# keisuke-777/HandyRL

Measured on AMD Instinct MI355X. Metric: learner env-steps/sec at B=4096 T=32 (TicTacToe net, UPGO/VTRACE), higher is better.
Workload: dtype f32; 1 GPU; TicTacToe SimpleConv2dModel learner step: forward + IS ratios + fused HIP V-trace/UPGO scans + losses + backward + grad all-reduce + clip + Adam; global_batch=4096, per_gpu_batch=4096, seq_len=32, players=2, parallelism=dp1, hip_graph=True

## Files before the change

handyrl_amd/_native.py:

```python

import ctypes
import os

import torch

LIB_PATH = os.path.join(os.path.dirname(os.path.abspath(__file__)), '_lib', 'libhrl.so')
LIB_PATH = os.environ.get('HRL_LIB_PATH', LIB_PATH)

HRL_OK = 0
HRL_EINVAL = -22

ALG = {'MC': 0, 'TD': 1, 'UPGO': 2, 'VTRACE': 3}

_f32p = ctypes.c_void_p
_i64 = ctypes.c_int64
_dbl = ctypes.c_double

SIGNATURES = {
    'hrl_abi_version': (ctypes.c_int, []),
    'hrl_targets_set_short_form': (ctypes.c_int, [ctypes.c_int]),
    'hrl_strerror': (ctypes.c_char_p, [ctypes.c_int]),
    'hrl_compute_target': (ctypes.c_int, [
        ctypes.c_int, _f32p, _f32p, _f32p, _f32p, _f32p,
        _i64, _i64, _i64, _i64, _i64, _i64, _dbl, _dbl, _f32p, _f32p, ctypes.c_void_p]),
    'hrl_compute_targets_fused': (ctypes.c_int, [
        ctypes.c_int, ctypes.c_int, _f32p, _f32p, _f32p, _f32p, _f32p,
        _i64, _i64, _i64, _i64, _i64, _i64, _dbl, _dbl, _f32p, _f32p, ctypes.c_void_p]),
    'hrl_compute_targets_strided': (ctypes.c_int, [
        ctypes.c_int, ctypes.c_int, _f32p, _f32p, _f32p, _f32p, _f32p, ctypes.c_void_p,
        _i64, _i64, _i64, _i64, _i64, _dbl, _dbl, _f32p, _f32p, ctypes.c_void_p]),
    'hrl_bn_workspace_bytes': (ctypes.c_int64, [_i64, _i64, _i64]),
    'hrl_bn_forward_train': (ctypes.c_int, [
        _f32p, _i64, _i64, _i64, _f32p, _f32p, _f32p, _f32p, _dbl, _dbl, ctypes.c_int, _f32p, _f32p, _f32p,
        ctypes.c_void_p, _i64, ctypes.c_void_p]),
    'hrl_bn_backward': (ctypes.c_int, [
        _f32p, _f32p, _i64, _i64, _i64, _f32p, _f32p, _f32p, _f32p, ctypes.c_int, _f32p, _f32p, _f32p,
        ctypes.c_void_p, _i64, ctypes.c_void_p]),
    'hrl_bn_workspace_bytes_grouped': (ctypes.c_int64, [_i64, _i64, _i64, _i64]),
    'hrl_bn_forward_train_grouped': (ctypes.c_int, [
        _f32p, _i64, _i64, _i64, _i64, _f32p, _f32p, _f32p, _f32p, _dbl, _dbl, ctypes.c_int, _f32p, _f32p, _f32p,
        ctypes.c_void_p, _i64, ctypes.c_void_p]),
    'hrl_bn_backward_grouped': (ctypes.c_int, [
        _f32p, _f32p, _i64, _i64, _i64, _i64, _f32p, _f32p, _f32p, _f32p, ctypes.c_int, _f32p, _f32p, _f32p,
        ctypes.c_void_p, _i64, ctypes.c_void_p]),
    'hrl_loss_workspace_bytes': (ctypes.c_int64, [_i64, _i64, _i64, _i64]),
    'hrl_loss_forward': (ctypes.c_int, [
        _f32p, _f32p, ctypes.c_void_p, _i64, _i64, _i64, _i64, _i64,
        _f32p, _f32p, _f32p, _f32p, _f32p, _f32p, _f32p, _f32p, _f32p,
        ctypes.c_int, ctypes.c_int, ctypes.c_int, _dbl, _dbl, _dbl, _dbl,
        ctypes.c_void_p, _i64, _f32p, ctypes.c_void_p]),
    'hrl_loss_backward': (ctypes.c_int, [
        _f32p, ctypes.c_void_p, _i64, _i64, _i64, _i64, _i64,
        _f32p, _f32p, _f32p, _f32p, _f32p, _f32p, _dbl, _dbl,
        ctypes.c_void_p, _i64, _f32p, _f32p, _f32p, _f32p, ctypes.c_void_p]),
    'hrl_loss_partials': (ctypes.c_int64, [_i64, _i64, _i64, _i64, ctypes.c_void_p]),
    'hrl_loss_forward_ex': (ctypes.c_int, [
        _f32p, _f32p, ctypes.c_void_p, _i64, _i64, _i64, _i64, _i64,
        _f32p, _f32p, _f32p, _f32p, _f32p, _f32p, _f32p, _f32p, _f32p,
        ctypes.c_int, ctypes.c_int, ctypes.c_int, _dbl, _dbl, _dbl, _dbl,
        ctypes.c_void_p, _i64, _f32p, _f32p, _f32p, _f32p, _i64, ctypes.c_int, ctypes.c_void_p]),
    'hrl_loss_backward_ex': (ctypes.c_int, [
        _f32p, ctypes.c_void_p, _i64, _i64, _i64, _i64, _i64,
        _f32p, _f32p, _f32p, _f32p, _f32p, _f32p, _dbl, _dbl,
        ctypes.c_void_p, _i64, _f32p, _f32p, _f32p, _f32p, _f32p, _f32p, _f32p, _i64, _f32p, _f32p,
        ctypes.c_void_p]),
    'hrl_output_mask_forward': (ctypes.c_int, [_f32p, _f32p, _f32p, _f32p, _f32p, _i64, _i64, _i64, _i64, _f32p,
                                               _f32p, ctypes.c_void_p]),
    'hrl_output_mask_backward': (ctypes.c_int, [_f32p, _f32p, _f32p, _f32p, _i64, _i64, _i64, _i64, _f32p, _f32p,
                                                ctypes.c_void_p]),
    'hrl_board_weight': (ctypes.c_int, [_f32p, _i64, _i64, _i64, _i64, _i64, _i64, _f32p, ctypes.c_void_p]),
    'hrl_board_fold': (ctypes.c_int, [_f32p, _i64, _i64, _i64, _i64, _i64, _i64, _f32p, ctypes.c_void_p]),
    'hrl_board_bias': (ctypes.c_int, [_f32p, _i64, _i64, _f32p, ctypes.c_void_p]),
    'hrl_board_bias_fold': (ctypes.c_int, [_f32p, _i64, _i64, _f32p, ctypes.c_void_p]),
    'hrl_conv3x3_workspace_bytes': (ctypes.c_int64, [_i64]),
    'hrl_conv3x3_forward': (ctypes.c_int, [_f32p, _i64, _i64, _i64, _f32p, _f32p, ctypes.c_int, _f32p,
                                           ctypes.c_void_p, _i64, ctypes.c_void_p]),
    'hrl_conv3x3_wgrad': (ctypes.c_int, [_f32p, _f32p, _i64, _i64, _i64, _f32p, ctypes.c_void_p, _i64,
                                         ctypes.c_void_p]),
    'hrl_colsum_workspace_bytes': (ctypes.c_int64, [_i64, _i64]),
    'hrl_colsum': (ctypes.c_int, [_f32p, _i64, _i64, _f32p, ctypes.c_void_p, _i64, ctypes.c_void_p]),
    'hrl_bn_finalize_stats': (ctypes.c_int, [ctypes.c_void_p, _i64, _i64, _i64, _f32p, _f32p, _f32p, _f32p,
                                             ctypes.c_double, ctypes.c_double, _f32p, _f32p, _f32p, _f32p,
                                             ctypes.c_void_p]),
    'hrl_bn_forward_eval': (ctypes.c_int, [_f32p, _i64, _i64, _i64, _f32p, _f32p, _f32p, _f32p, ctypes.c_double,
                                           ctypes.c_int, _f32p, _f32p, ctypes.c_void_p]),
    'hrl_bn_apply': (ctypes.c_int, [_f32p, _i64, _i64, _i64, _f32p, _f32p, ctypes.c_int, _f32p, ctypes.c_void_p]),
    'hrl_conv3x3_stats_blocks': (ctypes.c_int64, [_i64]),
    'hrl_conv3x3_block_sum_blocks': (ctypes.c_int64, [_i64]),
    'hrl_conv3x3_set_split': (ctypes.c_int, [ctypes.c_int]),
    'hrl_conv3x3_set_block_form': (ctypes.c_int, [ctypes.c_int]),
    'hrl_conv3x3_set_fwd_form': (ctypes.c_int, [ctypes.c_int]),
    'hrl_torus_set_split': (ctypes.c_int, [ctypes.c_int]),
    'hrl_torus_set_form': (ctypes.c_int, [ctypes.c_int]),
    'hrl_conv3x3_pack_n': (ctypes.c_int, [ctypes.c_void_p, ctypes.c_int, _f32p, ctypes.c_void_p]),
    'hrl_conv3x3_pack_n_zero': (ctypes.c_int, [ctypes.c_void_p, ctypes.c_int, _f32p, _f32p, _i64, ctypes.c_void_p]),
    'hrl_conv3x3_forward_ex': (ctypes.c_int, [_f32p, _i64, _f32p, _f32p, _f32p, _f32p, ctypes.c_int, _f32p,
                                              ctypes.c_int, _f32p, _f32p, _f32p, _f32p, ctypes.c_void_p,
                                              ctypes.c_void_p, _i64, ctypes.c_void_p]),
    'hrl_bn_finalize_backward': (ctypes.c_int, [ctypes.c_void_p, _i64, _i64, _i64, _f32p, _f32p, _f32p, _f32p,
                                                _f32p, _f32p, ctypes.c_void_p]),
    'hrl_bn_backward_apply': (ctypes.c_int, [_f32p, _f32p, _i64, _i64, _i64, _f32p, _f32p, _f32p, _f32p,
                                             ctypes.c_int, _f32p, _f32p, _f32p, ctypes.c_void_p]),
    'hrl_conv3x3_block_backward': (ctypes.c_int, [_f32p, _f32p, _i64, _f32p, _f32p, _f32p, _f32p, _f32p, _f32p,
                                                  _f32p, _f32p, _f32p, _f32p, _f32p, _f32p, ctypes.c_int, _f32p,
                                                  _f32p, _f32p, ctypes.c_void_p, ctypes.c_void_p, _i64,
                                                  ctypes.c_void_p]),
    'hrl_conv3x3_block_backward_dz': (ctypes.c_int, [_f32p, _f32p, _f32p, _f32p, _i64, _f32p, _f32p, _f32p, _f32p,
                                                     _f32p, _f32p, _f32p, _f32p, _f32p, _f32p, _f32p, _f32p,
                                                     ctypes.c_int, _f32p, _f32p, _f32p, ctypes.c_void_p,
                                                     ctypes.c_void_p, _i64, ctypes.c_void_p]),
    'hrl_conv3x3_wgrad_ex': (ctypes.c_int, [_f32p, _f32p, _f32p, _f32p, _i64, _f32p, ctypes.c_void_p, _i64,
                                            ctypes.c_void_p]),
    'hrl_hidden_gather': (ctypes.c_int, [ctypes.c_void_p, _f32p, _i64, _i64, ctypes.c_int, ctypes.c_void_p,
                                         ctypes.c_int, ctypes.c_void_p, ctypes.c_void_p]),
    'hrl_hidden_gather_backward': (ctypes.c_int, [ctypes.c_void_p, _f32p, _i64, _i64, ctypes.c_int, ctypes.c_void_p,
                                                  ctypes.c_int, ctypes.c_void_p, ctypes.c_void_p]),
    'hrl_hidden_gather_backward_add': (ctypes.c_int, [ctypes.c_void_p, _f32p, _i64, _i64, ctypes.c_int,
                                                      ctypes.c_void_p, ctypes.c_int, ctypes.c_void_p, ctypes.c_void_p,
                                                      ctypes.c_void_p, ctypes.c_void_p]),
    'hrl_hidden_update_gather': (ctypes.c_int, [ctypes.c_void_p, ctypes.c_void_p, _i64, _f32p, _f32p, _i64, _i64,
                                                ctypes.c_int, ctypes.c_void_p, ctypes.c_int, ctypes.c_void_p,
                                                ctypes.c_void_p, ctypes.c_void_p]),
    'hrl_hidden_update_gather_backward': (ctypes.c_int, [ctypes.c_void_p, _f32p, _f32p, _i64, _i64, _i64,
                                                         ctypes.c_int, ctypes.c_void_p, ctypes.c_int, ctypes.c_void_p,
                                                         ctypes.c_void_p, ctypes.c_void_p, ctypes.c_void_p,
                                                         ctypes.c_void_p, ctypes.c_void_p, ctypes.c_void_p]),
    'hrl_hidden_update_backward_add': (ctypes.c_int, [ctypes.c_void_p, _f32p, _i64, _i64, _i64, ctypes.c_int,
                                                      ctypes.c_void_p, ctypes.c_void_p, ctypes.c_void_p,
                                                      ctypes.c_void_p, ctypes.c_void_p, ctypes.c_void_p]),
    'hrl_hidden_update': (ctypes.c_int, [ctypes.c_void_p, ctypes.c_void_p, _i64, _f32p, _i64, _i64, ctypes.c_int,
                                         ctypes.c_void_p, ctypes.c_void_p, ctypes.c_void_p]),
    'hrl_hidden_update_backward': (ctypes.c_int, [ctypes.c_void_p, _f32p, _i64, _i64, _i64, ctypes.c_int,
                                                  ctypes.c_void_p, ctypes.c_void_p, ctypes.c_void_p, ctypes.c_void_p]),
    'hrl_lstm_gates_forward': (ctypes.c_int, [_f32p, _i64, _f32p, _f32p, _i64, _i64, _i64, _f32p, _i64, _f32p,
                                              _f32p, _f32p, ctypes.c_void_p]),
    'hrl_lstm_gates_backward': (ctypes.c_int, [_f32p, _f32p, _f32p, _f32p, _f32p, _i64, _i64, _i64, _f32p, _f32p,
                                               ctypes.c_void_p]),
    'hrl_torus_workspace_bytes': (ctypes.c_int64, [_i64]),
    'hrl_torus_stats_blocks': (ctypes.c_int64, [_i64]),
    'hrl_torus_conv_forward': (ctypes.c_int, [_f32p, _i64, _i64, _i64, _i64, _i64, _f32p, _f32p, ctypes.c_int,
                                              _f32p, ctypes.c_void_p, _f32p, _f32p, ctypes.c_void_p, _i64,
                                              ctypes.c_void_p]),
    'hrl_stem_workspace_bytes': (ctypes.c_int64, [_i64]),
    'hrl_stem_forward': (ctypes.c_int, [_f32p, _i64, _i64, _f32p, _f32p, _f32p, ctypes.c_void_p]),
    'hrl_stem_wgrad': (ctypes.c_int, [_f32p, _f32p, _i64, _i64, _f32p, _f32p, ctypes.c_void_p, _i64,
                                      ctypes.c_void_p]),
    'hrl_stem_set_wgrad_form': (ctypes.c_int, [ctypes.c_int]),
    'hrl_stem_set_fwd_form': (ctypes.c_int, [ctypes.c_int]),
    'hrl_clip_grad_norm': (ctypes.c_int, [_f32p, _i64, _dbl, _f32p, ctypes.c_void_p]),
    'hrl_clip_workspace_bytes': (ctypes.c_int64, [_i64]),
    'hrl_grad_fold_norm_blocks': (ctypes.c_int64, [_i64]),
    'hrl_grad_fold_norm': (ctypes.c_int, [_f32p, _i64, ctypes.c_void_p, ctypes.c_void_p, ctypes.c_void_p,
                                          ctypes.c_void_p, ctypes.c_void_p, ctypes.c_void_p, ctypes.c_void_p,
                                          ctypes.c_int, _f32p, ctypes.c_void_p, ctypes.c_void_p, ctypes.c_int,
                                          ctypes.c_void_p, _i64, ctypes.c_void_p]),
    'hrl_grad_fold_norm_ex': (ctypes.c_int, [_f32p, _i64, ctypes.c_void_p, ctypes.c_void_p, ctypes.c_void_p,
                                             ctypes.c_void_p, ctypes.c_void_p, ctypes.c_void_p, ctypes.c_void_p,
                                             ctypes.c_int, _f32p, ctypes.c_void_p, ctypes.c_void_p, ctypes.c_int,
                                             ctypes.c_void_p, _i64, ctypes.c_void_p, _i64, _dbl, _f32p,
                                             ctypes.c_void_p]),
    'hrl_adam_clip': (ctypes.c_int, [_f32p, _i64, ctypes.c_void_p, _dbl, _f32p, ctypes.c_void_p, ctypes.c_void_p,
                                     ctypes.c_void_p, ctypes.c_int, _f32p, _f32p, _f32p, _f32p, _dbl, _dbl, _dbl,
                                     _dbl, ctypes.c_void_p, ctypes.c_int, _f32p, ctypes.c_void_p]),
    'hrl_conv3x3_wgrad_partials': (ctypes.c_int64, [_i64, ctypes.c_void_p]),
    'hrl_stem_wgrad_partials': (ctypes.c_int64, [_i64, ctypes.c_void_p]),
    'hrl_clip_grad_norm_ws': (ctypes.c_int, [_f32p, _i64, _dbl, _f32p, ctypes.c_void_p, _i64, ctypes.c_void_p]),
    'hrl_heads_workspace_bytes': (ctypes.c_int64, [_i64]),
    'hrl_heads_bn_parts': (ctypes.c_int64, [_i64]),
    'hrl_heads_set_bwd_form': (ctypes.c_int, [ctypes.c_int]),
    'hrl_heads_forward': (ctypes.c_int, [_f32p, _i64, _f32p, _f32p, _f32p, _f32p, _f32p, _f32p, _f32p, _f32p,
                                         _f32p, _f32p, _f32p, _f32p, ctypes.c_int, ctypes.c_void_p]),
    'hrl_heads_backward': (ctypes.c_int, [_f32p, _i64, _f32p, _f32p, _f32p, _f32p, _f32p, _f32p, _f32p,
                                          ctypes.c_void_p, _f32p, _f32p, _f32p, _f32p, _f32p, _f32p, _f32p, _f32p,
                                          _f32p, _f32p, _f32p, _f32p, ctypes.c_void_p, _i64, ctypes.c_void_p]),
    'hrl_heads_backward_dz': (ctypes.c_int, [_f32p, _i64, _f32p, _f32p, _f32p, _f32p, _f32p, _f32p, _f32p,
                                             ctypes.c_void_p, _f32p, _f32p, _f32p, _f32p, _f32p, _f32p, _f32p, _f32p,
                                             _f32p, _f32p, _f32p, _f32p, ctypes.c_void_p, _i64, ctypes.c_void_p]),
    'hrl_bn_apply_residual': (ctypes.c_int, [_f32p, _f32p, _i64, _i64, _i64, _f32p, _f32p, _f32p, ctypes.c_void_p]),
    'hrl_bn_backward_masked': (ctypes.c_int, [_f32p, _f32p, _f32p, _i64, _i64, _i64, _f32p, _f32p, _f32p, _f32p,
                                              _f32p, _f32p, ctypes.c_void_p, _i64, ctypes.c_void_p]),
    'hrl_torus_conv_wgrad': (ctypes.c_int, [_f32p, _f32p, _i64, _i64, _i64, _i64, _i64, _f32p, _f32p,
                                            ctypes.c_void_p, _i64, ctypes.c_void_p]),
    'hrl_torus_conv_wgrad_bn': (ctypes.c_int, [_f32p, _i64, _i64, _i64, _i64, _f32p, _f32p, _f32p, _f32p,
                                               ctypes.c_int, _f32p, _f32p, _f32p, _f32p, _f32p, _f32p, _f32p, _f32p,
                                               ctypes.c_void_p, _i64, ctypes.c_void_p]),
    'hrl_bn_backward_masked_coefs': (ctypes.c_int, [_f32p, _f32p, _f32p, _i64, _i64, _i64, _f32p, _f32p, _f32p,
                                                    _f32p, _f32p, _f32p, _f32p, ctypes.c_void_p, _i64,
                                                    ctypes.c_void_p]),
    'hrl_torus_unit_forward': (ctypes.c_int, [_f32p, _f32p, _f32p, _f32p, _f32p, _i64, _i64, _i64, _f32p, _f32p,
                                              _f32p, ctypes.c_void_p, ctypes.c_void_p, _i64, ctypes.c_void_p]),
    'hrl_torus_unit_input_grad': (ctypes.c_int, [_f32p, _i64, _i64, _i64, _f32p, _f32p, _f32p, _f32p, _f32p,
                                                 _f32p, _f32p, ctypes.c_void_p, ctypes.c_void_p, _i64,
                                                 ctypes.c_void_p]),
    'hrl_board_conv_workspace_bytes': (ctypes.c_int64, [_i64]),
    'hrl_board_conv_forward': (ctypes.c_int, [_f32p, _i64, _i64, _i64, _i64, _f32p, _i64, _i64, _i64, _f32p, _f32p,
                                              ctypes.c_void_p, _i64, ctypes.c_void_p]),
    'hrl_board_conv_pack': (ctypes.c_int, [_f32p, _i64, _i64, _i64, ctypes.c_void_p, _i64, ctypes.c_void_p]),
    'hrl_board_conv_forward_packed': (ctypes.c_int, [_f32p, _i64, _i64, _i64, _i64, ctypes.c_void_p, _i64, _f32p,
                                                     _f32p, ctypes.c_void_p]),
    'hrl_gboard_pack_bytes': (ctypes.c_int64, [_i64, _i64]),
    'hrl_gboard_pack': (ctypes.c_int, [_f32p, _i64, _i64, _i64, _i64, ctypes.c_void_p, _i64, ctypes.c_void_p]),
    'hrl_gboard_pack_adjoint': (ctypes.c_int, [_f32p, _i64, _i64, _i64, _i64, ctypes.c_void_p, _i64,
                                               ctypes.c_void_p]),
    'hrl_gboard_wgrad_workspace_bytes': (ctypes.c_int64, [_i64, _i64, _i64]),
    'hrl_gboard_wgrad': (ctypes.c_int, [ctypes.c_void_p, ctypes.c_void_p, ctypes.c_void_p, ctypes.c_void_p,
                                        ctypes.c_void_p, ctypes.c_int, _i64, _i64, _f32p, _i64, _i64, _f32p,
                                        ctypes.c_void_p, _i64, ctypes.c_void_p]),
    'hrl_gboard_set_whole_ring': (ctypes.c_int, [ctypes.c_int]),
    'hrl_gboard_set_nctw': (ctypes.c_int, [ctypes.c_int]),
    'hrl_gboard_launch_stats': (ctypes.c_int, [ctypes.c_void_p, ctypes.c_int, ctypes.c_int]),
    'hrl_gboard_pointwise_wgrad_workspace_bytes': (_i64, [_i64, _i64, _i64]),
    'hrl_gboard_pointwise_wgrad': (ctypes.c_int, [_f32p, _i64, _f32p, _i64, _i64, _i64, _i64, _f32p, ctypes.c_void_p,
                                                  _i64, ctypes.c_void_p]),
    'hrl_gboard_forward_groups': (ctypes.c_int, [ctypes.c_void_p, ctypes.c_void_p, _i64, _i64, _i64, ctypes.c_void_p,
                                                 _i64, _i64, _f32p, _i64, ctypes.c_void_p]),
    'hrl_lstm_gates_backward_ex': (ctypes.c_int, [_f32p, _f32p, _f32p, _f32p, _i64, ctypes.c_int, _i64, _f32p, _i64,
                                                  _i64, _i64, _f32p, _f32p, _f32p, ctypes.c_int, ctypes.c_void_p]),
    'hrl_lstm_gates_forward_grouped': (ctypes.c_int, [ctypes.c_int, _f32p, _i64, ctypes.c_void_p, ctypes.c_void_p,
                                                      ctypes.c_void_p, _i64, _i64, _i64, ctypes.c_void_p,
                                                      ctypes.c_void_p, ctypes.c_void_p, ctypes.c_void_p]),
    'hrl_gboard_forward': (ctypes.c_int, [_f32p, _i64, _f32p, _i64, _i64, _i64, _i64, ctypes.c_void_p, _i64, _i64,
                                          _f32p, _f32p, _f32p, ctypes.c_int, _f32p, _i64, ctypes.c_void_p]),
    'hrl_gboard_pointwise': (ctypes.c_int, [_f32p, _i64, _i64, _f32p, _i64, _i64, _i64, _f32p, _i64, _f32p, _f32p,
                                            ctypes.c_int, _f32p, _i64, ctypes.c_void_p]),
    'hrl_torus_head_pool': (ctypes.c_int, [_f32p, _f32p, _i64, _i64, _i64, _i64, _f32p, _f32p, ctypes.c_void_p]),
    'hrl_torus_head_unpool': (ctypes.c_int, [_f32p, _f32p, _f32p, _i64, _i64, _i64, _i64, _f32p,
                                             ctypes.c_void_p]),
    'hrl_bn_backward_apply_masked': (ctypes.c_int, [_f32p, _f32p, _f32p, _i64, _i64, _i64, _f32p, _f32p, _f32p,
                                                    _f32p, _f32p, _f32p, ctypes.c_void_p]),
    'hrl_geister_legal': (ctypes.c_int, [ctypes.c_void_p, ctypes.c_void_p, ctypes.c_void_p, _i64, ctypes.c_void_p,
                                         ctypes.c_void_p]),
    'hrl_geister_observation': (ctypes.c_int, [ctypes.c_void_p, ctypes.c_void_p, ctypes.c_void_p, ctypes.c_void_p,
                                               _i64, ctypes.c_int, _f32p, _f32p, ctypes.c_void_p]),
    'hrl_geister_step': (ctypes.c_int, [ctypes.c_void_p, ctypes.c_void_p, ctypes.c_void_p, ctypes.c_void_p,
                                        ctypes.c_void_p, ctypes.c_void_p, ctypes.c_void_p, ctypes.c_void_p,
                                        ctypes.c_void_p, _i64, ctypes.c_void_p, ctypes.c_void_p]),
    'hrl_selfplay_sample_record': (ctypes.c_int, [_f32p, _i64, ctypes.c_void_p, _f32p, ctypes.c_void_p, _f32p,
                                                  ctypes.c_void_p, ctypes.c_void_p, ctypes.c_void_p, _i64, _i64,
                                                  _i64, _i64, ctypes.c_void_p, _f32p, _f32p, ctypes.c_void_p, _f32p,
                                                  ctypes.c_void_p, ctypes.c_void_p, ctypes.c_void_p]),
    'hrl_masked_rows_copy': (ctypes.c_int, [ctypes.c_int, ctypes.c_void_p, ctypes.c_void_p, ctypes.c_void_p,
                                            ctypes.c_void_p, ctypes.c_void_p, ctypes.c_void_p, _i64,
                                            ctypes.c_void_p]),
    'hrl_geister_observation_record': (ctypes.c_int, [ctypes.c_void_p, ctypes.c_void_p, ctypes.c_void_p,
                                                      ctypes.c_void_p, _i64, ctypes.c_int, _f32p, _f32p,
                                                      ctypes.c_void_p, ctypes.c_void_p, _i64, _f32p, _f32p,
                                                      ctypes.c_void_p]),
    'hrl_geister_observation_record_at': (ctypes.c_int, [ctypes.c_void_p, ctypes.c_void_p, ctypes.c_void_p,
                                                         ctypes.c_void_p, _i64, ctypes.c_int, _f32p, _f32p,
                                                         ctypes.c_void_p, ctypes.c_void_p, _i64, _f32p, _f32p,
                                                         ctypes.c_void_p]),
    'hrl_selfplay_sample_record_stream': (ctypes.c_int, [_f32p, _i64, ctypes.c_void_p, ctypes.c_uint64,
                                                         ctypes.c_void_p, ctypes.c_void_p, _f32p, ctypes.c_void_p,
                                                         ctypes.c_void_p, ctypes.c_void_p, _i64, _i64, _i64, _i64,
                                                         ctypes.c_void_p, _f32p, _f32p, ctypes.c_void_p, _f32p,
                                                         ctypes.c_void_p, ctypes.c_void_p, ctypes.c_void_p]),
    'hrl_selfplay_harvest': (ctypes.c_int, [ctypes.c_void_p, ctypes.c_void_p, ctypes.c_void_p, _f32p, _dbl,
                                            ctypes.c_void_p, ctypes.c_void_p, ctypes.c_void_p, ctypes.c_void_p,
                                            ctypes.c_void_p, ctypes.c_void_p]),
    'hrl_eval_act': (ctypes.c_int, [_f32p, _i64, ctypes.c_void_p, ctypes.c_uint64, _dbl, ctypes.c_void_p,
                                    ctypes.c_void_p, ctypes.c_void_p, ctypes.c_void_p, _i64, ctypes.c_void_p, _i64, _i64,
                                    _i64, _i64, _i64, ctypes.c_void_p, ctypes.c_void_p, ctypes.c_void_p, _f32p,
                                    ctypes.c_void_p, ctypes.c_void_p]),
# ... 83 lines not shown
```

handyrl_amd/csrc/hrl_conv.hip:

```cpp

#include <hip/hip_runtime.h>
#include <stdint.h>
#include <stdlib.h>

#include <type_traits>

#include "../../include/hrl_nn.h"
#include "../../include/hrl_targets.h"
#include "hrl_split.h"
#include "hrl_stamps.h"

namespace {

HRL_STAMP_DECL

typedef float f32x4 __attribute__((ext_vector_type(4)));

constexpr int kBoard = 3;
constexpr int kCells = kBoard * kBoard;
constexpr int kTaps = 9;
constexpr int kC = 32;
constexpr int kRow = kC * kCells;
constexpr int kStride = kRow + 2;
constexpr int kTile = 16;
// ... 386 lines not shown
                }
            }
        }
        __builtin_amdgcn_wave_barrier();
    }
    __syncthreads();
    float *red = lds;
    constexpr int kW = kTaps * kC * kC;
#pragma unroll
    for (int t = 0; t < kTaps; ++t)
#pragma unroll
        for (int it = 0; it < 2; ++it)
#pragma unroll
            for (int jt = 0; jt < 2; ++jt)
#pragma unroll
                for (int r = 0; r < 4; ++r) {
                    const int ci = it * 16 + (lane >> 4) * 4 + r;
                    const int co = jt * 16 + (lane & 15);
                    red[wave * kW + (t * kC + ci) * kC + co] = acc[t][it][jt][r];
                }
    __syncthreads();
    float *out = partial + (int64_t)blockIdx.x * kW;
    for (int i = threadIdx.x; i < kW; i += kThreads)
        out[i] = ((red[i] + red[kW + i]) + red[2 * kW + i]) + red[3 * kW + i];
}

constexpr int kStrideW = kRow + 4;
typedef float f32x16 __attribute__((ext_vector_type(16)));
typedef __bf16 bf16x8_t __attribute__((ext_vector_type(8)));

__device__ __forceinline__ f32x16 mfma32(const uint4 &a, const uint4 &b, f32x16 c) {
    return __builtin_amdgcn_mfma_f32_32x32x16_bf16(__builtin_bit_cast(bf16x8_t, a), __builtin_bit_cast(bf16x8_t, b),
                                                   c, 0, 0, 0);
}

template <bool PRO>
__global__ __launch_bounds__(kThreads) void conv3x3_wgrad_split_kernel(const float *__restrict__ x,
                                                                       const float *__restrict__ in_alpha,
                                                                       const float *__restrict__ in_beta,
                                                                       const float *__restrict__ dy, int64_t M,
                                                                       float *__restrict__ partial) {
    __shared__ __attribute__((aligned(16))) float lds[2 * kWaves * kTile * kStrideW];
    static_assert(2 * kWaves * kTile * kStrideW >= kWaves * kTaps * kC * kC, "fold buffer");
    const int lane = threadIdx.x & 63;
    const int wave = threadIdx.x >> 6;
    float *xs = lds + wave * kTile * kStrideW;
    float *gs = lds + (kWaves + wave) * kTile * kStrideW;
    const int r = lane & 31, h = lane >> 5;
    float pa = 1.f, pb = 0.f;
    if constexpr (PRO) {
        pa = in_alpha[r];
        pb = in_beta[r];
    }
    const int64_t ntiles = (M + kTile - 1) / kTile;
    const int64_t stride = (int64_t)gridDim.x * kWaves;
    const int64_t lim = M * kRow;

    f32x16 acc[kTaps];
#pragma unroll
    for (int t = 0; t < kTaps; ++t)
#pragma unroll
        for (int i = 0; i < 16; ++i) acc[t][i] = 0.f;

    for (int64_t tile = (int64_t)blockIdx.x * kWaves + wave; tile < ntiles; tile += stride) {
        {
            const int64_t base = tile * kTile * kRow;
            float4 sx[kVec], sg[kVec];
#pragma unroll
            for (int k = 0; k < kVec; ++k) {
                const int64_t e = base + (int64_t)(k * 64 + lane) * 4;
                const int64_t ec = e < lim ? e : lim - 4;
                sx[k] = *reinterpret_cast<const float4 *>(x + ec);
                sg[k] = *reinterpret_cast<const float4 *>(dy + ec);
            }
#pragma unroll
            for (int k = 0; k < kVec; ++k) {
                const int e = (k * 64 + lane) * 4;
                const int row = e / kRow, c = e - row * kRow;
                const bool ok = base + e < lim;
                *reinterpret_cast<float4 *>(xs + row * kStrideW + c) = sx[k];
                *reinterpret_cast<float4 *>(gs + row * kStrideW + c) = ok ? sg[k] : make_float4(0.f, 0.f, 0.f, 0.f);
            }
        }
        __builtin_amdgcn_s_waitcnt(0xc07f);
        __builtin_amdgcn_wave_barrier();

        uint4 Bh[kCells], Bm[kCells], Bl[kCells];
        const float *gcol = gs + (8 * h) * kStrideW + r * kCells;
#pragma unroll
        for (int q = 0; q < kCells; ++q) {
            float v[8];
#pragma unroll
            for (int j = 0; j < 8; ++j) v[j] = gcol[j * kStrideW + q];
            hrl_split::split8(v, Bh[q], Bm[q], Bl[q]);
        }
        const float *xcol = xs + (8 * h) * kStrideW + r * kCells;
#pragma unroll
        for (int p = 0; p < kCells; ++p) {
            float v[8];
#pragma unroll
            for (int j = 0; j < 8; ++j) {
                float a = xcol[j * kStrideW + p];
                if constexpr (PRO) {
                    const float t = a * pa + pb;
                    a = t < 0.f ? 0.f : t;
                }
                v[j] = a;
            }
            uint4 Ah, Am, Al;
            hrl_split::split8(v, Ah, Am, Al);
#pragma unroll
            for (int q = 0; q < kCells; ++q) {
                const int tap = tap_of(p, q);
                if (tap < 0) continue;
                f32x16 c = acc[tap];
                c = mfma32(Al, Bh[q], c);
                c = mfma32(Am, Bm[q], c);
                c = mfma32(Ah, Bl[q], c);
                c = mfma32(Am, Bh[q], c);
                c = mfma32(Ah, Bm[q], c);
                c = mfma32(Ah, Bh[q], c);
                acc[tap] = c;
            }
        }
        __builtin_amdgcn_wave_barrier();
    }
    __syncthreads();
    float *red = lds;
    constexpr int kW = kTaps * kC * kC;
#pragma unroll
    for (int t = 0; t < kTaps; ++t)
#pragma unroll
        for (int i = 0; i < 16; ++i) {
            const int ci = (i & 3) + 8 * (i >> 2) + 4 * h;
            red[wave * kW + (t * kC + ci) * kC + r] = acc[t][i];
        }
    __syncthreads();
    float *out = partial + (int64_t)blockIdx.x * kW;
    for (int i = threadIdx.x; i < kW; i += kThreads)
        out[i] = ((red[i] + red[kW + i]) + red[2 * kW + i]) + red[3 * kW + i];
}

struct BlockBwdArgs {
    const float *g, *y;
    const float *bn_w, *bn_b, *bn_mean, *bn_invstd, *bn_k, *bn_gm;
    const float *x, *in_alpha, *in_beta;
    const float *wpk;
    const float *ep_mean, *ep_alpha, *ep_beta;
    float *gin;
    double *part;
    float *wpart;
    int64_t M;
    const float *w1p = nullptr, *w1v = nullptr;
};

typedef unsigned int u32x3 __attribute__((ext_vector_type(3)));
typedef unsigned int u32x2 __attribute__((ext_vector_type(2)));
typedef unsigned int u32x4 __attribute__((ext_vector_type(4)));

__device__ __forceinline__ __amdgpu_buffer_rsrc_t wave_rsrc(const void *base, uint32_t bytes) {
    const uint64_t p = reinterpret_cast<uint64_t>(base);
    const uint32_t lo = __builtin_amdgcn_readfirstlane((uint32_t)p);
    const uint32_t hi = __builtin_amdgcn_readfirstlane((uint32_t)(p >> 32));
    const uint32_t n = __builtin_amdgcn_readfirstlane(bytes);
    return __builtin_amdgcn_make_buffer_rsrc(reinterpret_cast<void *>(((uint64_t)hi << 32) | lo), (short)0, (int)n,
                                             0x00020000);
}

__device__ __forceinline__ void load_cells(__amdgpu_buffer_rsrc_t rs, int off, float (&d)[kCells]) {
#pragma unroll
    for (int m = 0; m < 3; ++m) {
        const u32x3 v = __builtin_amdgcn_raw_buffer_load_b96(rs, off + 12 * m, 0, 0);
        d[3 * m + 0] = __uint_as_float(v.x);
        d[3 * m + 1] = __uint_as_float(v.y);
        d[3 * m + 2] = __uint_as_float(v.z);
    }
}

__device__ __forceinline__ void store_cells(__amdgpu_buffer_rsrc_t rs, int off, const float (&d)[kCells]) {
#pragma unroll
    for (int m = 0; m < 3; ++m) {
        u32x3 v;
        v.x = __float_as_uint(d[3 * m + 0]);
        v.y = __float_as_uint(d[3 * m + 1]);
        v.z = __float_as_uint(d[3 * m + 2]);
        __builtin_amdgcn_raw_buffer_store_b96(v, rs, off + 12 * m, 0, 0);
    }
}

template <bool PRO, int EPI, bool DG>
__global__ __launch_bounds__(kThreads) void conv3x3_block_bwd_kernel(BlockBwdArgs a) {
    constexpr int kWWords = kTaps * 2 * 3 * 64 * 4;
    constexpr int kTileF = kTile * kStride;
    constexpr int kW = kTaps * kC * kC;
    constexpr int kFoldF = (kWaves - 1) * kW;
    constexpr int kUseF = DG ? kWWords + kWaves * kTileF : 0;
    constexpr int kSmemF = kUseF > kFoldF ? kUseF : kFoldF;
    __shared__ __attribute__((aligned(16))) float smem[kSmemF];
    uint32_t *w_lds_u = reinterpret_cast<uint32_t *>(smem);
    const int lane = threadIdx.x & 63;
    const int wave = threadIdx.x >> 6;
    float *as = smem + kWWords + wave * kTileF;
    if constexpr (DG) {
        for (int i = threadIdx.x; i < kWWords; i += kThreads) {
            const int d = i & 3, l = (i >> 2) & 63, f = i >> 8;
            const int part = f % 3, tc = f / 3;
            const int ci = 8 * (l >> 4) + 2 * d, j = l & 15;
            const float w0 = a.wpk[(tc * kC + ci) * 16 + j];
            const float w1 = a.wpk[(tc * kC + ci + 1) * 16 + j];
            w_lds_u[i] = split_part(w0, part) | (split_part(w1, part) << 16);
        }
    }
    const int r = lane & 31, h = lane >> 5;
    const float mu = a.bn_mean[r], kk = a.bn_k[r], gmn = a.bn_gm[r], is = a.bn_invstd[r];
    const float ww = a.bn_w ? a.bn_w[r] : 1.0f;
    const float al = is * ww;
    const float be = (a.bn_b ? a.bn_b[r] : 0.0f) - mu * al;
    float pa = 1.f, pb = 0.f;
    if constexpr (PRO) {
        pa = a.in_alpha[r];
        pb = a.in_beta[r];
    }
    float em = 0.f, ea = 1.f, eb = 0.f;
    if constexpr (DG && EPI == 2) {
        em = a.ep_mean[r];
        ea = a.ep_alpha[r];
        eb = a.ep_beta[r];
    }
    double s1 = 0.0, s2 = 0.0;
    f32x16 wacc[kTaps];
#pragma unroll
    for (int t = 0; t < kTaps; ++t)
#pragma unroll
        for (int i = 0; i < 16; ++i) wacc[t][i] = 0.f;
    if constexpr (DG) __syncthreads();

    const int64_t ntiles = (a.M + kTile - 1) / kTile;
    const int64_t stride = (int64_t)gridDim.x * kWaves;
    const int off0 = ((8 * h) * kRow + r * kCells) * 4;
    HRL_STAMP_WALL(14);
    int st_it = 0;
    for (int64_t tile = (int64_t)blockIdx.x * kWaves + wave; tile < ntiles; tile += stride, ++st_it) {
        if (st_it < 2) HRL_STAMP(6 * st_it + 0);
        const int64_t row0 = tile * kTile;
        const int rows = (int)min<int64_t>(kTile, a.M - row0);
        const uint32_t bytes = (uint32_t)rows * kRow * 4;
        const int64_t eofs = row0 * kRow;
        const __amdgpu_buffer_rsrc_t rg = wave_rsrc(a.g + eofs, bytes);
        const __amdgpu_buffer_rsrc_t ry = wave_rsrc(a.y + eofs, bytes);
        const __amdgpu_buffer_rsrc_t rx = wave_rsrc(a.x + eofs, bytes);
        float G[8][kCells], X[8][kCells];
        {
            float Y[8][kCells];
            auto bn_apply = [&]() __attribute__((always_inline)) {
#pragma unroll
                for (int j = 0; j < 8; ++j) {
                    const bool valid = 8 * h + j < rows;
#pragma unroll
                    for (int c = 0; c < kCells; ++c) {
                        const float yv = Y[j][c];
                        float gv = G[j][c];
                        if (!(yv * al + be > 0.f)) gv = 0.f;
                        const float t = (yv - mu) * kk;
                        const float d = (((gv - gmn) - t) * is) * ww;
                        G[j][c] = valid ? d : 0.f;
                    }
                }
            };
#pragma unroll
            for (int j = 0; j < 8; ++j) {
                load_cells(rg, off0 + j * kRow * 4, G[j]);
                load_cells(ry, off0 + j * kRow * 4, Y[j]);
                load_cells(rx, off0 + j * kRow * 4, X[j]);
            }
            bn_apply();
        }
        if (st_it < 2) HRL_STAMP(6 * st_it + 1);
        if constexpr (DG) {
#pragma unroll
            for (int j = 0; j < 8; ++j)
#pragma unroll
                for (int c = 0; c < kCells; ++c) as[(8 * h + j) * kStride + r * kCells + c] = G[j][c];
        }
        {
            uint4 Bh[kCells], Bm[kCells], Bl[kCells];
#pragma unroll
            for (int q = 0; q < kCells; ++q) {
                float v[8];
#pragma unroll
                for (int j = 0; j < 8; ++j) v[j] = G[j][q];
                hrl_split::split8(v, Bh[q], Bm[q], Bl[q]);
            }
#pragma unroll
            for (int p = 0; p < kCells; ++p) {
                float v[8];
#pragma unroll
                for (int j = 0; j < 8; ++j) {
                    float xv = X[j][p];
                    if constexpr (PRO) {
                        const float t = xv * pa + pb;
                        xv = t < 0.f ? 0.f : t;
                    }
                    v[j] = xv;
                }
                uint4 Ah, Am, Al;
                hrl_split::split8(v, Ah, Am, Al);
#pragma unroll
                for (int q = 0; q < kCells; ++q) {
                    const int tap = tap_of(p, q);
                    if (tap < 0) continue;
                    f32x16 c = wacc[tap];
                    c = mfma32(Al, Bh[q], c);
                    c = mfma32(Am, Bm[q], c);
                    c = mfma32(Ah, Bl[q], c);
                    c = mfma32(Am, Bh[q], c);
                    c = mfma32(Ah, Bm[q], c);
                    c = mfma32(Ah, Bh[q], c);
                    wacc[tap] = c;
                }
            }
        }
        if (st_it < 2) HRL_STAMP(6 * st_it + 2);
        if constexpr (DG) {
            float R[8][kCells];
            if constexpr (EPI == 2 || EPI == 3) {
#pragma unroll
                for (int j = 0; j < 8; ++j) load_cells(rx, off0 + j * kRow * 4, R[j]);
            }
            __builtin_amdgcn_s_waitcnt(0xc07f);
            __builtin_amdgcn_wave_barrier();
            f32x4 acc[kCells][2];
#pragma unroll
            for (int q = 0; q < kCells; ++q) acc[q][0] = acc[q][1] = (f32x4){0.f, 0.f, 0.f, 0.f};
            split_tile_mfma<false, true>(as, w_lds_u, lane, nullptr, nullptr, acc);
            __builtin_amdgcn_s_waitcnt(0xc07f);
            __builtin_amdgcn_wave_barrier();
            if (st_it < 2) HRL_STAMP(6 * st_it + 3);
#pragma unroll
            for (int q = 0; q < kCells; ++q)
#pragma unroll
                for (int ct = 0; ct < 2; ++ct)
#pragma unroll
                    for (int rr = 0; rr < 4; ++rr) {
                        const int row = (lane >> 4) * 4 + rr;
                        const int co = ct * 16 + (lane & 15);
                        as[row * kStride + co * kCells + q] = acc[q][ct][rr];
                    }
            __builtin_amdgcn_s_waitcnt(0xc07f);
            __builtin_amdgcn_wave_barrier();
            const __amdgpu_buffer_rsrc_t ro = wave_rsrc(a.gin + eofs, bytes);
            float t1 = 0.f, t2 = 0.f;
#pragma unroll
            for (int j = 0; j < 8; ++j) {
                const bool valid = 8 * h + j < rows;
                float o[kCells];
#pragma unroll
                for (int c = 0; c < kCells; ++c) {
                    float v = as[(8 * h + j) * kStride + r * kCells + c];
                    const float rv = (EPI == 2 || EPI == 3) ? R[j][c] : 0.f;
                    if constexpr (EPI == 3) {
                        if (!(rv > 0.f)) v = 0.f;
                    } else if constexpr (EPI == 2) {
                        const float gm = (rv * ea + eb > 0.f && valid) ? v : 0.f;
                        t1 += gm;
                        t2 += gm * (rv - em);
                    }
                    o[c] = v;
                }
                store_cells(ro, off0 + j * kRow * 4, o);
            }
            if constexpr (EPI == 2) {
                s1 += (double)t1;
                s2 += (double)t2;
            }
            __builtin_amdgcn_s_waitcnt(0xc07f);
            __builtin_amdgcn_wave_barrier();
        }
        if (st_it < 2) HRL_STAMP(6 * st_it + 4);
    }
    HRL_STAMP(12);
    __syncthreads();
    float *red = smem;
    if (wave > 0) {
#pragma unroll
        for (int t = 0; t < kTaps; ++t)
#pragma unroll
            for (int i = 0; i < 16; ++i) {
                const int ci = (i & 3) + 8 * (i >> 2) + 4 * h;
                red[(wave - 1) * kW + (t * kC + ci) * kC + r] = wacc[t][i];
            }
    }
    __syncthreads();
    if (wave == 0) {
        float *out = a.wpart + (int64_t)blockIdx.x * kW;
#pragma unroll
        for (int t = 0; t < kTaps; ++t)
#pragma unroll
            for (int i = 0; i < 16; ++i) {
                const int idx = (t * kC + (i & 3) + 8 * (i >> 2) + 4 * h) * kC + r;
                out[idx] = ((wacc[t][i] + red[idx]) + red[kW + idx]) + red[2 * kW + idx];
            }
    }
    if constexpr (DG && EPI == 2) {
        __syncthreads();
        double *dred = reinterpret_cast<double *>(smem);
        dred[((wave * 2 + h) * kC + r) * 2 + 0] = s1;
        dred[((wave * 2 + h) * kC + r) * 2 + 1] = s2;
        __syncthreads();
        if (threadIdx.x < 2 * kC) {
            const int c = threadIdx.x >> 1, k = threadIdx.x & 1;
            double t = 0.0;
            for (int i = 0; i < 2 * kWaves; ++i) t += dred[(i * kC + c) * 2 + k];
            a.part[((int64_t)blockIdx.x * kC + c) * 2 + k] = t;
        }
    }
    HRL_STAMP(13);
    HRL_STAMP_WALL(15);
}

namespace bb2 {

constexpr int kWaves = 8;
constexpr int kThreads = 64 * kWaves;
constexpr int kPartBytes = kCells * kC * kTile * 2;
constexpr int kImgBytes = 3 * kPartBytes;
constexpr int kDy0 = 0;
constexpr int kX0 = 2 * kImgBytes;
constexpr int kXrStride = kRow + 4;
constexpr int kXrBytes = kTile * kXrStride * 4;
constexpr int kXr0 = 4 * kImgBytes;
constexpr int kLdsBytes = kXr0 + 2 * kXrBytes;
static_assert(kLdsBytes <= 160 * 1024, "LDS");
constexpr int kDzStride = 28;
constexpr int kDzBytes = kTile * kDzStride * 4;
constexpr int kDz0 = kLdsBytes;
constexpr int kLdsBytesDz = kDz0 + 2 * kDzBytes;
static_assert(kLdsBytesDz <= 160 * 1024, "LDS");
static_assert(kDzBytes / 4 <= 7 * 64, "a dword per lane of waves 0..6");

typedef short v4s __attribute__((ext_vector_type(4)));
typedef __attribute__((address_space(3))) v4s lds_v4s;

__device__ __forceinline__ int img_off(int c, int ch, int half) {
    const int R = ch >> 3, j = ch & 7;
    return c * 1024 + R * 256 + 16 * ((2 * j + half) ^ (9 * (R & 1)));
}

__device__ __forceinline__ void bar_lds() {
    asm volatile("s_waitcnt lgkmcnt(0)" ::: "memory");
    __builtin_amdgcn_s_barrier();
    asm volatile("" ::: "memory");
}

template <int W> struct Role;
template <> struct Role<0> { static constexpr bool kIg = true, kCFirst = true; static constexpr int kCt = 0, kNq = 5, kNt = 0;
                             static constexpr int kQ[5] = {4, 5, 6, 7, 8}; static constexpr int kTap[1] = {0}; };
template <> struct Role<1> { static constexpr bool kIg = true, kCFirst = true; static constexpr int kCt = 1, kNq = 5, kNt = 0;
                             static constexpr int kQ[5] = {4, 5, 6, 7, 8}; static constexpr int kTap[1] = {0}; };
template <> struct Role<2> { static constexpr bool kIg = true, kCFirst = false; static constexpr int kCt = 0, kNq = 4, kNt = 0;
                             static constexpr int kQ[4] = {0, 1, 2, 3}; static constexpr int kTap[1] = {0}; };
template <> struct Role<3> { static constexpr bool kIg = true, kCFirst = false; static constexpr int kCt = 1, kNq = 4, kNt = 0;
                             static constexpr int kQ[4] = {0, 1, 2, 3}; static constexpr int kTap[1] = {0}; };
template <> struct Role<4> { static constexpr bool kIg = false, kCFirst = false; static constexpr int kCt = 0, kNq = 0, kNt = 2;
                             static constexpr int kQ[1] = {0}; static constexpr int kTap[2] = {0, 1}; };
template <> struct Role<5> { static constexpr bool kIg = false, kCFirst = false; static constexpr int kCt = 0, kNq = 0, kNt = 2;
                             static constexpr int kQ[1] = {0}; static constexpr int kTap[2] = {2, 5}; };
template <> struct Role<6> { static constexpr bool kIg = false, kCFirst = true; static constexpr int kCt = 0, kNq = 0, kNt = 2;
                             static constexpr int kQ[1] = {0}; static constexpr int kTap[2] = {3, 4}; };
template <> struct Role<7> { static constexpr bool kIg = false, kCFirst = true; static constexpr int kCt = 0, kNq = 0, kNt = 3;
                             static constexpr int kQ[1] = {0}; static constexpr int kTap[3] = {6, 7, 8}; };

template <int W> __device__ constexpr bool uses_p(int p) {
    using R = Role<W>;
    if constexpr (R::kIg) {
        for (int s = 0; s < R::kNq; ++s)
            if (tap_of(p, R::kQ[s]) >= 0) return true;
    } else {
        for (int s = 0; s < R::kNt; ++s) {
            const int dy = R::kTap[s] / 3, dx = R::kTap[s] % 3;
            const int qy = p / 3 - dy + 1, qx = p % 3 - dx + 1;
            if (qy >= 0 && qy < 3 && qx >= 0 && qx < 3) return true;
        }
    }
    return false;
}
template <int W> __device__ constexpr bool uses_tap(int t) {
    using R = Role<W>;
    for (int s = 0; s < R::kNq; ++s)
        for (int p = 0; p < kCells; ++p)
            if (tap_of(p, R::kQ[s]) == t) return true;
    return false;
}

#ifdef HRL_STAMPS
#define BB2_STAMP(it, k)                                                                                        \
    do {                                                                                                       \
        if ((it) == 2 || (it) == 3) {                                                                          \
            const unsigned long long t_ = __builtin_amdgcn_s_memtime();                                        \
            if (lane == 0 && g_hrl_stamps)                                                                     \
                g_hrl_stamps[(((size_t)blockIdx.x * 8 + W) * 2 + (it) - 2) * 8 + (k)] = t_;                    \
        }                                                                                                      \
    } while (0)
#else
#define BB2_STAMP(it, k) do { } while (0)
#endif

template <bool PRO, int EPI, int W, bool DZ = false>
__device__ __forceinline__ void run(const BlockBwdArgs &a, unsigned char *smem, int lane) {
    static_assert(!DZ || EPI == 2, "the dz form is the last chain block's");
    using R = Role<W>;
    constexpr bool kIg = R::kIg;
    constexpr int kNq = R::kNq > 0 ? R::kNq : 1;
    constexpr int kNt = R::kNt > 0 ? R::kNt : 1;
    constexpr int kCt = R::kCt;
    const int ch = lane & 31, hh = lane >> 5;
    constexpr bool kFwd = EPI == 1;
    float mu = 0.f, kk = 0.f, gmn = 0.f, is = 1.f, ww = 1.f, al = 1.f, be = 0.f;
    if constexpr (!kFwd) {
        kk = a.bn_k[ch]; gmn = a.bn_gm[ch];
        mu = a.bn_mean[ch]; is = a.bn_invstd[ch];
        ww = a.bn_w ? a.bn_w[ch] : 1.0f;
        al = is * ww;
        be = (a.bn_b ? a.bn_b[ch] : 0.0f) - mu * al;
    }
    float pa = 1.f, pb = 0.f;
    if constexpr (PRO) {
        pa = a.in_alpha[ch];
        pb = a.in_beta[ch];
    }
    float w1[3] = {0.f, 0.f, 0.f};
    if constexpr (DZ) {
        w1[0] = a.w1p[ch];
        w1[1] = a.w1p[kC + ch];
        w1[2] = a.w1v[ch];
    }
    uint4 wh[kTaps], wm[kTaps], wl[kTaps];
    if constexpr (kIg) {
        const int ci0 = 8 * (lane >> 4), j = lane & 15;
#pragma unroll
        for (int t = 0; t < kTaps; ++t) {
            if (!uses_tap<W>(t)) continue;
            uint32_t hv[4], mv[4], lv[4];
#pragma unroll
            for (int d = 0; d < 4; ++d) {
                const int tc = t * 2 + kCt;
                const float w0 = a.wpk[(tc * kC + ci0 + 2 * d) * 16 + j];
                const float w1 = a.wpk[(tc * kC + ci0 + 2 * d + 1) * 16 + j];
                uint32_t h0, m0, l0, h1, m1, l1;
                hrl_split::split3(w0, h0, m0, l0);
                hrl_split::split3(w1, h1, m1, l1);
                hv[d] = h0 | (h1 << 16);
                mv[d] = m0 | (m1 << 16);
                lv[d] = l0 | (l1 << 16);
            }
            wh[t] = make_uint4(hv[0], hv[1], hv[2], hv[3]);
            wm[t] = make_uint4(mv[0], mv[1], mv[2], mv[3]);
            wl[t] = make_uint4(lv[0], lv[1], lv[2], lv[3]);
        }
    }
    float em = 0.f, ea = 1.f, eb = 0.f;
    if constexpr (EPI == 2 && kIg) {
        em = a.ep_mean[kCt * 16 + (lane & 15)];
        ea = a.ep_alpha[kCt * 16 + (lane & 15)];
        eb = a.ep_beta[kCt * 16 + (lane & 15)];
    }
    double s1 = 0.0, s2 = 0.0;
    f32x16 wacc[kNt];
#pragma unroll
    for (int t = 0; t < kNt; ++t)
#pragma unroll
        for (int i = 0; i < 16; ++i) wacc[t][i] = 0.f;

    const int64_t ntiles = (a.M + kTile - 1) / kTile;
    const int64_t t0 = blockIdx.x;
    const int64_t step = gridDim.x;
    const int n_iter = t0 < ntiles ? (int)((ntiles - 1 - t0) / step + 1) : 0;
    const int rho0 = 2 * ((W + (ch >> 2)) & 7);
    const int c0 = hh ? 4 : 0;
    const int ldoff = (rho0 * kRow + ch * kCells + c0) * 4;
    float G[2][5], Y[2][5], X[2][5];
    auto rsrc_of = [&](const float *base, int it, int &rows) __attribute__((always_inline)) {
        const int64_t t = t0 + (int64_t)it * step;
        const bool ok = it < n_iter;
        rows = ok ? (int)min<int64_t>(kTile, a.M - t * kTile) : 0;
        return wave_rsrc(base + (ok ? t * kTile * kRow : 0), (uint32_t)rows * kRow * 4);
    };
    auto issue = [&](int it) __attribute__((always_inline)) {
        int rows;
        const __amdgpu_buffer_rsrc_t rg = rsrc_of(a.g, it, rows), ry = rsrc_of(a.y, it, rows),
                                     rx = rsrc_of(a.x, it, rows);
#pragma unroll
        for (int r = 0; r < 2; ++r) {
            const int off = ldoff + r * kRow * 4;
#pragma unroll
            for (int k = kFwd ? 2 : (DZ ? 1 : 0); k < 3; ++k) {
                const __amdgpu_buffer_rsrc_t rs = k == 0 ? rg : (k == 1 ? ry : rx);
                float(&d)[5] = k == 0 ? G[r] : (k == 1 ? Y[r] : X[r]);
                const u32x3 v = __builtin_amdgcn_raw_buffer_load_b96(rs, off, 0, 0);
                const u32x2 u = __builtin_amdgcn_raw_buffer_load_b64(rs, off + 12, 0, 0);
                d[0] = __uint_as_float(v.x);
                d[1] = __uint_as_float(v.y);
                d[2] = __uint_as_float(v.z);
                d[3] = __uint_as_float(u.x);
                d[4] = __uint_as_float(u.y);
            }
        }
    };
    auto load_dz = [&](int it) __attribute__((always_inline)) {
        float v = 0.f;
        if constexpr (DZ && W < 7) {
            const int64_t t = t0 + (int64_t)it * step;
            const bool ok = it < n_iter;
            const int rows = ok ? (int)min<int64_t>(kTile, a.M - t * kTile) : 0;
            const __amdgpu_buffer_rsrc_t rz =
                wave_rsrc(a.g + (ok ? t * kTile * kDzStride : 0), (uint32_t)rows * kDzStride * 4);
            v = __uint_as_float(__builtin_amdgcn_raw_buffer_load_b32(rz, (W * 64 + lane) * 4, 0, 0));
        }
        return v;
    };
    auto put_dz = [&](int it, float v) __attribute__((always_inline)) {
        if constexpr (DZ && W < 7)
            reinterpret_cast<float *>(smem + kDz0 + (it & 1) * kDzBytes)[W * 64 + lane] = v;
    };
    float DZv = 0.f;
    auto stage = [&](int it) __attribute__((always_inline)) {
        const int64_t t = t0 + (int64_t)it * step;
        const int rows = (int)max<int64_t>(0, min<int64_t>(kTile, a.M - t * kTile));
        unsigned char *dyi = smem + kDy0 + (it & 1) * kImgBytes;
        unsigned char *xi = smem + kX0 + (it & 1) * kImgBytes;
        const float *dzl = reinterpret_cast<const float *>(smem + kDz0 + (it & 1) * kDzBytes);
        uint32_t dp[3][5], xp[3][5];
#pragma unroll
        for (int i = 0; i < 5; ++i) {
            float dv[2], xv2[2];
#pragma unroll
            for (int r = 0; r < 2; ++r) {
                const bool valid = rho0 + r < rows;
                const float yv = Y[r][i];
                float gv;
                if constexpr (DZ) {
                    const float *dzr = dzl + (rho0 + r) * kDzStride + c0 + i;
                    gv = 0.f;
#pragma unroll
                    for (int m = 0; m < 3; ++m) gv += w1[m] * dzr[m * kCells];
                } else {
                    gv = G[r][i];
                }
                if (!(yv * al + be > 0.f)) gv = 0.f;
                const float tt = (yv - mu) * kk;
                float d = (((gv - gmn) - tt) * is) * ww;
                d = valid ? d : 0.f;
                float xv = X[r][i];
                if constexpr (PRO) {
                    const float u = xv * pa + pb;
                    xv = u < 0.f ? 0.f : u;
                }
                if constexpr (kFwd) d = xv;
                dv[r] = d;
                xv2[r] = xv;
            }
            hrl_split::split_pair(dv[0], dv[1], dp[0][i], dp[1][i], dp[2][i]);
            if constexpr (!kFwd) hrl_split::split_pair(xv2[0], xv2[1], xp[0][i], xp[1][i], xp[2][i]);
        }
        const int half = rho0 >> 3, sub = 2 * (rho0 & 7);
#pragma unroll
        for (int i = 0; i < 5; ++i) {
            const int o = img_off(c0 + i, ch, half) + sub;
#pragma unroll
            for (int part = 0; part < 3; ++part) {
                *reinterpret_cast<uint32_t *>(dyi + part * kPartBytes + o) = dp[part][i];
                if constexpr (!kFwd) *reinterpret_cast<uint32_t *>(xi + part * kPartBytes + o) = xp[part][i];
            }
        }
        if constexpr (EPI == 2 || EPI == 3) {
            float *xr = reinterpret_cast<float *>(smem + kXr0 + (it & 1) * kXrBytes);
#pragma unroll
            for (int r = 0; r < 2; ++r)
#pragma unroll
                for (int i = 0; i < 5; ++i) xr[(rho0 + r) * kXrStride + ch * kCells + c0 + i] = X[r][i];
        }
    };
    f32x4 acc[kNq];
    auto compute = [&](int it) __attribute__((always_inline)) {
        const unsigned char *dyi = smem + kDy0 + (it & 1) * kImgBytes;
        if constexpr (!kIg && kFwd) {
        } else if constexpr (!kIg) {
            const unsigned char *xi = smem + kX0 + (it & 1) * kImgBytes;
            const int kg = lane >> 5;
#pragma unroll
            for (int p = 0; p < kCells; ++p) {
                if (!uses_p<W>(p)) continue;
                const int o = img_off(p, ch, kg);
                const uint4 Ah = *reinterpret_cast<const uint4 *>(xi + o);
                const uint4 Am = *reinterpret_cast<const uint4 *>(xi + kPartBytes + o);
                const uint4 Al = *reinterpret_cast<const uint4 *>(xi + 2 * kPartBytes + o);
#pragma unroll
                for (int s = 0; s < R::kNt; ++s) {
                    const int dy = R::kTap[s] / 3, dx = R::kTap[s] % 3;
                    const int qy = p / 3 - dy + 1, qx = p % 3 - dx + 1;
                    if (qy < 0 || qy > 2 || qx < 0 || qx > 2) continue;
                    const int ob = img_off(qy * 3 + qx, ch, kg);
                    const uint4 Bh = *reinterpret_cast<const uint4 *>(dyi + ob);
                    const uint4 Bm = *reinterpret_cast<const uint4 *>(dyi + kPartBytes + ob);
                    const uint4 Bl = *reinterpret_cast<const uint4 *>(dyi + 2 * kPartBytes + ob);
                    f32x16 c = wacc[s];
                    c = mfma32(Al, Bh, c);
                    c = mfma32(Am, Bm, c);
                    c = mfma32(Ah, Bl, c);
                    c = mfma32(Am, Bh, c);
                    c = mfma32(Ah, Bm, c);
                    c = mfma32(Ah, Bh, c);
                    wacc[s] = c;
                }
            }
        } else {
#pragma unroll
            for (int s = 0; s < kNq; ++s) acc[s] = (f32x4){0.f, 0.f, 0.f, 0.f};
            const int g = lane >> 4, i = lane & 15, qq = i >> 2, pp = i & 3;
            const int tr_sub = 8 * (pp & 1);
#pragma unroll
            for (int p = 0; p < kCells; ++p) {
                if (!uses_p<W>(p)) continue;
                uint32_t A[3][4];
#pragma unroll
                for (int part = 0; part < 3; ++part) {
#pragma unroll
                    for (int hlf = 0; hlf < 2; ++hlf) {
                        const int o = part * kPartBytes + img_off(p, 8 * g + 4 * hlf + qq, pp >> 1) + tr_sub;
                        const v4s r = __builtin_amdgcn_ds_read_tr16_b64_v4i16(
                            (lds_v4s *)((__attribute__((address_space(3))) unsigned char *)(dyi + o)));
                        const uint2 u = __builtin_bit_cast(uint2, r);
                        A[part][2 * hlf] = u.x;
                        A[part][2 * hlf + 1] = u.y;
                    }
                }
                const uint4 Ah = make_uint4(A[0][0], A[0][1], A[0][2], A[0][3]);
                const uint4 Am = make_uint4(A[1][0], A[1][1], A[1][2], A[1][3]);
                const uint4 Al = make_uint4(A[2][0], A[2][1], A[2][2], A[2][3]);
#pragma unroll
                for (int s = 0; s < R::kNq; ++s) {
                    const int tap = tap_of(p, R::kQ[s]);
                    if (tap < 0) continue;
                    const uint4 Bl = wl[tap];
                    f32x4 c = acc[s];
                    c = mfma_bf16(Al, wh[tap], c);
                    c = mfma_bf16(Am, wm[tap], c);
                    c = mfma_bf16(Ah, Bl, c);
                    c = mfma_bf16(Am, wh[tap], c);
                    c = mfma_bf16(Ah, wm[tap], c);
                    c = mfma_bf16(Ah, wh[tap], c);
                    acc[s] = c;
                }
            }
        }
    };
    auto epilogue = [&](int it) __attribute__((always_inline)) {
        if constexpr (kIg) {
            int rows;
            const __amdgpu_buffer_rsrc_t ro = rsrc_of(a.gin, it, rows);
            const int co = kCt * 16 + (lane & 15);
            float rv[kNq < 4 ? 4 : kNq][4];
            if constexpr (EPI == 2 || EPI == 3) {
                const float *xr = reinterpret_cast<const float *>(smem + kXr0 + (it & 1) * kXrBytes);
#pragma unroll
                for (int rr = 0; rr < 4; ++rr) {
                    const int row = (lane >> 4) * 4 + rr;
#pragma unroll
                    for (int s = 0; s < R::kNq; ++s) rv[s][rr] = xr[row * kXrStride + co * kCells + R::kQ[s]];
                }
            }
            if constexpr (EPI == 1) {
                float t1 = 0.f, t2 = 0.f;
#pragma unroll
                for (int s = 0; s < R::kNq; ++s) {
#pragma unroll
                    for (int rr = 0; rr < 4; ++rr) {
                        const int row = (lane >> 4) * 4 + rr;
                        const float u = row < rows ? acc[s][rr] : 0.f;
                        t1 += u;
                        t2 += u * u;
                    }
                }
                s1 += (double)t1;
                s2 += (double)t2;
            }
            if constexpr (EPI == 2) {
                float t1 = 0.f, t2 = 0.f;
#pragma unroll
                for (int s = 0; s < R::kNq; ++s) {
#pragma unroll
                    for (int rr = 0; rr < 4; ++rr) {
                        const int row = (lane >> 4) * 4 + rr;
                        const float x0 = rv[s][rr];
                        const float gm = (x0 * ea + eb > 0.f && row < rows) ? acc[s][rr] : 0.f;
                        t1 += gm;
                        t2 += gm * (x0 - em);
                    }
                }
                s1 += (double)t1;
                s2 += (double)t2;
            }
#pragma unroll
            for (int rr = 0; rr < 4; ++rr) {
                const int row = (lane >> 4) * 4 + rr;
                const int off = (row * kRow + co * kCells + R::kQ[0]) * 4;
                float v[kNq];
#pragma unroll
                for (int s = 0; s < R::kNq; ++s) {
                    v[s] = acc[s][rr];
                    if constexpr (EPI == 3)
                        if (!(rv[s][rr] > 0.f)) v[s] = 0.f;
                }
                u32x4 w;
                w.x = __float_as_uint(v[0]);
                w.y = __float_as_uint(v[1]);
                w.z = __float_as_uint(v[2]);
                w.w = __float_as_uint(v[3]);
                __builtin_amdgcn_raw_buffer_store_b128(w, ro, off, 0, 0);
                if constexpr (R::kNq > 4)
                    __builtin_amdgcn_raw_buffer_store_b32(__float_as_uint(v[4 % kNq]), ro, off + 16, 0, 0);
            }
        }
    };

    if constexpr (DZ) {
        if (n_iter > 0) {
            const float d0 = load_dz(0), d1 = load_dz(1);
            issue(0);
            put_dz(0, d0);
            put_dz(1, d1);
            DZv = load_dz(2);
        }
        bar_lds();
        if (n_iter > 0) {
            stage(0);
            issue(1);
        }
    } else if (n_iter > 0) {
        issue(0);
        stage(0);
        issue(1);
    }
    bar_lds();
    for (int it = 0; it < n_iter; ++it) {
        BB2_STAMP(it, 0);
        if constexpr (R::kCFirst) {
            compute(it);
            epilogue(it);
            BB2_STAMP(it, 1);
            stage(it + 1);
            if constexpr (DZ) {
                put_dz(it + 2, DZv);
                DZv = load_dz(it + 3);
            }
            issue(it + 2);
            BB2_STAMP(it, 2);
        } else {
            stage(it + 1);
            if constexpr (DZ) {
                put_dz(it + 2, DZv);
                DZv = load_dz(it + 3);
            }
            issue(it + 2);
            BB2_STAMP(it, 1);
            compute(it);
            epilogue(it);
            BB2_STAMP(it, 2);
        }
        bar_lds();
        BB2_STAMP(it, 3);
    }
    if constexpr (!kIg && !kFwd) {
        constexpr int kW = kTaps * kC * kC;
        float *outp = a.wpart + (int64_t)blockIdx.x * kW;
        const int h = lane >> 5;
#pragma unroll
        for (int s = 0; s < R::kNt; ++s)
#pragma unroll
            for (int i = 0; i < 16; ++i) {
                const int ci = (i & 3) + 8 * (i >> 2) + 4 * h;
                outp[(R::kTap[s] * kC + ci) * kC + ch] = wacc[s][i];
            }
    }
    if constexpr (EPI == 1 || EPI == 2) {
        __syncthreads();
        double *dred = reinterpret_cast<double *>(smem);
        if (kIg) {
            dred[(W * 64 + lane) * 2 + 0] = s1;
            dred[(W * 64 + lane) * 2 + 1] = s2;
        }
        __syncthreads();
        if (W == 0) {
            const int c = lane >> 1, k = lane & 1, ct = c >> 4, l16 = c & 15;
            double tot = 0.0;
            for (int w = ct; w < 4; w += 2)
                for (int lg = 0; lg < 4; ++lg) tot += dred[(w * 64 + lg * 16 + l16) * 2 + k];
            a.part[((int64_t)blockIdx.x * kC + c) * 2 + k] = tot;
        }
    }
}

}

namespace fw3 {

constexpr int kSlots = 5;
constexpr int kRawBytes = kTile * kRow * 4;
constexpr int kPieces = kRawBytes / 1024;
constexpr int kImg0 = 0;
constexpr int kRaw0 = 2 * bb2::kImgBytes;
constexpr int kLdsBytes = kRaw0 + kSlots * kRawBytes;
static_assert(kLdsBytes <= 160 * 1024, "LDS");
static_assert(kRawBytes % 1024 == 0, "whole LDS-DMA pieces per tile");

template <int N> __device__ __forceinline__ void vm_wait() { asm volatile("s_waitcnt vmcnt(%0)" ::"n"(N) : "memory"); }

__device__ __forceinline__ void dma16(u32x4 desc, uint32_t voff, uint32_t lds_byte) {
    uint32_t keep;
    asm volatile("s_mov_b32 %0, m0\n\ts_mov_b32 m0, %3\n\ts_nop 0\n\tbuffer_load_dwordx4 %1, %2, 0 offen lds\n\t"
                 "s_mov_b32 m0, %0"
                 : "=&s"(keep)
                 : "v"(voff), "s"(desc), "s"(lds_byte)
                 : "memory");
}

__device__ __forceinline__ u32x4 wave_desc(const void *base, uint32_t bytes) {
    const uint64_t p = reinterpret_cast<uint64_t>(base);
    u32x4 d;
    d.x = __builtin_amdgcn_readfirstlane((uint32_t)p);
    d.y = __builtin_amdgcn_readfirstlane((uint32_t)(p >> 32)) & 0xffffu;
    d.z = __builtin_amdgcn_readfirstlane(bytes);
    d.w = 0x00020000u;
    return d;
}

template <int G> struct Cells;
template <> struct Cells<0> { static constexpr int kN = 3; static constexpr int kQ[3] = {0, 1, 2}; };
template <> struct Cells<1> { static constexpr int kN = 2; static constexpr int kQ[2] = {3, 4}; };
template <> struct Cells<2> { static constexpr int kN = 2; static constexpr int kQ[2] = {5, 6}; };
template <> struct Cells<3> { static constexpr int kN = 2; static constexpr int kQ[2] = {7, 8}; };

template <int G> __device__ constexpr bool g_uses_p(int p) {
    for (int s = 0; s < Cells<G>::kN; ++s)
        if (tap_of(p, Cells<G>::kQ[s]) >= 0) return true;
    return false;
}
template <int G> __device__ constexpr bool g_uses_tap(int t) {
    for (int s = 0; s < Cells<G>::kN; ++s)
        for (int p = 0; p < kCells; ++p)
            if (tap_of(p, Cells<G>::kQ[s]) == t) return true;
    return false;
}

template <int W> __device__ constexpr int pieces_of() {
    int n = 0;
    for (int p = W; p < kPieces; p += 8) ++n;
    return n;
}

template <int NP, int NS>
__device__ __forceinline__ void wait_tile_after(int it) {
    static_assert((kSlots - 2) * (NP + NS) + NS <= 63, "vmcnt");
    if (it == 0) vm_wait<(kSlots - 2) * NP + NS>();
    else if (it == 1) vm_wait<(kSlots - 2) * NP + 2 * NS>();
    else if (it == 2) vm_wait<(kSlots - 2) * NP + 3 * NS>();
    else vm_wait<(kSlots - 2) * (NP + NS) + NS>();
    static_assert(kSlots == 5, "the early-iteration counts above are written for kSlots = 5");
}

template <bool PRO, int W>
__device__ __forceinline__ void run(const BlockBwdArgs &a, unsigned char *smem, int lane) {
    constexpr int kCt = W & 1, G = W >> 1;
    using C = Cells<G>;
    constexpr int kNq = C::kN;
    constexpr int NP = pieces_of<W>();
    constexpr int NS = 4;
    const int64_t ntiles = (a.M + kTile - 1) / kTile;
    const int64_t t0 = blockIdx.x;
    const int64_t step = gridDim.x;
    const int n_iter = t0 < ntiles ? (int)((ntiles - 1 - t0) / step + 1) : 0;
    const int ch = lane & 31, hh = lane >> 5;
    uint4 wh[kTaps], wm[kTaps], wl[kTaps];
    {
        const int ci0 = 8 * (lane >> 4), j = lane & 15;
#pragma unroll
        for (int t = 0; t < kTaps; ++t) {
            if (!g_uses_tap<G>(t)) continue;
            uint32_t hv[4], mv[4], lv[4];
#pragma unroll
            for (int d = 0; d < 4; ++d) {
                const int tc = t * 2 + kCt;
                const float w0 = a.wpk[(tc * kC + ci0 + 2 * d) * 16 + j];
                const float w1 = a.wpk[(tc * kC + ci0 + 2 * d + 1) * 16 + j];
                uint32_t h0, m0, l0, h1, m1, l1;
                hrl_split::split3(w0, h0, m0, l0);
                hrl_split::split3(w1, h1, m1, l1);
                hv[d] = h0 | (h1 << 16);
                mv[d] = m0 | (m1 << 16);
                lv[d] = l0 | (l1 << 16);
            }
            wh[t] = make_uint4(hv[0], hv[1], hv[2], hv[3]);
            wm[t] = make_uint4(mv[0], mv[1], mv[2], mv[3]);
            wl[t] = make_uint4(lv[0], lv[1], lv[2], lv[3]);
        }
    }
    float pa = 1.f, pb = 0.f;
    if constexpr (PRO) {
        pa = a.in_alpha[ch];
        pb = a.in_beta[ch];
    }
    asm volatile("s_waitcnt vmcnt(0)" ::: "memory");
    const uint32_t smem_base = (uint32_t)(uintptr_t)smem;
    auto dma = [&](int it, int slot) __attribute__((always_inline)) {
        const int64_t t = t0 + (int64_t)it * step;
        const bool ok = it < n_iter;
        const int rows = ok ? (int)min<int64_t>(kTile, a.M - t * kTile) : 0;
        const u32x4 desc = wave_desc(a.x + (ok ? t * kTile * kRow : 0), (uint32_t)rows * kRow * 4);
        const uint32_t raw = smem_base + kRaw0 + (uint32_t)slot * kRawBytes;
#pragma unroll
        for (int j = 0; j < NP; ++j) {
            const int p = W + 8 * j;
            dma16(desc, p * 1024 + lane * 16, raw + p * 1024);
        }
    };
    const int c0 = hh ? 4 : 0;
    const int rho0 = 2 * ((W + (ch >> 2)) & 7);
    auto stage = [&](int it, int slot) __attribute__((always_inline)) {
        const float *raw = reinterpret_cast<const float *>(smem + kRaw0 + slot * kRawBytes);
        unsigned char *xi = smem + kImg0 + (it & 1) * bb2::kImgBytes;
        uint32_t xp[3][5];
        float xv[2][5];
#pragma unroll
        for (int r = 0; r < 2; ++r) {
            const float *src = raw + (rho0 + r) * kRow + ch * kCells + c0;
#pragma unroll
            for (int i = 0; i < 5; ++i) {
                float v = src[i];
                if constexpr (PRO) {
                    const float u = v * pa + pb;
                    v = u < 0.f ? 0.f : u;
                }
                xv[r][i] = v;
            }
        }
#pragma unroll
        for (int i = 0; i < 5; ++i) hrl_split::split_pair(xv[0][i], xv[1][i], xp[0][i], xp[1][i], xp[2][i]);
        const int half = rho0 >> 3, sub = 2 * (rho0 & 7);
#pragma unroll
        for (int i = 0; i < 5; ++i) {
            const int o = bb2::img_off(c0 + i, ch, half) + sub;
#pragma unroll
            for (int part = 0; part < 3; ++part)
                *reinterpret_cast<uint32_t *>(xi + part * bb2::kPartBytes + o) = xp[part][i];
        }
    };
    const int co = kCt * 16 + (lane & 15);
    const int g = lane >> 4, i16 = lane & 15, qq = i16 >> 2, pp = i16 & 3;
    const int tr_sub = 8 * (pp & 1);
    double s1 = 0.0, s2 = 0.0;
#pragma unroll
    for (int j = 0; j < kSlots; ++j) dma(j, j);
    vm_wait<(kSlots - 1) * NP>();
    bb2::bar_lds();
    stage(0, 0);
    vm_wait<(kSlots - 2) * NP>();
    bb2::bar_lds();
    int slot = 0;
    for (int it = 0; it < n_iter; ++it) {
        BB2_STAMP(it, 0);
        dma(it + kSlots, slot);
        const int next = slot + 1 == kSlots ? 0 : slot + 1;
        stage(it + 1, next);
        BB2_STAMP(it, 1);
        const unsigned char *img = smem + kImg0 + (it & 1) * bb2::kImgBytes;
        f32x4 acc[kNq];
#pragma unroll
        for (int s = 0; s < kNq; ++s) acc[s] = (f32x4){0.f, 0.f, 0.f, 0.f};
#pragma unroll
        for (int p = 0; p < kCells; ++p) {
            if (!g_uses_p<G>(p)) continue;
            uint32_t A[3][4];
#pragma unroll
            for (int part = 0; part < 3; ++part) {
#pragma unroll
                for (int hlf = 0; hlf < 2; ++hlf) {
                    const int o = part * bb2::kPartBytes + bb2::img_off(p, 8 * g + 4 * hlf + qq, pp >> 1) + tr_sub;
                    const bb2::v4s r = __builtin_amdgcn_ds_read_tr16_b64_v4i16(
                        (bb2::lds_v4s *)((__attribute__((address_space(3))) unsigned char *)(img + o)));
                    const uint2 u = __builtin_bit_cast(uint2, r);
                    A[part][2 * hlf] = u.x;
                    A[part][2 * hlf + 1] = u.y;
                }
            }
            const uint4 Ah = make_uint4(A[0][0], A[0][1], A[0][2], A[0][3]);
            const uint4 Am = make_uint4(A[1][0], A[1][1], A[1][2], A[1][3]);
            const uint4 Al = make_uint4(A[2][0], A[2][1], A[2][2], A[2][3]);
#pragma unroll
            for (int s = 0; s < kNq; ++s) {
                const int tap = tap_of(p, C::kQ[s]);
                if (tap < 0) continue;
                f32x4 c = acc[s];
                c = mfma_bf16(Al, wh[tap], c);
                c = mfma_bf16(Am, wm[tap], c);
                c = mfma_bf16(Ah, wl[tap], c);
                c = mfma_bf16(Am, wh[tap], c);
                c = mfma_bf16(Ah, wm[tap], c);
                c = mfma_bf16(Ah, wh[tap], c);
                acc[s] = c;
            }
        }
        BB2_STAMP(it, 2);
        const int64_t t = t0 + (int64_t)it * step;
        const int rows = (int)min<int64_t>(kTile, a.M - t * kTile);
        const __amdgpu_buffer_rsrc_t od = wave_rsrc(a.gin + t * kTile * kRow, (uint32_t)rows * kRow * 4);
        float t1 = 0.f, t2 = 0.f;
#pragma unroll
        for (int s = 0; s < kNq; ++s) {
#pragma unroll
            for (int rr = 0; rr < 4; ++rr) {
                const int row = (lane >> 4) * 4 + rr;
                const float u = row < rows ? acc[s][rr] : 0.f;
                t1 += u;
                t2 += u * u;
            }
        }
        s1 += (double)t1;
        s2 += (double)t2;
#pragma unroll
        for (int rr = 0; rr < 4; ++rr) {
            const int row = (lane >> 4) * 4 + rr;
            const int off = (row * kRow + co * kCells + C::kQ[0]) * 4;
            if constexpr (kNq == 3) {
                u32x3 v;
                v.x = __float_as_uint(acc[0][rr]);
                v.y = __float_as_uint(acc[1][rr]);
                v.z = __float_as_uint(acc[2 % kNq][rr]);
                __builtin_amdgcn_raw_buffer_store_b96(v, od, off, 0, 0);
            } else {
                u32x2 v;
                v.x = __float_as_uint(acc[0][rr]);
                v.y = __float_as_uint(acc[1][rr]);
                __builtin_amdgcn_raw_buffer_store_b64(v, od, off, 0, 0);
            }
        }
        wait_tile_after<NP, NS>(it);
        BB2_STAMP(it, 3);
        bb2::bar_lds();
        slot = next;
    }
    vm_wait<0>();
    __syncthreads();
    double *dred = reinterpret_cast<double *>(smem);
    dred[(W * 64 + lane) * 2 + 0] = s1;
    dred[(W * 64 + lane) * 2 + 1] = s2;
    __syncthreads();
    if (W == 0) {
        const int c = lane >> 1, k = lane & 1, ct = c >> 4, l16 = c & 15;
        double tot = 0.0;
        for (int w = ct; w < 8; w += 2)
            for (int lg = 0; lg < 4; ++lg) tot += dred[(w * 64 + lg * 16 + l16) * 2 + k];
        a.part[((int64_t)blockIdx.x * kC + c) * 2 + k] = tot;
    }
}

}

template <bool PRO>
__global__ __launch_bounds__(bb2::kThreads) void conv3x3_fwd_dma_kernel(BlockBwdArgs a) {
    __shared__ __attribute__((aligned(16))) unsigned char smem[fw3::kLdsBytes];
    const int lane = threadIdx.x & 63;
    const int wave = __builtin_amdgcn_readfirstlane(threadIdx.x >> 6);
    switch (wave) {
    case 0: fw3::run<PRO, 0>(a, smem, lane); break;
    case 1: fw3::run<PRO, 1>(a, smem, lane); break;
    case 2: fw3::run<PRO, 2>(a, smem, lane); break;
    case 3: fw3::run<PRO, 3>(a, smem, lane); break;
    case 4: fw3::run<PRO, 4>(a, smem, lane); break;
    case 5: fw3::run<PRO, 5>(a, smem, lane); break;
    case 6: fw3::run<PRO, 6>(a, smem, lane); break;
    default: fw3::run<PRO, 7>(a, smem, lane); break;
    }
}

template <bool PRO, int EPI, bool DZ = false>
__global__ __launch_bounds__(bb2::kThreads) void conv3x3_block_bwd2_kernel(BlockBwdArgs a) {
    __shared__ __attribute__((aligned(16))) unsigned char smem[DZ ? bb2::kLdsBytesDz : bb2::kLdsBytes];
    const int lane = threadIdx.x & 63;
    const int wave = __builtin_amdgcn_readfirstlane(threadIdx.x >> 6);
    switch (wave) {
    case 0: bb2::run<PRO, EPI, 0, DZ>(a, smem, lane); break;
    case 1: bb2::run<PRO, EPI, 1, DZ>(a, smem, lane); break;
    case 2: bb2::run<PRO, EPI, 2, DZ>(a, smem, lane); break;
    case 3: bb2::run<PRO, EPI, 3, DZ>(a, smem, lane); break;
    case 4: bb2::run<PRO, EPI, 4, DZ>(a, smem, lane); break;
    case 5: bb2::run<PRO, EPI, 5, DZ>(a, smem, lane); break;
    case 6: bb2::run<PRO, EPI, 6, DZ>(a, smem, lane); break;
    default: bb2::run<PRO, EPI, 7, DZ>(a, smem, lane); break;
    }
}

__global__ __launch_bounds__(256) void conv3x3_wgrad_reduce_kernel(const float *__restrict__ partial, int nparts,
                                                                   float *__restrict__ dw) {
    __shared__ float red[4][64];
    constexpr int kW = kTaps * kC * kC;
    const int col = threadIdx.x & 63, sub = threadIdx.x >> 6;
    const int i = blockIdx.x * 64 + col;
    float s0 = 0.f, s1 = 0.f, s2 = 0.f, s3 = 0.f;
    int w = sub;
    for (; w + 12 < nparts; w += 16) {
        s0 += partial[(int64_t)w * kW + i];
        s1 += partial[(int64_t)(w + 4) * kW + i];
        s2 += partial[(int64_t)(w + 8) * kW + i];
        s3 += partial[(int64_t)(w + 12) * kW + i];
    }
    for (; w < nparts; w += 4) s0 += partial[(int64_t)w * kW + i];
    red[sub][col] = (s0 + s1) + (s2 + s3);
    __syncthreads();
    if (sub == 0) {
        const float s = ((red[0][col] + red[1][col]) + red[2][col]) + red[3][col];
        const int co = i % kC, ci = (i / kC) % kC, tap = i / (kC * kC);
        dw[(co * kC + ci) * kTaps + tap] = s;
    }
}

__global__ void conv3x3_pack_kernel(const float *__restrict__ w, int flip, float *__restrict__ wpk) {
    const int i = blockIdx.x * blockDim.x + threadIdx.x;
    if (i >= kTaps * 2 * kC * 16) return;
    const int j = i % 16, k = (i / 16) % kC, ct = (i / (16 * kC)) % 2, tap = i / (16 * kC * 2);
    const int out_c = ct * 16 + j;
    const int in_c = k;
    float v;
    if (!flip) v = w[(out_c * kC + in_c) * kTaps + tap];
    else v = w[(in_c * kC + out_c) * kTaps + (kTaps - 1 - tap)];
    wpk[i] = v;
}

constexpr int kPack = kTaps * 2 * kC * 16;
struct WeightList {
    const float *w[8];
};
__device__ __forceinline__ void pack_n_element(const WeightList &wl, int n, float *__restrict__ packed, int i) {
    if (i >= n * 2 * kPack) return;
    const int l = i / (2 * kPack), flip = (i / kPack) & 1, e = i % kPack;
    const int j = e % 16, k = (e / 16) % kC, ct = (e / (16 * kC)) % 2, tap = e / (16 * kC * 2);
    const int out_c = ct * 16 + j, in_c = k;
    const float *w = wl.w[l];
    packed[i] = !flip ? w[(out_c * kC + in_c) * kTaps + tap] : w[(in_c * kC + out_c) * kTaps + (kTaps - 1 - tap)];
}
__global__ void conv3x3_pack_n_kernel(WeightList wl, int n, float *__restrict__ packed) {
    pack_n_element(wl, n, packed, blockIdx.x * blockDim.x + threadIdx.x);
}

__global__ __launch_bounds__(256) void conv3x3_pack_n_zero_kernel(WeightList wl, int n, float *__restrict__ packed,
                                                                  int pack_blocks, float *__restrict__ zero,
                                                                  int64_t nz, int head, int64_t nvec) {
    if ((int)blockIdx.x < pack_blocks) {
        pack_n_element(wl, n, packed, blockIdx.x * blockDim.x + threadIdx.x);
        return;
    }
    const int64_t zb = (int64_t)blockIdx.x - pack_blocks;
    const int64_t v = zb * 256 + threadIdx.x;
    if (v < nvec) reinterpret_cast<float4 *>(zero + head)[v] = make_float4(0.f, 0.f, 0.f, 0.f);
    if (zb == 0) {
        const int t = threadIdx.x;
        const int64_t tail0 = head + nvec * 4;
        if (t < head) zero[t] = 0.f;
        if (tail0 + t < nz && t < 4) zero[tail0 + t] = 0.f;
    }
}

int g_split = 1;
int g_block_form = 1;
int g_fwd_form = 2;

constexpr int kGrid = 256;

int status() {
    const hipError_t e = hipGetLastError();
    return e == hipSuccess ? HRL_OK : HRL_ELAUNCH_BASE - (int)e;
}

bool aligned16(const void *p) { return (reinterpret_cast<uintptr_t>(p) & 15) == 0; }

int grid_for(int64_t M) {
    const int64_t tiles = (M + kTile - 1) / kTile;
    const int64_t blocks = (tiles + kWaves - 1) / kWaves;
    return (int)(blocks < kGrid ? blocks : kGrid);
}

}

extern "C" {

#ifdef HRL_STAMPS
int hrl_debug_set_stamps_conv(void *buf) { return (int)hipMemcpyToSymbol(HIP_SYMBOL(g_hrl_stamps), &buf, sizeof(buf)); }
#endif

int64_t hrl_conv3x3_workspace_bytes(int64_t M) {
    if (M < 1) return -1;
    return (int64_t)grid_for(M) * kTaps * kC * kC * 4 + (int64_t)kTaps * 2 * kC * 16 * 4 * 2;
}

int64_t hrl_conv3x3_stats_blocks(int64_t M) { return M < 1 ? -1 : grid_for(M); }

int64_t hrl_conv3x3_block_sum_blocks(int64_t M) { return M < 1 ? -1 : grid_for(M); }

int hrl_conv3x3_set_block_form(int form) {
    const int prev = g_block_form;
    g_block_form = form < 0 ? 0 : (form > 1 ? 1 : form);
    return prev;
}

int hrl_conv3x3_set_fwd_form(int form) {
    const int prev = g_fwd_form;
    g_fwd_form = form < 0 ? 0 : (form > 2 ? 2 : form);
    return prev;
}

int hrl_conv3x3_set_split(int on) {
    const int prev = g_split;
    g_split = on ? 1 : 0;
    return prev;
}

int hrl_conv3x3_forward_ex(const float *x, int64_t M, const float *in_alpha, const float *in_beta,
                           const float *weight, const float *bias, int flip, float *y, int epilogue,
                           const float *ref, const float *ep_mean, const float *ep_alpha, const float *ep_beta,
                           double *part, void *workspace, int64_t workspace_bytes, void *stream) {
    if (M < 1 || !x || !weight || !y || !workspace) return HRL_EINVAL;
    if (!aligned16(x) || !aligned16(y) || workspace_bytes < hrl_conv3x3_workspace_bytes(M)) return HRL_EINVAL;
    if ((in_alpha == nullptr) != (in_beta == nullptr)) return HRL_EINVAL;
    if (epilogue < 0 || epilogue > 3) return HRL_EINVAL;
    if ((epilogue == 1 || epilogue == 2) && !part) return HRL_EINVAL;
    if ((epilogue == 2 || epilogue == 3) && (!ref || !aligned16(ref))) return HRL_EINVAL;
    if (epilogue == 2 && (!ep_mean || !ep_alpha || !ep_beta)) return HRL_EINVAL;
    if (epilogue >= 2 && bias) return HRL_EINVAL;
    hipStream_t s = static_cast<hipStream_t>(stream);
    const float *wpk = weight;
    if (!(flip & 2)) {
        float *dst = static_cast<float *>(workspace);
        hipLaunchKernelGGL(conv3x3_pack_kernel, dim3((kPack + 255) / 256), dim3(256), 0, s, weight, flip & 1, dst);
        const int rc = status();
        if (rc) return rc;
        wpk = dst;
    }
    if (epilogue == 1 && (flip & 2) && !bias && g_split && g_fwd_form >= 1 && M * kRow * 4 <= 0xffffffffLL) {
        BlockBwdArgs a{};
        a.x = x; a.in_alpha = in_alpha; a.in_beta = in_beta; a.wpk = wpk; a.gin = y; a.part = part; a.M = M;
        const dim3 grid(grid_for(M)), block(bb2::kThreads);
        if (g_fwd_form == 2) {
// ... 26 lines not shown
#undef HRL_CONV_LAUNCH
    return status();
}

int hrl_conv3x3_pack_n(const float *const *weights, int n, float *packed, void *stream) {
    if (n < 1 || n > 8 || !weights || !packed) return HRL_EINVAL;
    WeightList wl{};
    for (int i = 0; i < n; ++i) {
        if (!weights[i]) return HRL_EINVAL;
        wl.w[i] = weights[i];
    }
    hipLaunchKernelGGL(conv3x3_pack_n_kernel, dim3((n * 2 * kPack + 255) / 256), dim3(256), 0,
                       static_cast<hipStream_t>(stream), wl, n, packed);
    return status();
}

int hrl_conv3x3_pack_n_zero(const float *const *weights, int n, float *packed, float *zero, int64_t zero_floats,
                            void *stream) {
    if (n < 1 || n > 8 || !weights || !packed || zero_floats < 0 || zero_floats > ((int64_t)1 << 36)) return HRL_EINVAL;
    if (zero_floats > 0 && (!zero || (reinterpret_cast<uintptr_t>(zero) & 3) != 0)) return HRL_EINVAL;
    WeightList wl{};
    for (int i = 0; i < n; ++i) {
        if (!weights[i]) return HRL_EINVAL;
        wl.w[i] = weights[i];
    }
    const int pack_blocks = (n * 2 * kPack + 255) / 256;
    int64_t head = 0, nvec = 0;
    if (zero_floats > 0) {
        head = (int64_t)((16 - (reinterpret_cast<uintptr_t>(zero) & 15)) & 15) / 4;
        if (head > zero_floats) head = zero_floats;
        nvec = (zero_floats - head) / 4;
    }
    const int64_t zero_blocks = zero_floats > 0 ? (nvec > 256 ? (nvec + 255) / 256 : 1) : 0;
    hipLaunchKernelGGL(conv3x3_pack_n_zero_kernel, dim3((unsigned)(pack_blocks + zero_blocks)), dim3(256), 0,
                       static_cast<hipStream_t>(stream), wl, n, packed, pack_blocks, zero, zero_floats, (int)head,
                       nvec);
    return status();
}

int hrl_conv3x3_forward(const float *x, int64_t M, int64_t C_in, int64_t C_out, const float *weight,
                        const float *bias, int flip, float *y, void *workspace, int64_t workspace_bytes,
                        void *stream) {
    if (C_in != kC || C_out != kC) return HRL_EINVAL;
    return hrl_conv3x3_forward_ex(x, M, nullptr, nullptr, weight, bias, flip, y, 0, nullptr, nullptr, nullptr,
                                  nullptr, nullptr, workspace, workspace_bytes, stream);
}

int hrl_conv3x3_wgrad_ex(const float *x, const float *in_alpha, const float *in_beta, const float *dy, int64_t M,
                         float *dweight, void *workspace, int64_t workspace_bytes, void *stream) {
    if (M < 1 || !x || !dy || !dweight || !workspace) return HRL_EINVAL;
    if ((in_alpha == nullptr) != (in_beta == nullptr)) return HRL_EINVAL;
    if (!aligned16(x) || !aligned16(dy) || workspace_bytes < hrl_conv3x3_workspace_bytes(M)) return HRL_EINVAL;
    hipStream_t s = static_cast<hipStream_t>(stream);
    const int grid = grid_for(M);
    float *partial = static_cast<float *>(workspace) + kTaps * 2 * kC * 16 * 2;
    if (g_split) {
        if (in_alpha)
            hipLaunchKernelGGL((conv3x3_wgrad_split_kernel<true>), dim3(grid), dim3(kThreads), 0, s, x, in_alpha,
                               in_beta, dy, M, partial);
        else
            hipLaunchKernelGGL((conv3x3_wgrad_split_kernel<false>), dim3(grid), dim3(kThreads), 0, s, x, in_alpha,
                               in_beta, dy, M, partial);
    } else if (in_alpha) {
        hipLaunchKernelGGL((conv3x3_wgrad_kernel<true>), dim3(grid), dim3(kThreads), 0, s, x, in_alpha, in_beta, dy,
                           M, partial);
    } else {
        hipLaunchKernelGGL((conv3x3_wgrad_kernel<false>), dim3(grid), dim3(kThreads), 0, s, x, in_alpha, in_beta,
                           dy, M, partial);
    }
    int rc = status();
    if (rc) return rc;
    hipLaunchKernelGGL(conv3x3_wgrad_reduce_kernel, dim3(kTaps * kC * kC / 64), dim3(256), 0, s, partial, grid,
                       dweight);
    return status();
}

int hrl_conv3x3_block_backward(const float *g, const float *y, int64_t M, const float *bn_weight,
                               const float *bn_bias, const float *save_mean, const float *save_invstd,
                               const float *kcoef, const float *gmean, const float *x, const float *in_alpha,
                               const float *in_beta, const float *packed_flip, float *dweight, float *gin,
                               int epilogue, const float *ep_mean, const float *ep_alpha, const float *ep_beta,
                               double *part, void *workspace, int64_t workspace_bytes, void *stream) {
    if (M < 1 || !g || !y || !save_mean || !save_invstd || !kcoef || !gmean || !x || !workspace)
        return HRL_EINVAL;
    if ((in_alpha == nullptr) != (in_beta == nullptr)) return HRL_EINVAL;
    if (workspace_bytes < hrl_conv3x3_workspace_bytes(M) || M * kRow * 4 > 0xffffffffLL) return HRL_EINVAL;
    if (gin && (!packed_flip || epilogue < 0 || epilogue == 1 || epilogue > 3)) return HRL_EINVAL;
    if (gin && epilogue == 2 && (!ep_mean || !ep_alpha || !ep_beta || !part)) return HRL_EINVAL;
    hipStream_t s = static_cast<hipStream_t>(stream);
    const int grid = grid_for(M);
    float *wpart = static_cast<float *>(workspace) + kTaps * 2 * kC * 16 * 2;
    BlockBwdArgs a{g, y, bn_weight, bn_bias, save_mean, save_invstd, kcoef, gmean, x, in_alpha, in_beta, packed_flip,
                   ep_mean, ep_alpha, ep_beta, gin, part, wpart, M};
    const bool pro = in_alpha != nullptr;
#define HRL_BLOCK_LAUNCH(PRO, EPI, DG) \
    hipLaunchKernelGGL((conv3x3_block_bwd_kernel<PRO, EPI, DG>), dim3(grid), dim3(kThreads), 0, s, a)
#define HRL_BLOCK2_LAUNCH(PRO, EPI) \
    hipLaunchKernelGGL((conv3x3_block_bwd2_kernel<PRO, EPI>), dim3(grid), dim3(bb2::kThreads), 0, s, a)
    if (!gin) {
        if (pro) HRL_BLOCK_LAUNCH(true, 0, false); else HRL_BLOCK_LAUNCH(false, 0, false);
    } else if (g_block_form == 0) {
        if (epilogue == 2) {
            if (pro) HRL_BLOCK_LAUNCH(true, 2, true); else HRL_BLOCK_LAUNCH(false, 2, true);
        } else if (epilogue == 3) {
            if (pro) HRL_BLOCK_LAUNCH(true, 3, true); else HRL_BLOCK_LAUNCH(false, 3, true);
        } else {
            if (pro) HRL_BLOCK_LAUNCH(true, 0, true); else HRL_BLOCK_LAUNCH(false, 0, true);
        }
    } else if (epilogue == 2) {
        if (pro) HRL_BLOCK2_LAUNCH(true, 2); else HRL_BLOCK2_LAUNCH(false, 2);
    } else if (epilogue == 3) {
        if (pro) HRL_BLOCK2_LAUNCH(true, 3); else HRL_BLOCK2_LAUNCH(false, 3);
    } else {
        if (pro) HRL_BLOCK2_LAUNCH(true, 0); else HRL_BLOCK2_LAUNCH(false, 0);
    }
#undef HRL_BLOCK_LAUNCH
#undef HRL_BLOCK2_LAUNCH
    int rc = status();
    if (rc || !dweight) return rc;
    hipLaunchKernelGGL(conv3x3_wgrad_reduce_kernel, dim3(kTaps * kC * kC / 64), dim3(256), 0, s, wpart, grid,
                       dweight);
    return status();
}

int hrl_conv3x3_block_backward_dz(const float *dz, const float *w1p, const float *w1v, const float *y, int64_t M,
                                  const float *bn_weight, const float *bn_bias, const float *save_mean,
                                  const float *save_invstd, const float *kcoef, const float *gmean, const float *x,
                                  const float *in_alpha, const float *in_beta, const float *packed_flip,
                                  float *dweight, float *gin, int epilogue, const float *ep_mean,
                                  const float *ep_alpha, const float *ep_beta, double *part, void *workspace,
                                  int64_t workspace_bytes, void *stream) {
    if (M < 1 || !dz || !w1p || !w1v || !y || !save_mean || !save_invstd || !kcoef || !gmean || !x || !workspace)
        return HRL_EINVAL;
    if ((in_alpha == nullptr) != (in_beta == nullptr)) return HRL_EINVAL;
    if (workspace_bytes < hrl_conv3x3_workspace_bytes(M) || M * kRow * 4 > 0xffffffffLL) return HRL_EINVAL;
    if (g_block_form != 1 || epilogue != 2 || !gin || !packed_flip) return HRL_EINVAL;
    if (!ep_mean || !ep_alpha || !ep_beta || !part) return HRL_EINVAL;
    hipStream_t s = static_cast<hipStream_t>(stream);
    const int grid = grid_for(M);
    float *wpart = static_cast<float *>(workspace) + kTaps * 2 * kC * 16 * 2;
    BlockBwdArgs a{dz, y, bn_weight, bn_bias, save_mean, save_invstd, kcoef, gmean, x, in_alpha, in_beta, packed_flip,
                   ep_mean, ep_alpha, ep_beta, gin, part, wpart, M, w1p, w1v};
    if (in_alpha)
        hipLaunchKernelGGL((conv3x3_block_bwd2_kernel<true, 2, true>), dim3(grid), dim3(bb2::kThreads), 0, s, a);
    else
        hipLaunchKernelGGL((conv3x3_block_bwd2_kernel<false, 2, true>), dim3(grid), dim3(bb2::kThreads), 0, s, a);
    int rc = status();
    if (rc || !dweight) return rc;
    hipLaunchKernelGGL(conv3x3_wgrad_reduce_kernel, dim3(kTaps * kC * kC / 64), dim3(256), 0, s, wpart, grid,
                       dweight);
    return status();
}

int64_t hrl_conv3x3_wgrad_partials(int64_t M, int64_t *offset_bytes) {
    if (M < 1) return -1;
    if (offset_bytes) *offset_bytes = (int64_t)kTaps * 2 * kC * 16 * 2 * 4;
    return grid_for(M);
}

int hrl_conv3x3_wgrad(const float *x, const float *dy, int64_t M, int64_t C_in, int64_t C_out, float *dweight,
                      void *workspace, int64_t workspace_bytes, void *stream) {
    if (C_in != kC || C_out != kC) return HRL_EINVAL;
    return hrl_conv3x3_wgrad_ex(x, nullptr, nullptr, dy, M, dweight, workspace, workspace_bytes, stream);
}

}
```

handyrl_amd/nn.py:

```python

import ctypes
import operator

import os

import torch
import torch.fx
import torch.nn as nn
import torch.nn.functional as F

from . import _native

__all__ = ['BatchNorm2d', 'BoardConv2d', 'Linear', 'accelerate', 'batch_norm_train', 'fuse_bn_relu', 'unfuse']

_MAX_ROW = 3072
_MAX_ROW_SCALAR = 1024


class DeferredGrads:

    def __init__(self):
        self.conv = {}
        self.late_params = set()
        self.affine = {}
# ... 1156 lines not shown
        g = torch.empty(N, C, H, W, device=x.device, dtype=x.dtype)
        _native.check(lib.hrl_torus_head_unpool(_native.ptr(dhead), _native.ptr(davg), _native.ptr(x), N, H, W,
                                                x.shape[1] * H * W, _native.ptr(g), _native.stream_of(x.device)),
                      'hrl_torus_head_unpool')
        return g, None


def geese_pool(h, x):
    if h.shape[1] != 32 or h.dtype != torch.float32 or x.dtype != torch.float32:
        raise RuntimeError('geese_pool: expects float32 h with 32 channels, got %s %s'
                           % (tuple(h.shape), h.dtype))
    return _GeesePool.apply(h, x)


def _board_head_spec(m):
    unit, fc = getattr(m, 'conv', None), getattr(m, 'fc', None)
    conv = getattr(unit, 'conv', None)
    if not isinstance(fc, nn.Linear) or fc.bias is not None or not isinstance(conv, nn.Conv2d):
        return None
    if getattr(unit, 'bn', 0) is not None or conv.bias is None or conv.kernel_size != (1, 1) or \
            conv.stride != (1, 1) or conv.groups != 1 or conv.padding_mode != 'zeros':
        return None
    act = getattr(m, 'activation', None)
    slope = act.negative_slope if isinstance(act, nn.LeakyReLU) else getattr(m, 'LEAKY_SLOPE', None)
    return (conv, fc) if slope == 0.1 else None


def _head_pair(model):
    pol = val = None
    for m in model.modules():
        spec = _board_head_spec(m)
        if spec is None:
            continue
        conv, fc = spec
        shape = (conv.in_channels, conv.out_channels, fc.in_features, fc.out_features)
        if shape == (32, 2, 18, 9):
            pol = m if pol is None else False
        elif shape == (32, 1, 9, 1):
            val = m if val is None else False
    return (pol, val) if pol and val else None


class _BoardHeadsFn(torch.autograd.Function):

    @staticmethod
    def forward(ctx, h, w1p, b1p, w1v, b1v, wp, wv):
        h = h.contiguous()
        N = h.shape[0]
        dev = h.device
        lib = _native.load()
        a_p = torch.empty(N, 18, device=dev, dtype=h.dtype)
        a_v = torch.empty(N, 9, device=dev, dtype=h.dtype)
        p = torch.empty(N, 9, device=dev, dtype=h.dtype)
        v = torch.empty(N, 1, device=dev, dtype=h.dtype)
        P = _native.ptr
        w1p, w1v, wp, wv = w1p.contiguous(), w1v.contiguous(), wp.contiguous(), wv.contiguous()
        _native.check(lib.hrl_heads_forward(P(h), N, P(w1p), P(b1p.contiguous()), P(w1v), P(b1v.contiguous()),
                                            P(wp), P(wv), None, None, P(a_p), P(a_v), P(p), P(v), 0,
                                            _native.stream_of(dev)), 'hrl_heads_forward')
        ctx.save_for_backward(h, w1p, w1v, wp, wv, a_p, a_v)
        ctx.biases = (b1p, b1v)
        return p, v

    @staticmethod
    def backward(ctx, dp, dv):
        h, w1p, w1v, wp, wv, a_p, a_v = ctx.saved_tensors
        N = h.shape[0]
        dev = h.device
        lib = _native.load()
        dp, dv = dp.contiguous(), dv.contiguous()
        dh = torch.empty_like(h)
        b1p, b1v = ctx.biases
        bufs = [_grad_buffer(t) for t in (w1p, b1p, w1v, b1v, wp, wv)]
        ws_bytes = lib.hrl_heads_workspace_bytes(N)
        ws = torch.empty(ws_bytes, dtype=torch.uint8, device=dev)
        P = _native.ptr

        def call(*dws):
            _native.check(lib.hrl_heads_backward(P(h), N, P(w1p), P(w1v), P(wp), P(wv), None, None, None, None,
                                                 P(a_p), P(a_v), P(dp), P(dv), None, P(dh), *(P(t) for t in dws),
                                                 P(ws), ws_bytes, _native.stream_of(dev)), 'hrl_heads_backward')
        df = _defer_folds(bufs, 6) if lib.hrl_heads_set_bwd_form(0) == 2 else None
        if df is not None:
            _heads_backward_deferred(lib, df, bufs, N, ws, call)
        else:
            call(*(b[0] for b in bufs))
        return (dh, *(_ret(b) for b in bufs))


class _FusedHeads(nn.Module):

    def __init__(self, head_p, head_v):
        super().__init__()
        object.__setattr__(self, 'head_p', head_p)
        object.__setattr__(self, 'head_v', head_v)

    def forward(self, x):
        if not (x.is_cuda and x.dtype == torch.float32 and x.dim() == 4 and tuple(x.shape[1:]) == (32, 3, 3)
                and x.shape[0] > 0):
            return self.head_p(x), self.head_v(x)
        (cp, fp), (cv, fv) = _board_head_spec(self.head_p), _board_head_spec(self.head_v)
        params = (cp.weight, cp.bias, cv.weight, cv.bias, fp.weight, fv.weight)
        if torch.is_grad_enabled() and (x.requires_grad or any(t.requires_grad for t in params)):
            return _BoardHeadsFn.apply(x, *params)
        x = x.contiguous()
        N = x.shape[0]
        p = torch.empty(N, 9, device=x.device, dtype=x.dtype)
        v = torch.empty(N, 1, device=x.device, dtype=x.dtype)
        P = _native.ptr
        _native.check(_native.load().hrl_heads_forward(P(x), N, P(cp.weight.contiguous()), P(cp.bias.contiguous()),
                                                       P(cv.weight.contiguous()), P(cv.bias.contiguous()),
                                                       P(fp.weight.contiguous()), P(fv.weight.contiguous()), None,
                                                       None, None, None, P(p), P(v), 0, _native.stream_of(x.device)),
                      'hrl_heads_forward')
        return p, v


def _fuse_heads(gm, heads):
    head_p, head_v = heads
    calls = {}
    for node in gm.graph.nodes:
        if node.op == 'call_module':
            m = gm.get_submodule(node.target)
            if m is head_p or m is head_v:
                calls.setdefault('p' if m is head_p else 'v', []).append(node)
    if len(calls.get('p', [])) != 1 or len(calls.get('v', [])) != 1:
        return 0
    np_, nv_ = calls['p'][0], calls['v'][0]
    if np_.args != nv_.args or len(np_.args) != 1 or np_.kwargs or nv_.kwargs:
        return 0
    gm.add_submodule('_hrl_heads', _FusedHeads(head_p, head_v))
    first = np_ if list(gm.graph.nodes).index(np_) < list(gm.graph.nodes).index(nv_) else nv_
    with gm.graph.inserting_before(first):
        call = gm.graph.call_module('_hrl_heads', np_.args)
        outs = [gm.graph.call_function(operator.getitem, (call, i)) for i in range(2)]
    np_.replace_all_uses_with(outs[0])
    nv_.replace_all_uses_with(outs[1])
    gm.graph.erase_node(np_)
    gm.graph.erase_node(nv_)
    return 1


class _StemConv(torch.autograd.Function):

    @staticmethod
    def forward(ctx, x, weight, bias):
        N, Cin = x.shape[0], x.shape[1]
        lib = _native.load()
        y = torch.empty(N, 32, 3, 3, device=x.device, dtype=x.dtype)
        w = weight.contiguous()
        b = bias.contiguous() if bias is not None else None
        _native.check(lib.hrl_stem_forward(_native.ptr(x), N, Cin, _native.ptr(w), _native.ptr(b), _native.ptr(y),
                                           _native.stream_of(x.device)), 'hrl_stem_forward')
        ctx.save_for_backward(x, w)
        ctx.params = (weight, bias)
        return y

    @staticmethod
    def backward(ctx, dy):
        x, w = ctx.saved_tensors
        weight, bias = ctx.params
        N, Cin = x.shape[0], x.shape[1]
        lib = _native.load()
        ws_bytes = lib.hrl_stem_workspace_bytes(N)
        ws = torch.empty(ws_bytes, dtype=torch.uint8, device=x.device)
        bw = _grad_buffer(weight)
        bb = _grad_buffer(bias) if bias is not None else (None, False)
        df = _defer_folds([bw, bb]) if lib.hrl_stem_set_wgrad_form(0) == 2 else None
        dwp, dbp = (None, None) if df is not None else (bw[0], bb[0])
        _native.check(lib.hrl_stem_wgrad(_native.ptr(x), _native.ptr(dy.contiguous()), N, Cin, _native.ptr(dwp),
                                         _native.ptr(dbp), _native.ptr(ws), ws_bytes,
                                         _native.stream_of(x.device)), 'hrl_stem_wgrad')
        if df is not None:
            row = ctypes.c_int64(0)
            nparts = lib.hrl_stem_wgrad_partials(N, ctypes.byref(row))
            part = ws.view(torch.float32)
            nw = 32 * Cin * 9
            df.add(part, row.value, 0, nparts, bw[0], nw)
            if bb[0] is not None:
                df.add(part, row.value, nw, nparts, bb[0], 32)
            df.keep.append(ws)
        return None, _ret(bw), _ret(bb)


class _BoardWeight(torch.autograd.Function):

    @staticmethod
    def forward(ctx, weight, H, W):
        Cout, Cin, kh, kw = weight.shape
        w = weight.contiguous()
        out = torch.empty(Cin * H * W, Cout * H * W, dtype=w.dtype, device=w.device)
        _native.check(_native.load().hrl_board_weight(_native.ptr(w), Cout, Cin, kh, kw, H, W, _native.ptr(out),
                                                       _native.stream_of(w.device)), 'hrl_board_weight')
        ctx.geom = (Cout, Cin, kh, kw, H, W)
        ctx.weight = weight
        return out

    @staticmethod
    def backward(ctx, grad):
        Cout, Cin, kh, kw, H, W = ctx.geom
        g = grad.contiguous()
        buf = _grad_buffer(ctx.weight)
        _native.check(_native.load().hrl_board_fold(_native.ptr(g), Cout, Cin, kh, kw, H, W, _native.ptr(buf[0]),
                                                     _native.stream_of(g.device)), 'hrl_board_fold')
        return _ret(buf), None, None


class _BoardBias(torch.autograd.Function):

    @staticmethod
    def forward(ctx, bias, HW):
        out = torch.empty(bias.shape[0] * HW, dtype=bias.dtype, device=bias.device)
        _native.check(_native.load().hrl_board_bias(_native.ptr(bias.contiguous()), bias.shape[0], HW,
                                                     _native.ptr(out), _native.stream_of(bias.device)), 'hrl_board_bias')
        ctx.shape = (bias.shape[0], HW)
        ctx.bias = bias
        return out

    @staticmethod
    def backward(ctx, grad):
        Cout, HW = ctx.shape
        g = grad.contiguous()
        buf = _grad_buffer(ctx.bias)
        _native.check(_native.load().hrl_board_bias_fold(_native.ptr(g), Cout, HW, _native.ptr(buf[0]),
                                                          _native.stream_of(g.device)), 'hrl_board_bias_fold')
        return _ret(buf), None


class _LSTMGates(torch.autograd.Function):

    @staticmethod
    def forward(ctx, zx, zh, c, save=True, bias=None, bias_rows=1, out=None):
        ctx.set_materialize_grads(False)
        N, G, Hh, Ww = zh.shape
        H, HW = G // 4, Hh * Ww
        zh = zh.contiguous()
        c = c.contiguous()
        if zx is not None and (zx.shape != zh.shape or zx.stride()[1:] != zh.stride()[1:]):
            zx = zx.contiguous()
        if out is not None:
            h_out, c_out = out
            assert not save and h_out.shape == c.shape and c_out.shape == c.shape
            assert h_out.is_contiguous() and c_out.is_contiguous()
        else:
            h_out = torch.empty_like(c)
            c_out = torch.empty_like(c)
        gates = torch.empty_like(zh) if save else None
        lib = _native.load()
        if bias is not None:
            assert zx is not None and not save and bias.is_contiguous() and bias.numel() == bias_rows * G
        _native.check(lib.hrl_lstm_gates_forward(_native.ptr(zx), 0 if zx is None else zx.stride(0), _native.ptr(zh),
                                                 _native.ptr(c), N, H, HW, _native.ptr(bias), bias_rows,
                                                 _native.ptr(h_out), _native.ptr(c_out), _native.ptr(gates),
                                                 _native.stream_of(zh.device)),
                      'hrl_lstm_gates_forward')
        ctx.save_for_backward(gates, c, c_out)
        ctx.has_zx = zx is not None
        return h_out, c_out

    @staticmethod
    def backward(ctx, dh, dc_out):
        if dh is None and dc_out is None:
            return None, None, None, None, None, None, None
        gates, c, c_out = ctx.saved_tensors
        N, G, Hh, Ww = gates.shape
        dz = torch.empty_like(gates)
        dc = torch.empty_like(c)
        dh = None if dh is None else dh.contiguous()
        dc_out = None if dc_out is None else dc_out.contiguous()
        _native.check(_native.load().hrl_lstm_gates_backward(
            _native.ptr(gates), _native.ptr(c), _native.ptr(c_out), _native.ptr(dh), _native.ptr(dc_out),
            N, G // 4, Hh * Ww, _native.ptr(dz), _native.ptr(dc), _native.stream_of(gates.device)),
            'hrl_lstm_gates_backward')
        return (dz if ctx.has_zx else None), dz, dc, None, None, None, None


def lstm_gates(zx, zh, c, bias=None, bias_rows=1, out=None):
    if not zh.is_cuda:
        raise RuntimeError('lstm_gates runs on the HIP device only (no CPU fallback)')
    save = torch.is_grad_enabled() and any(t is not None and t.requires_grad for t in (zx, zh, c))
    if (bias is not None or out is not None) and save:
        raise ValueError('lstm_gates: the folded bias and output buffers are inference-only forms')
    return _LSTMGates.apply(zx, zh, c, save, bias, bias_rows, out)


def _live(xs):
    return [k for k, x in enumerate(xs) if x is not None]


def _rows_view(t, lead):
    rows = t.flatten(lead) if t.dim() > lead else t.unsqueeze(-1)
    if rows.stride(-1) != 1:
        rows = rows.contiguous()
    rows = rows.reshape(-1, rows.shape[-1]) if lead > 1 else rows
    if rows.stride(-1) != 1 or (rows.shape[0] > 1 and rows.stride(0) < rows.shape[-1]):
        rows = rows.contiguous()
    return rows


class _HiddenGather(torch.autograd.Function):

    @staticmethod
    def forward(ctx, m, summed, B, P, *H):
        ctx.set_materialize_grads(False)
        H = [h.contiguous() for h in H]
        rows = B if summed else B * P
        outs = [torch.empty(rows, *h.shape[2:], dtype=h.dtype, device=h.device) for h in H]
        F = [h[0, 0].numel() for h in H]
        _native.check(_native.load().hrl_hidden_gather(
            _native.ptr_array(H), _native.ptr(m), B, P, len(H), _native.i64_array(F), int(summed),
            _native.ptr_array(outs), _native.stream_of(m.device)), 'hrl_hidden_gather')
        ctx.save_for_backward(m)
        ctx.meta = (summed, B, P, [tuple(h.shape) for h in H])
        return (*outs, *[h.view_as(h) for h in H])

    @staticmethod
    def backward(ctx, *grads):
        (m,) = ctx.saved_tensors
        summed, B, P, shapes = ctx.meta
        n = len(shapes)
        gout, galias = grads[:n], grads[n:]
        dH = [None] * n
        live = [k for k in range(n) if gout[k] is not None]
        for k in range(n):
            if gout[k] is None and galias[k] is not None:
                dH[k] = galias[k]
        if live:
            g = [gout[k].contiguous() for k in live]
            F = [int(torch.Size(shapes[k][2:]).numel()) for k in live]
            add = [None if galias[k] is None else _rows_view(galias[k], 2) for k in live]
            d = [torch.empty(shapes[k], dtype=m.dtype, device=m.device) for k in live]
            _native.check(_native.load().hrl_hidden_gather_backward_add(
                _native.ptr_array(g), _native.ptr(m), B, P, len(live), _native.i64_array(F), int(summed),
                _native.ptr_array(add) if any(a is not None for a in add) else None,
                _native.i64_array([a.stride(-2) if a is not None else f for a, f in zip(add, F)]),
# ... 66 lines not shown

    @staticmethod
    def forward(ctx, m, m_next, summed, B, P, Pn, n, out_k, *tensors):
        ctx.set_materialize_grads(False)
        H = [h.contiguous() for h in tensors[:n]]
        nh = [x.contiguous() for x in tensors[n:]]
        outs = [torch.empty_like(h) for h in H]
        rows = B if summed else B * P
        gath = [torch.empty(rows, *h.shape[2:], dtype=h.dtype, device=h.device) for h in H]
        F = [h[0, 0].numel() for h in H]
        _native.check(_native.load().hrl_hidden_update_gather(
            _native.ptr_array(H), _native.ptr_array(nh), Pn, _native.ptr(m), _native.ptr(m_next), B, P, n,
            _native.i64_array(F), int(summed), _native.ptr_array(outs), _native.ptr_array(gath),
            _native.stream_of(m.device)), 'hrl_hidden_update_gather')
        ctx.save_for_backward(m, m_next)
        ctx.meta = (summed, B, P, Pn, n, out_k, [tuple(h.shape) for h in H], [tuple(x.shape) for x in nh])
        res = (*gath, *[o.view_as(o) for o in outs])
        if out_k >= 0:
            res = res + (tensors[n + out_k].view_as(tensors[n + out_k]),)
        return res

    @staticmethod
    def backward(ctx, *grads):
        m, m_next = ctx.saved_tensors
        summed, B, P, Pn, n, out_k, h_shapes, nh_shapes = ctx.meta
        ggath, gstate = grads[:n], grads[n:2 * n]
        gk = grads[2 * n] if out_k >= 0 else None
        dH, dnh = [None] * n, [None] * n
        live = [k for k in range(n) if ggath[k] is not None or gstate[k] is not None]
        if gk is not None and out_k not in live:
            dnh[out_k] = gk
        if live:
            g = [None if ggath[k] is None else ggath[k].contiguous() for k in live]
            st = [None if gstate[k] is None else _rows_view(gstate[k], 2) for k in live]
            add = [_rows_view(gk, 1) if (k == out_k and gk is not None) else None for k in live]
            F = [int(torch.Size(h_shapes[k][2:]).numel()) for k in live]
            a = [torch.empty(h_shapes[k], dtype=m.dtype, device=m.device) for k in live]
            b = [torch.empty(nh_shapes[k], dtype=m.dtype, device=m.device) for k in live]
            _native.check(_native.load().hrl_hidden_update_gather_backward(
                _native.ptr_array(g), _native.ptr(m), _native.ptr(m_next), B, P, Pn, len(live), _native.i64_array(F),
                int(summed), _native.ptr_array(st) if any(x is not None for x in st) else None,
                _native.i64_array([x.stride(-2) if x is not None else f for x, f in zip(st, F)]),
                _native.ptr_array(add) if any(x is not None for x in add) else None,
                _native.i64_array([x.stride(-2) if x is not None else f for x, f in zip(add, F)]),
                _native.ptr_array(a), _native.ptr_array(b), _native.stream_of(m.device)),
                'hrl_hidden_update_gather_backward')
            for k, x, y in zip(live, a, b):
                dH[k], dnh[k] = x, y
        return (None, None, None, None, None, None, None, None, *dH, *dnh)


def _board_conv_ok(m):
    k = m.kernel_size
    return (m.stride == (1, 1) and m.dilation == (1, 1) and m.groups == 1 and m.padding_mode == 'zeros'
            and isinstance(m.padding, tuple) and m.padding == (k[0] // 2, k[1] // 2) and k[0] % 2 == 1
            and k[1] % 2 == 1)


class BatchNorm2d(nn.BatchNorm2d):

    fused_relu = False

    def forward(self, x):
        row = x.shape[1] * x.shape[2] * x.shape[3] if x.dim() == 4 else 0
        shape_ok = (x.is_cuda and x.dtype == torch.float32 and x.dim() == 4
                    and x.shape[0] > 0 and (row <= _MAX_ROW_SCALAR or (row % 4 == 0 and row <= _MAX_ROW)))
        if shape_ok and not self.training and self.track_running_stats and self.running_mean is not None:
            return batch_norm_eval(x, self.weight, self.bias, self.running_mean, self.running_var, self.eps,
                                   self.fused_relu)
        use_hip = shape_ok and self.training
        if not use_hip:
            y = super().forward(x)
            return torch.relu(y) if self.fused_relu else y
        self._check_input_dim(x)
        momentum = 0.0 if self.momentum is None else self.momentum
        if self.track_running_stats and self.num_batches_tracked is not None:
            self.num_batches_tracked.add_(1)
            if self.momentum is None:
                momentum = 1.0 / float(self.num_batches_tracked.item())
        rm = self.running_mean if self.track_running_stats else None
        rv = self.running_var if self.track_running_stats else None
        return batch_norm_train(x, self.weight, self.bias, rm, rv, momentum, self.eps, self.fused_relu)


def accelerate(model):
    for name, child in list(model.named_children()):
        if type(child) is nn.Conv2d and _board_conv_ok(child):
            new = BoardConv2d(child.in_channels, child.out_channels, child.kernel_size, stride=1,
                              padding=child.padding, bias=child.bias is not None,
                              device=child.weight.device, dtype=child.weight.dtype)
            new.weight = child.weight
            if child.bias is not None:
                new.bias = child.bias
            new.train(child.training)
            setattr(model, name, new)
        elif type(child) is nn.Linear:
            new = Linear(child.in_features, child.out_features, bias=child.bias is not None,
                         device=child.weight.device, dtype=child.weight.dtype)
            new.weight = child.weight
            if child.bias is not None:
                new.bias = child.bias
            new.train(child.training)
            setattr(model, name, new)
        elif type(child) is nn.BatchNorm2d:
            new = BatchNorm2d(child.num_features, eps=child.eps, momentum=child.momentum,
                              affine=child.affine, track_running_stats=child.track_running_stats)
            new.weight, new.bias = child.weight, child.bias
            if child.track_running_stats:
                new.running_mean, new.running_var = child.running_mean, child.running_var
                new.num_batches_tracked = child.num_batches_tracked
            new.train(child.training)
            setattr(model, name, new)
        else:
            accelerate(child)
    if hasattr(model, 'use_hip'):
        model.use_hip = True
    return model


class _MultiBoardConv(nn.Module):

    def __init__(self, convs):
        super().__init__()
        object.__setattr__(self, 'convs', list(convs))

    def forward(self, x):
        convs = self.convs
        if not (x.is_cuda and x.dim() == 4 and x.dtype == torch.float32
                and x.shape[2] * x.shape[3] <= BOARD_MAX_CELLS):
            return tuple(c(x) for c in convs)
        N, Cin, H, W = x.shape
        HW = H * W
        wb = torch.cat([_BoardWeight.apply(c.weight, H, W) for c in convs], dim=1)
        parts = [_BoardBias.apply(c.bias, HW) if c.bias is not None else c.weight.new_zeros(c.out_channels * HW)
                 for c in convs]
        y = _RowMatmul.apply(x.reshape(N, Cin * HW), wb, torch.cat(parts))
        outs, off = [], 0
        for c in convs:
            n = c.out_channels * HW
            outs.append(y[:, off:off + n].reshape(N, c.out_channels, H, W))
            off += n
        return tuple(outs)


_UNIT = {}

def _unit_coefs(dev):
    u = _UNIT.get(dev)
    if u is None:
        u = _UNIT[dev] = torch.stack([torch.ones(32, device=dev), torch.zeros(32, device=dev)])
    return u


def _chain_forward(h0, meta, relu_in, params, apply_out=True):
    lib = _native.load()
    M = h0.shape[0]
    dev = h0.device
    stream = _native.stream_of(dev)
    P = _native.ptr
    ws_bytes = lib.hrl_conv3x3_workspace_bytes(M)
    ws = torch.empty(ws_bytes, dtype=torch.uint8, device=dev)
    nblk = lib.hrl_conv3x3_stats_blocks(M)
    part = torch.empty(nblk * 32 * 2, dtype=torch.float64, device=dev)
    unit = _unit_coefs(dev) if relu_in else None
    x = h0
    a_prev, b_prev = (unit[0], unit[1]) if relu_in else (None, None)
    ys, coefs = [], []
    weights = [params[3 * i].contiguous() for i in range(len(meta))]
    packed = torch.empty(len(weights), 2, 9216, dtype=torch.float32, device=dev)
    for k in range(0, len(weights), 8):
        zero = take_zero(dev)
        if zero is not None:
            _native.check(lib.hrl_conv3x3_pack_n_zero(_native.ptr_array(weights[k:k + 8]), len(weights[k:k + 8]),
                                                      P(packed[k]), P(zero), zero.numel(), stream),
                          'hrl_conv3x3_pack_n_zero')
            continue
        _native.check(lib.hrl_conv3x3_pack_n(_native.ptr_array(weights[k:k + 8]), len(weights[k:k + 8]),
                                             P(packed[k]), stream), 'hrl_conv3x3_pack_n')
    for i, (rm, rv, momentum, eps) in enumerate(meta):
        w, gamma, beta = params[3 * i:3 * i + 3]
        y = torch.empty_like(h0)
        _native.check(lib.hrl_conv3x3_forward_ex(P(x), M, P(a_prev), P(b_prev), P(packed[i, 0]), None, 2, P(y),
                                                 1, None, None, None, None, P(part), P(ws), ws_bytes, stream),
                      'hrl_conv3x3_forward_ex')
        coef = torch.empty(4, 32, dtype=torch.float32, device=dev)
        _native.check(lib.hrl_bn_finalize_stats(P(part), nblk, 32, M * 9, P(gamma), P(beta), P(rm), P(rv),
                                                float(momentum), float(eps), P(coef[0]), P(coef[1]),
                                                P(coef[2]), P(coef[3]), stream), 'hrl_bn_finalize_stats')
        ys.append(y)
        coefs.append(coef)
        x, a_prev, b_prev = y, coef[2], coef[3]
    out = None
    if apply_out:
        out = torch.empty_like(h0)
        _native.check(lib.hrl_bn_apply(P(x), M, 32, 9, P(a_prev), P(b_prev), 1, P(out), stream), 'hrl_bn_apply')
    return out, ys, coefs, unit, packed


HEADS_DZ = True


def _heads_dz_ok(lib, n):
    return HEADS_DZ and n >= 2 and lib.hrl_heads_set_bwd_form(0) == 2 and _block_form(lib) == 1


def _block_form(lib):
    form = lib.hrl_conv3x3_set_block_form(1)
    lib.hrl_conv3x3_set_block_form(form)
    return form


def _chain_backward(h0, ys, coefs, unit, params, relu_in, g, need_input_grad, packed, part_in=None, nblk_in=0,
                    heads_dz=None):
    lib = _native.load()
    n = len(ys)
    M = h0.shape[0]
    dev = h0.device
    stream = _native.stream_of(dev)
    P = _native.ptr
    ws_bytes = lib.hrl_conv3x3_workspace_bytes(M)
    ws = torch.empty(ws_bytes, dtype=torch.uint8, device=dev)
    bn_ws_bytes = lib.hrl_bn_workspace_bytes(M, 32, 9)
    bn_ws = torch.empty(bn_ws_bytes, dtype=torch.uint8, device=dev)
    nblk = lib.hrl_conv3x3_block_sum_blocks(M)
    part = torch.empty(nblk * 32 * 2, dtype=torch.float64, device=dev)
    g = g.contiguous()
    assert heads_dz is None or (part_in is not None and n >= 2)
    grads = [None] * (3 * n)
    sums, sums_n = (part_in, nblk_in) if part_in is not None else (None, 0)
    for i in reversed(range(n)):
        w, gamma, beta = params[3 * i:3 * i + 3]
        mean, invstd = coefs[i][0], coefs[i][1]
        bw, bgam, bbet = _grad_buffer(w), _grad_buffer(gamma), _grad_buffer(beta)
        dgam, dbet = bgam[0], bbet[0]
        if i == 0:
            x, a, b = h0, (unit[0] if unit is not None else None), (unit[1] if unit is not None else None)
        else:
            x, a, b = ys[i - 1], coefs[i - 1][2], coefs[i - 1][3]
        dw = bw[0]
        if sums is not None:
            kg = torch.empty(2, 32, dtype=torch.float32, device=dev)
            _native.check(lib.hrl_bn_finalize_backward(P(sums), sums_n, 32, M * 9, P(gamma), P(invstd),
                                                       P(dgam), P(dbet), P(kg[0]), P(kg[1]), stream),
                          'hrl_bn_finalize_backward')
            gin, epi, ep = None, 0, (None, None, None)
            if i > 0:
                gin, epi, ep = torch.empty_like(h0), 2, (coefs[i - 1][0], coefs[i - 1][2], coefs[i - 1][3])
            elif need_input_grad:
                gin, epi = torch.empty_like(h0), (3 if relu_in else 0)
            df = _defer_folds([bw])
            wsb = ws if df is None else torch.empty(ws_bytes, dtype=torch.uint8, device=dev)
            ev = _block_timing_start()
            if heads_dz is not None and i == n - 1:
                _native.check(lib.hrl_conv3x3_block_backward_dz(
                    P(g), P(heads_dz[0]), P(heads_dz[1]), P(ys[i]), M, P(gamma), P(beta), P(mean), P(invstd),
                    P(kg[0]), P(kg[1]), P(x), P(a), P(b), P(packed[i, 1]), None if df is not None else P(dw), P(gin),
                    epi, P(ep[0]), P(ep[1]), P(ep[2]), P(part), P(wsb), ws_bytes, stream),
                    'hrl_conv3x3_block_backward_dz')
            else:
                _native.check(lib.hrl_conv3x3_block_backward(
                    P(g), P(ys[i]), M, P(gamma), P(beta), P(mean), P(invstd), P(kg[0]), P(kg[1]), P(x), P(a), P(b),
                    P(packed[i, 1]), None if df is not None else P(dw), P(gin), epi, P(ep[0]), P(ep[1]), P(ep[2]),
                    P(part) if i > 0 else None, P(wsb), ws_bytes, stream), 'hrl_conv3x3_block_backward')
            _block_timing_end(ev)
            if df is not None:
                off = ctypes.c_int64(0)
                nparts = lib.hrl_conv3x3_wgrad_partials(M, ctypes.byref(off))
                df.add(wsb[off.value:].view(torch.float32), 9216, 0, nparts, dw, 9216, mode=1)
                df.keep.append(wsb)
            grads[3 * i:3 * i + 3] = [_ret(bw), _ret(bgam), _ret(bbet)]
            g = gin
            if i > 0:
                sums, sums_n = part, lib.hrl_conv3x3_block_sum_blocks(M)
            continue
        dy = torch.empty_like(h0)
        _native.check(lib.hrl_bn_backward(P(ys[i]), P(g), M, 32, 9, P(gamma), P(beta), P(mean), P(invstd),
                                          1, P(dy), P(dgam), P(dbet), P(bn_ws), bn_ws_bytes, stream),
                      'hrl_bn_backward')
        _native.check(lib.hrl_conv3x3_wgrad_ex(P(x), P(a), P(b), P(dy), M, P(dw), P(ws), ws_bytes, stream),
                      'hrl_conv3x3_wgrad_ex')
        grads[3 * i:3 * i + 3] = [_ret(bw), _ret(bgam), _ret(bbet)]
        if i > 0:
            g = torch.empty_like(h0)
            _native.check(lib.hrl_conv3x3_forward_ex(P(dy), M, None, None, P(packed[i, 1]), None, 3, P(g), 2,
                                                     P(ys[i - 1]),
                                                     P(coefs[i - 1][0]), P(coefs[i - 1][2]),
                                                     P(coefs[i - 1][3]), P(part), P(ws), ws_bytes, stream),
                          'hrl_conv3x3_forward_ex(flip, bn sums)')
            sums, sums_n = part, lib.hrl_conv3x3_stats_blocks(M)
        elif need_input_grad:
            g = torch.empty_like(h0)
            _native.check(lib.hrl_conv3x3_forward_ex(P(dy), M, None, None, P(packed[i, 1]), None, 3, P(g),
                                                     3 if relu_in else 0, P(h0) if relu_in else None,
                                                     None, None, None, None, P(ws), ws_bytes, stream),
                          'hrl_conv3x3_forward_ex(flip)')
        else:
            g = None
    return g, grads


class _BoardChain(torch.autograd.Function):

    @staticmethod
    def forward(ctx, h0, meta, relu_in, *params):
        h0 = h0.contiguous()
        out, ys, coefs, unit, packed = _chain_forward(h0, meta, relu_in, params)
        ctx.save_for_backward(h0, *ys, *coefs, packed, *params)
        ctx.n = len(meta)
        ctx.relu_in = relu_in
        return out

    @staticmethod
    def backward(ctx, g):
        n = ctx.n
        t = ctx.saved_tensors
        h0, ys, coefs, packed, params = t[0], list(t[1:1 + n]), list(t[1 + n:1 + 2 * n]), t[1 + 2 * n], t[2 + 2 * n:]
        unit = _unit_coefs(h0.device) if ctx.relu_in else None
        g_in, grads = _chain_backward(h0, ys, coefs, unit, params, ctx.relu_in, g, ctx.needs_input_grad[0], packed)
        return (g_in, None, None, *grads)


class _ChainHeadsFn(torch.autograd.Function):

    @staticmethod
    def forward(ctx, h0, meta, relu_in, tanh_v, w1p, b1p, w1v, b1v, wp, wv, *params):
        h0 = h0.contiguous()
        _, ys, coefs, unit, packed = _chain_forward(h0, meta, relu_in, params, apply_out=False)
        y, coef = ys[-1], coefs[-1]
        N = h0.shape[0]
        dev = h0.device
        lib = _native.load()
        a_p = torch.empty(N, 18, device=dev, dtype=h0.dtype)
        a_v = torch.empty(N, 9, device=dev, dtype=h0.dtype)
        p = torch.empty(N, 9, device=dev, dtype=h0.dtype)
        v = torch.empty(N, 1, device=dev, dtype=h0.dtype)
        P = _native.ptr
        w1p, w1v, wp, wv = w1p.contiguous(), w1v.contiguous(), wp.contiguous(), wv.contiguous()
        _native.check(lib.hrl_heads_forward(P(y), N, P(w1p), P(b1p.contiguous()), P(w1v), P(b1v.contiguous()),
                                            P(wp), P(wv), P(coef[2]), P(coef[3]), P(a_p), P(a_v), P(p), P(v),
                                            int(tanh_v), _native.stream_of(dev)), 'hrl_heads_forward(bn)')
        ctx.save_for_backward(h0, *ys, *coefs, a_p, a_v, w1p, w1v, wp, wv, packed, v, *params)
        ctx.tanh_v = tanh_v
        ctx.biases = (b1p, b1v)
        ctx.n = len(meta)
        ctx.relu_in = relu_in
        return p, v

    @staticmethod
    def backward(ctx, dp, dv):
        n = ctx.n
        t = ctx.saved_tensors
        h0, ys, coefs = t[0], list(t[1:1 + n]), list(t[1 + n:1 + 2 * n])
        a_p, a_v, w1p, w1v, wp, wv, packed, v = t[1 + 2 * n:9 + 2 * n]
        params = t[9 + 2 * n:]
        b1p, b1v = ctx.biases
        N = h0.shape[0]
        dev = h0.device
        lib = _native.load()
        P = _native.ptr
        y, coef = ys[-1], coefs[-1]
        dp, dv = dp.contiguous(), dv.contiguous()
        use_dz = _heads_dz_ok(lib, n)
        dh = torch.empty(N, 28, device=dev, dtype=h0.dtype) if use_dz else torch.empty_like(h0)
        heads_backward = lib.hrl_heads_backward_dz if use_dz else lib.hrl_heads_backward
        hbufs = [_grad_buffer(x) for x in (w1p, b1p, w1v, b1v, wp, wv)]
        ws_bytes = lib.hrl_heads_workspace_bytes(N)
        ws = torch.empty(ws_bytes, dtype=torch.uint8, device=dev)
        nparts = lib.hrl_heads_bn_parts(N)
        bn_part = torch.empty(nparts * 64, dtype=torch.float64, device=dev)
        def call(*dws):
            _native.check(heads_backward(P(y), N, P(w1p), P(w1v), P(wp), P(wv), P(coef[2]), P(coef[3]),
                                         P(coef[0]), P(bn_part), P(a_p), P(a_v), P(dp), P(dv),
                                         P(v) if ctx.tanh_v else None, P(dh), *(P(t) for t in dws),
                                         P(ws), ws_bytes, _native.stream_of(dev)), 'hrl_heads_backward(bn)')
        df = _defer_folds(hbufs, 6) if lib.hrl_heads_set_bwd_form(0) == 2 else None
        if df is not None:
            _heads_backward_deferred(lib, df, hbufs, N, ws, call)
        else:
            call(*(b[0] for b in hbufs))
        unit = _unit_coefs(dev) if ctx.relu_in else None
        g_in, grads = _chain_backward(h0, ys, coefs, unit, params, ctx.relu_in, dh, ctx.needs_input_grad[0], packed,
                                      part_in=bn_part, nblk_in=nparts, heads_dz=(w1p, w1v) if use_dz else None)
        return (g_in, None, None, None, *(_ret(b) for b in hbufs), *grads)


class _ConvBNChain(nn.Module):

    def __init__(self, convs, bns, relu_in=False):
        super().__init__()
        object.__setattr__(self, 'convs', list(convs))
        object.__setattr__(self, 'bns', list(bns))
        self.relu_in = relu_in

    @staticmethod
    def layers_ok(convs, bns):
        return all(type(c) is BoardConv2d and c.bias is None and tuple(c.weight.shape) == (32, 32, 3, 3)
                   and _board_conv_ok(c) for c in convs) and \
            all(isinstance(b, BatchNorm2d) and b.affine and b.track_running_stats and b.momentum is not None
                and b.num_features == 32 for b in bns)

    def forward(self, x):
        convs, bns = self.convs, self.bns
        if not self.fused_ok(x):
            if self.relu_in:
                x = torch.relu(x)
            for c, b in zip(convs, bns):
                x = b(c(x))
            return x
        meta, params = self.meta_params()
        return _BoardChain.apply(x, meta, self.relu_in, *params)

    def fused_ok(self, x):
        return (x.is_cuda and x.dtype == torch.float32 and x.dim() == 4 and tuple(x.shape[1:]) == (32, 3, 3)
                and x.shape[0] > 0 and all(b.training and b.fused_relu for b in self.bns)
                and torch.is_grad_enabled())

    def meta_params(self):
        counters = [b.num_batches_tracked for b in self.bns]
        if not _defer_counters(counters):
            torch._foreach_add_(counters, 1)
        meta, params = [], []
        for c, b in zip(self.convs, self.bns):
            meta.append((b.running_mean, b.running_var, b.momentum, b.eps))
            params += [c.weight, b.weight, b.bias]
        return meta, params


class _ChainHeads(nn.Module):

    def __init__(self, chain, heads):
        super().__init__()
        object.__setattr__(self, 'chain', chain)
        object.__setattr__(self, 'heads', heads)
        self.tanh_v = False

    def forward(self, x):
        if not self.chain.fused_ok(x):
            p, v = self.heads(self.chain(x))
            return p, (torch.tanh(v) if self.tanh_v else v)
        (cp, fp), (cv, fv) = _board_head_spec(self.heads.head_p), _board_head_spec(self.heads.head_v)
        meta, params = self.chain.meta_params()
        return _ChainHeadsFn.apply(x, meta, self.chain.relu_in, self.tanh_v, cp.weight, cp.bias, cv.weight, cv.bias,
                                   fp.weight, fv.weight, *params)


def _fuse_chain_heads(gm):
    for node in list(gm.graph.nodes):
        if node.op != 'call_module' or not isinstance(gm.get_submodule(node.target), _FusedHeads):
            continue
        src = node.args[0] if len(node.args) == 1 else None
        if not (isinstance(src, torch.fx.Node) and src.op == 'call_module'
                and isinstance(gm.get_submodule(src.target), _ConvBNChain) and len(src.users) == 1):
            return 0
        fused = _ChainHeads(gm.get_submodule(src.target), gm.get_submodule(node.target))
        gm.add_submodule('_hrl_chain_heads', fused)
        with gm.graph.inserting_before(src):
            call = gm.graph.call_module('_hrl_chain_heads', src.args)
        node.replace_all_uses_with(call)
        gm.graph.erase_node(node)
        gm.graph.erase_node(src)
        for item in list(call.users):
            if item.op == 'call_function' and item.target is operator.getitem and item.args[1] == 1 \
                    and len(item.users) == 1:
                user = next(iter(item.users))
                if _is_tanh(user, item):
                    user.replace_all_uses_with(item)
                    gm.graph.erase_node(user)
                    fused.tanh_v = True
        return 1
    return 0


class _LeafTracer(torch.fx.Tracer):

    def __init__(self, leaves=()):
        super().__init__()
        self.extra = set(id(m) for m in leaves)

    def is_leaf_module(self, m, qualname):
        return isinstance(m, (BatchNorm2d, BoardConv2d, Linear, _MultiBoardConv, _ConvBNChain)) or \
            id(m) in self.extra or super().is_leaf_module(m, qualname)


def _is_tanh(node, arg):
    if node.op == 'call_function' and node.target in (torch.tanh, torch.nn.functional.tanh):
        return node.args == (arg,) and not node.kwargs
    if node.op == 'call_method' and node.target == 'tanh':
        return node.args == (arg,) and not node.kwargs
    return False


def _is_relu(gm, node):
    if node.op == 'call_function' and node.target in (torch.relu, torch.nn.functional.relu):
        return len(node.args) == 1
    if node.op == 'call_method' and node.target == 'relu':
        return len(node.args) == 1
    if node.op == 'call_module':
        return isinstance(gm.get_submodule(node.target), nn.ReLU)
    return False


def fuse_bn_relu(model, example=None):
    if hasattr(model, 'init_hidden') or 'forward' in model.__dict__:
        return 0
    try:
        heads = _head_pair(model)
        graph = _LeafTracer(leaves=heads or ()).trace(model)
    except Exception:
        return 0
    gm = torch.fx.GraphModule(model, graph)
    pairs = []
    for node in gm.graph.nodes:
        if node.op == 'call_module' and isinstance(gm.get_submodule(node.target), BatchNorm2d):
            users = list(node.users)
            if len(users) == 1 and _is_relu(gm, users[0]) and users[0].args[0] is node:
                pairs.append((node, users[0]))
    for bn_node, relu_node in pairs:
        relu_node.replace_all_uses_with(bn_node)
        gm.graph.erase_node(relu_node)
    bns = [gm.get_submodule(n.target) for n, _ in pairs]
    chains = _fuse_chains(gm, set(n for n, _ in pairs))
    merged = 0
    for node in list(gm.graph.nodes):
        sibs = [u for u in node.users if u.op == 'call_module' and type(gm.get_submodule(u.target)) is BoardConv2d
                and u.args == (node,) and not u.kwargs]
        if len(sibs) < 2:
            continue
        name = '_hrl_multiconv%d' % merged
        gm.add_submodule(name, _MultiBoardConv([gm.get_submodule(u.target) for u in sibs]))
        with gm.graph.inserting_after(node):
            multi = gm.graph.call_module(name, (node,))
        anchor = multi
        for i, u in enumerate(sibs):
            with gm.graph.inserting_after(anchor):
                item = gm.graph.call_function(operator.getitem, (multi, i))
            u.replace_all_uses_with(item)
            gm.graph.erase_node(u)
            anchor = item
        merged += 1
    fused_heads = _fuse_heads(gm, heads) if heads else 0
    if fused_heads:
        fused_heads += _fuse_chain_heads(gm)
    if not pairs and not merged and not fused_heads:
        return 0
    gm.graph.lint()
    gm.recompile()
    if example is not None:
        was = model.training
        model.eval()
        with torch.no_grad():
            ref = model(example, None)
            for bn in bns:
                bn.fused_relu = True
            new = gm(example, None)
        model.train(was)
        same = _same_outputs(ref, new, rtol=1e-4, atol=1e-5)
        if same and chains and example.is_cuda:
            same = _same_training_outputs(model, gm, bns, example)
        if not same:
            for bn in bns:
                bn.fused_relu = False
            return 0
    for bn in bns:
        bn.fused_relu = True
    model.forward = gm.forward
    object.__setattr__(model, '_hrl_graph', gm)
    return len(pairs) + merged + chains + fused_heads


def _same_outputs(ref, new, rtol=1e-5, atol=1e-6):
    return set(ref) == set(new) and all(
        torch.allclose(ref[k], new[k], rtol=rtol, atol=atol) for k in ref if ref[k] is not None)


def _same_training_outputs(model, gm, bns, example):
    buffers = [(b.running_mean.clone(), b.running_var.clone(), b.num_batches_tracked.clone()) for b in bns]

    def restore():
        for b, (m, v, n) in zip(bns, buffers):
            b.running_mean.copy_(m)
            b.running_var.copy_(v)
            b.num_batches_tracked.copy_(n)
    was = model.training
    model.train()
    try:
        for bn in bns:
            bn.fused_relu = False
        ref = model(example, None)
        restore()
        for bn in bns:
            bn.fused_relu = True
        new = gm(example, None)
        restore()
    finally:
        model.train(was)
    ref = {k: v.detach() for k, v in ref.items() if v is not None}
    new = {k: v.detach() for k, v in new.items() if v is not None}
    return _same_outputs(ref, new, rtol=1e-4, atol=1e-5)


def _fuse_chains(gm, fused_bn_nodes):
    def conv_bn(node):
        if node.op != 'call_module' or type(gm.get_submodule(node.target)) is not BoardConv2d or node.kwargs:
            return None
        users = list(node.users)
        if len(users) != 1 or users[0] not in fused_bn_nodes or users[0].args != (node,):
            return None
        return users[0]

    chains, seen = [], set()
    for node in list(gm.graph.nodes):
        if node in seen:
            continue
        bn = conv_bn(node)
        if bn is None:
            continue
        links = [(node, bn)]
        while True:
            users = list(links[-1][1].users)
            if len(users) != 1:
                break
            nxt = conv_bn(users[0])
            if nxt is None:
                break
            links.append((users[0], nxt))
        convs = [gm.get_submodule(c.target) for c, _ in links]
        bns = [gm.get_submodule(b.target) for _, b in links]
        if not _ConvBNChain.layers_ok(convs, bns):
            continue
        for c, b in links:
            seen.update((c, b))
        chains.append((links, convs, bns))
    for k, (links, convs, bns) in enumerate(chains):
        name = '_hrl_chain%d' % k
        first, last = links[0][0], links[-1][1]
        src = first.args[0]
        relu_in = (isinstance(src, torch.fx.Node) and _is_relu(gm, src) and len(src.users) == 1
                   and src.op != 'call_module')
        gm.add_submodule(name, _ConvBNChain(convs, bns, relu_in=relu_in))
        with gm.graph.inserting_before(first):
            call = gm.graph.call_module(name, (src.args[0],) if relu_in else first.args)
        last.replace_all_uses_with(call)
        for c, b in reversed(links):
            gm.graph.erase_node(b)
            gm.graph.erase_node(c)
        if relu_in:
            gm.graph.erase_node(src)
    return len(chains)


def unfuse(model):
    if 'forward' in model.__dict__:
        del model.forward
    model.__dict__.pop('_hrl_graph', None)
    for m in model.modules():
        if isinstance(m, BatchNorm2d):
            m.fused_relu = False
    return model
```

handyrl_amd/trainer.py:

```python

import contextlib
import copy

import torch
import torch.nn as nn

from . import distributed as hdist
from . import nn as hnn
from .nn import accelerate, fuse_bn_relu, deferred_weight_grads, deferred_folds, direct_grads
from .train import backward_total, forward_prediction, loss_terms
from .util import map_r, bimap_r

DEFAULT_LR = 3e-8


class StepTail:

    def __init__(self, grads, lr, weight_decay=1e-5, betas=(0.9, 0.999), eps=1e-8, max_norm=4.0):
        from . import _native
        self.lib = _native.load()
        self.grads = grads
        flat = grads.flat
        dev = flat.device
        n = flat.numel()
# ... 269 lines not shown
            return self.tail.state_tensors() + ([self.stats] if self._tail_stats else [])
        return [v for st in self.optimizer.state.values() for v in st.values() if isinstance(v, torch.Tensor)]

    def _body(self, batch, hidden):
        losses, dcnt = self._grads(batch, hidden)
        if self.reducer is not None:
            self.reducer.finish()
        return self._update(losses, dcnt)

    def _accumulate(self, out):
        if self._tail_stats:
            self.batches += 1
            return
        vec = torch.stack([out[k].reshape(()) for k in sorted(out)])
        if self.stats is None:
            self.stats_keys = sorted(out)
            self.stats = torch.zeros_like(vec)
            self.batches = 0
        self.stats += vec
        self.batches += 1

    def step(self, batch, hidden=None):
        if self.graph:
            if self._graph is None:
                self._capture(batch, hidden)
            else:
                if not _same_tensors(batch, self._static):
                    self.load_batch(batch)
                if hidden is not None and hidden is not self._static_hidden:
                    bimap_r(self._static_hidden, hidden, lambda dst, src: dst.copy_(src, non_blocking=True))
            self._graph.replay()
            if self._graph_update is not None:
                if self._graph_seg2 is not None:
                    works = [self.reducer.all_reduce_ranges(self.segments[0][0])]
                    self._graph_seg2.replay()
                    works.append(self.reducer.all_reduce_ranges(self.segments[1][0]))
                    for w in works:
                        for x in w:
                            x.wait()
                else:
                    self.reducer.all_reduce_flat()
                self._graph_update.replay()
            out = self._static_out
        else:
            out = self._body(batch, hidden)
        self._accumulate(out)
        return out

    def _capture(self, batch, hidden):
        self._static = batch
        self._static_hidden = hidden
        params = list(self.net.parameters())
        saved_p = [p.detach().clone() for p in params]
        saved_b = [b.detach().clone() for b in self.net.buffers()]
        side = torch.cuda.Stream(self.device)
        side.wait_stream(torch.cuda.current_stream(self.device))
        with torch.cuda.stream(side):
            for _ in range(3):
                self._body(batch, hidden)
            if self.reducer is not None and hidden is None and self.segment_backward:
                self._try_plan_segments(batch)
            elif self.reducer is not None and hidden is not None and self.defer and self.segment_backward:
                self._plan_flush_segments()
        torch.cuda.current_stream(self.device).wait_stream(side)
        with torch.no_grad():
            for p, v in zip(params, saved_p):
                p.copy_(v)
            for b, v in zip(self.net.buffers(), saved_b):
                b.copy_(v)
            for v in self._opt_state():
                v.zero_()
        if self.reducer is None:
            self._graph = torch.cuda.CUDAGraph()
            with torch.cuda.graph(self._graph):
                self._static_out = self._body(batch, hidden)
            return
        torch.cuda.synchronize(self.device)
        self.reducer.enabled = False
        seg2 = None
        try:
            grads_graph, update_graph = torch.cuda.CUDAGraph(), torch.cuda.CUDAGraph()
            if self.segments is not None and hidden is not None:
                seg2 = torch.cuda.CUDAGraph()
                with torch.cuda.graph(grads_graph, capture_error_mode='thread_local'):
                    self.grads.zero()
                    with deferred_weight_grads() as deferred:
                        outputs = forward_prediction(self.net, hidden, batch, self.args)
                        losses, dcnt = self.loss_fn(outputs, batch, self.args)
                        backward_total(losses)
                    deferred.flush(phase=1)
                with torch.cuda.graph(seg2, capture_error_mode='thread_local'):
                    deferred.flush(phase=2)
            elif self.segments is not None:
                seg2 = torch.cuda.CUDAGraph()
                with self._cut_hook():
                    with direct_grads():
                        with torch.cuda.graph(grads_graph, capture_error_mode='thread_local'):
                            self.grads.zero()
                            outputs = forward_prediction(self.net, hidden, batch, self.args)
                            losses, dcnt = self.loss_fn(outputs, batch, self.args)
                            cut, upper, lower = self._cut, self.segments[0][1], self.segments[1][1]
                            backward_total(losses, inputs=[cut] + upper, retain_graph=True)
                        with torch.cuda.graph(seg2, capture_error_mode='thread_local'):
                            torch.autograd.backward(cut, grad_tensors=cut.grad, inputs=lower)
            else:
                with torch.cuda.graph(grads_graph, capture_error_mode='thread_local'):
                    losses, dcnt = self._grads(batch, hidden)
            with torch.cuda.graph(update_graph, capture_error_mode='thread_local'):
                self._static_out = self._update(losses, dcnt)
        finally:
            self.reducer.enabled = True
            self.reducer.reset()
        self._graph, self._graph_update, self._graph_seg2 = grads_graph, update_graph, seg2

    @contextlib.contextmanager
    def _cut_hook(self):
        from . import nn as hnn
        mod = self._cut_module()
        handle = mod.register_forward_pre_hook(self._grab_cut) if mod is not None else None
        prev = hnn._CUT_FN
        if mod is None:
            hnn._CUT_FN = self._grab_cut_tensor
        try:
            yield
        finally:
            if handle is not None:
                handle.remove()
            hnn._CUT_FN = prev
            self._cut = None

    def _has_cut_site(self):
        if self._cut_module() is not None:
            return True
        return any(getattr(m, 'tower_split', None) for m in self.net.modules())

    def _grab_cut_tensor(self, t):
        cut = t.view_as(t)
        self._cut = cut
        return cut

    def _cut_module(self):
        from .nn import _ChainHeads, _ConvBNChain
        gm = getattr(self.net, '_hrl_graph', None)
        if gm is None:
            return None
        for node in gm.graph.nodes:
            if node.op == 'call_module':
                m = gm.get_submodule(node.target)
                if isinstance(m, (_ChainHeads, _ConvBNChain)):
                    return m
        return None

    def _grab_cut(self, _module, args):
        cut = args[0].view_as(args[0])
        self._cut = cut
        return (cut,) + tuple(args[1:])

    def _try_plan_segments(self, batch):
        if not self._has_cut_site():
            self.segment_error = 'no fused conv chain or split torus tower in the net'
            return
        try:
            with self._cut_hook(), direct_grads():
                outputs = forward_prediction(self.net, None, batch, self.args)
                losses, _ = self.loss_fn(outputs, batch, self.args)
                self._plan_segments(losses['total'])
        except RuntimeError as e:
            self.segments = None
            self.segment_error = str(e)
            split_torus_tower(self.net, False)

    def _plan_flush_segments(self):
        late = [p for p, l in zip(self.params, self.live) if l and id(p) in self._late_ids]
        early = [p for p, l in zip(self.params, self.live) if l and id(p) not in self._late_ids]
        if not late or not early:
            self.segments = None
            self.segment_error = 'no late (recurrent-cell) weight records in the unroll'
            return
        self.segments = [(self._ranges(early), early), (self._ranges(late), late)]

    def _ranges(self, ps):
        index = {id(p): i for i, p in enumerate(self.params)}
        out = []
        for off, n in sorted(self.grads.slices[index[id(p)]] for p in ps):
            if out and out[-1][1] == off:
                out[-1][1] = off + n
            else:
                out.append([off, off + n])
        return [tuple(r) for r in out]

    def _plan_segments(self, loss):
        cut = self._cut
        if cut is None or not cut.requires_grad or cut.grad_fn is None:
            raise RuntimeError('segmented capture: the chain input was not seen or does not require grad')

        def reach(root, stop):
            seen, params, todo = set(), set(), [root]
            while todo:
                fn = todo.pop()
                if fn is None or fn in seen or fn is stop:
                    continue
                seen.add(fn)
                var = getattr(fn, 'variable', None)
                if var is not None:
                    params.add(id(var))
                todo.extend(f for f, _ in fn.next_functions)
            return params
        up = reach(loss.grad_fn, cut.grad_fn)
        low = reach(cut.grad_fn, None)
        live = self.live or [True] * len(self.params)
        upper = [p for p, l in zip(self.params, live) if l and id(p) in up]
        lower = [p for p, l in zip(self.params, live) if l and id(p) in low]
        if set(map(id, upper)) & set(map(id, lower)) or len(upper) + len(lower) != sum(live):
            raise RuntimeError('segmented capture: parameters shared across the cut')
        self.segments = [(self._ranges(upper), upper), (self._ranges(lower), lower)]
        return cut, upper, lower

    def load_batch(self, batch):
        for k, v in batch.items():
            dst = self._static[k]
            if isinstance(v, dict):
                for kk, vv in v.items():
                    dst[kk].copy_(vv, non_blocking=True)
            else:
                dst.copy_(v, non_blocking=True)

    def pop_stats(self):
        if self.stats is None or self.batches == 0:
            return {}, 0
        vals = self.stats
        if self.reducer is not None:
            vals = hdist.all_reduce_sum_([vals.clone()], self.reducer.group)[0]
        vals = vals.tolist()
        res = dict(zip(self.stats_keys, vals))
        n = self.batches
        if self._tail_stats:
            self.stats.zero_()
            self.batches = 0
        else:
            self.stats = None
        return res, n


class Trainer:

    def __init__(self, args, model, batcher, device=None, graph=False, world_size=1, group=None, loss_fn=None):
        self.args = args
        self.model = model
        self.batcher = batcher
        self.device = device or torch.device('cuda', torch.cuda.current_device())
        self.default_lr = DEFAULT_LR
        self.data_cnt_ema = args['batch_size'] * world_size * args['forward_steps']
        self.steps = 0
        self.update_flag = False
        self.shutdown_flag = False
        self.learner = LearnerStep(model, args, self.device, lr=self.default_lr * self.data_cnt_ema,
                                   graph=graph, reduce_group=group, world_size=world_size, loss_fn=loss_fn)

    def _to_device(self, batch):
        return map_r(batch, lambda x: x.to(self.device, non_blocking=True) if x is not None else None)

    def train(self, max_steps=None):
        self.model.train()
        n = 0
        while (n == 0 or not (self.update_flag or self.shutdown_flag)) and (max_steps is None or n < max_steps):
            batch = self._to_device(self.batcher.batch())
            B, P = batch['value'].size(0), batch['value'].size(2)
            hidden = self.model.init_hidden([B, P]) if hasattr(self.model, 'init_hidden') else None
            if hidden is not None:
                hidden = self._to_device(hidden)
            self.learner.step(batch, hidden)
            n += 1
            self.steps += 1
        sums, batch_cnt = self.learner.pop_stats()
        data_cnt = sums.pop('dcnt', 0.0)
        sums.pop('grad_norm', None)
        print('loss = %s' % ' '.join('%s:%.3f' % (k, v / max(data_cnt, 1e-9)) for k, v in sums.items()))
        self.data_cnt_ema = self.data_cnt_ema * 0.8 + data_cnt / (1e-2 + batch_cnt) * 0.2
        self.lr = self.default_lr * self.data_cnt_ema / (1 + self.steps * 1e-5)
        self.learner.set_lr(self.lr)
        model = copy.deepcopy(self.model).cpu()
        model.eval()
        return model


def clip_grad_norm_reference(params, max_norm=4.0):
    return nn.utils.clip_grad_norm_(params, max_norm)
```

include/hrl_nn.h:

```cpp
#ifndef HRL_NN_H
#define HRL_NN_H

#include <stdint.h>

#ifdef __cplusplus
extern "C" {
#endif

int64_t hrl_bn_workspace_bytes(int64_t N, int64_t C, int64_t HW);

int hrl_bn_forward_train(const float *x, int64_t N, int64_t C, int64_t HW,
                         const float *weight, const float *bias,
                         float *running_mean, float *running_var, double momentum, double eps, int relu,
                         float *y, float *save_mean, float *save_invstd,
                         void *workspace, int64_t workspace_bytes, void *stream);

int hrl_bn_backward(const float *x, const float *dy, int64_t N, int64_t C, int64_t HW,
                    const float *weight, const float *bias, const float *save_mean, const float *save_invstd,
                    int relu, float *dx, float *dweight, float *dbias,
                    void *workspace, int64_t workspace_bytes, void *stream);

int hrl_bn_finalize_stats(const double *part, int64_t nparts, int64_t C, int64_t count, const float *weight,
                          const float *bias, float *running_mean, float *running_var, double momentum, double eps,
                          float *save_mean, float *save_invstd, float *alpha, float *beta, void *stream);
int hrl_bn_apply(const float *x, int64_t N, int64_t C, int64_t HW, const float *alpha, const float *beta, int relu,
                 float *y, void *stream);
int hrl_bn_forward_eval(const float *x, int64_t N, int64_t C, int64_t HW, const float *weight, const float *bias,
                        const float *running_mean, const float *running_var, double eps, int relu, float *y,
                        float *coef, void *stream);
int64_t hrl_bn_workspace_bytes_grouped(int64_t N, int64_t C, int64_t HW, int64_t G);
int hrl_bn_forward_train_grouped(const float *x, int64_t N, int64_t C, int64_t HW, int64_t G, const float *weight,
                                 const float *bias, float *running_mean, float *running_var, double momentum,
                                 double eps, int relu, float *y, float *save_mean, float *save_invstd,
                                 void *workspace, int64_t workspace_bytes, void *stream);
int hrl_bn_backward_grouped(const float *x, const float *dy, int64_t N, int64_t C, int64_t HW, int64_t G,
                            const float *weight, const float *bias, const float *save_mean, const float *save_invstd,
                            int relu, float *dx, float *dweight, float *dbias, void *workspace,
                            int64_t workspace_bytes, void *stream);
int hrl_bn_finalize_backward(const double *part, int64_t nparts, int64_t C, int64_t count, const float *weight,
                             const float *save_invstd, float *dweight, float *dbias, float *kcoef, float *gmean,
                             void *stream);
int hrl_bn_backward_apply(const float *x, const float *dy, int64_t N, int64_t C, int64_t HW, const float *weight,
                          const float *bias, const float *save_mean, const float *save_invstd, int relu,
                          const float *kcoef, const float *gmean, float *dx, void *stream);

int hrl_bn_apply_residual(const float *x, const float *res, int64_t N, int64_t C, int64_t HW, const float *alpha,
                          const float *beta, float *y, void *stream);
int hrl_bn_backward_masked(const float *x, const float *dy, const float *out, int64_t N, int64_t C, int64_t HW,
                           const float *weight, const float *save_mean, const float *save_invstd, float *dx,
                           float *dweight, float *dbias, void *workspace, int64_t workspace_bytes, void *stream);
int hrl_bn_backward_masked_coefs(const float *x, const float *dy, const float *out, int64_t N, int64_t C,
                                 int64_t HW, const float *weight, const float *save_mean, const float *save_invstd,
                                 float *kcoef, float *gmean, float *dweight, float *dbias, void *workspace,
                                 int64_t workspace_bytes, void *stream);
int hrl_bn_backward_apply_masked(const float *x, const float *dy, const float *out, int64_t N, int64_t C, int64_t HW,
                                 const float *weight, const float *save_mean, const float *save_invstd,
                                 const float *kcoef, const float *gmean, float *dx, void *stream);

int hrl_board_weight(const float *w, int64_t Cout, int64_t Cin, int64_t kh, int64_t kw, int64_t H, int64_t W,
                     float *w_board, void *stream);
int hrl_board_fold(const float *g_board, int64_t Cout, int64_t Cin, int64_t kh, int64_t kw, int64_t H, int64_t W,
                   float *g_w, void *stream);
int hrl_board_bias(const float *b, int64_t Cout, int64_t HW, float *b_board, void *stream);
int hrl_board_bias_fold(const float *g_board, int64_t Cout, int64_t HW, float *g_b, void *stream);

int64_t hrl_colsum_workspace_bytes(int64_t M, int64_t N);
int hrl_colsum(const float *x, int64_t M, int64_t N, float *out, void *workspace, int64_t workspace_bytes,
               void *stream);

int64_t hrl_conv3x3_workspace_bytes(int64_t M);
int hrl_conv3x3_forward(const float *x, int64_t M, int64_t C_in, int64_t C_out, const float *weight,
                        const float *bias, int flip, float *y, void *workspace, int64_t workspace_bytes,
                        void *stream);
int hrl_conv3x3_wgrad(const float *x, const float *dy, int64_t M, int64_t C_in, int64_t C_out, float *dweight,
                      void *workspace, int64_t workspace_bytes, void *stream);

int64_t hrl_conv3x3_stats_blocks(int64_t M);
int hrl_conv3x3_set_split(int on);
int hrl_conv3x3_set_block_form(int form);
int64_t hrl_conv3x3_block_sum_blocks(int64_t M);
int hrl_conv3x3_set_fwd_form(int form);
int hrl_conv3x3_pack_n(const float *const *weights, int n, float *packed, void *stream);
int hrl_conv3x3_pack_n_zero(const float *const *weights, int n, float *packed, float *zero, int64_t zero_floats,
                            void *stream);
int hrl_conv3x3_forward_ex(const float *x, int64_t M, const float *in_alpha, const float *in_beta,
                           const float *weight, const float *bias, int flip, float *y, int epilogue,
                           const float *ref, const float *ep_mean, const float *ep_alpha, const float *ep_beta,
                           double *part, void *workspace, int64_t workspace_bytes, void *stream);
int hrl_conv3x3_wgrad_ex(const float *x, const float *in_alpha, const float *in_beta, const float *dy, int64_t M,
                         float *dweight, void *workspace, int64_t workspace_bytes, void *stream);

int64_t hrl_conv3x3_wgrad_partials(int64_t M, int64_t *offset_bytes);
int hrl_conv3x3_block_backward(const float *g, const float *y, int64_t M, const float *bn_weight,
                               const float *bn_bias, const float *save_mean, const float *save_invstd,
                               const float *kcoef, const float *gmean, const float *x, const float *in_alpha,
                               const float *in_beta, const float *packed_flip, float *dweight, float *gin,
                               int epilogue, const float *ep_mean, const float *ep_alpha, const float *ep_beta,
                               double *part, void *workspace, int64_t workspace_bytes, void *stream);
int hrl_conv3x3_block_backward_dz(const float *dz, const float *w1p, const float *w1v, const float *y, int64_t M,
                                  const float *bn_weight, const float *bn_bias, const float *save_mean,
                                  const float *save_invstd, const float *kcoef, const float *gmean, const float *x,
                                  const float *in_alpha, const float *in_beta, const float *packed_flip,
                                  float *dweight, float *gin, int epilogue, const float *ep_mean,
                                  const float *ep_alpha, const float *ep_beta, double *part, void *workspace,
                                  int64_t workspace_bytes, void *stream);

int hrl_lstm_gates_forward(const float *zx, int64_t zx_stride, const float *zh, const float *c, int64_t N, int64_t H,
                           int64_t HW, const float *bias, int64_t bias_rows, float *h_out, float *c_out, float *gates,
                           void *stream);
int hrl_lstm_gates_forward_grouped(int L, const float *zh, int64_t zh_stride, const float *const *zx,
                                   const int64_t *zx_strides, const float *const *c, int64_t N, int64_t H, int64_t HW,
                                   float *const *h_out, float *const *c_out, float *const *gates, void *stream);
int hrl_lstm_gates_backward_ex(const float *gates, const float *c, const float *c_out, const float *dh,
                               int64_t dh_stride, int dh_parts, int64_t dh_part_stride, const float *dc_out,
                               int64_t N, int64_t H, int64_t HW, float *dz, float *dc, float *dzx, int dzx_init,
                               void *stream);
int hrl_lstm_gates_backward(const float *gates, const float *c, const float *c_out, const float *dh,
                            const float *dc_out, int64_t N, int64_t H, int64_t HW, float *dz, float *dc,
                            void *stream);

int hrl_hidden_gather(const float *const *H, const float *mask, int64_t B, int64_t P, int nleaves, const int64_t *F,
                      int sum, float *const *out, void *stream);
int hrl_hidden_gather_backward(const float *const *dout, const float *mask, int64_t B, int64_t P, int nleaves,
                               const int64_t *F, int sum, float *const *dH, void *stream);
int hrl_hidden_update(const float *const *H, const float *const *nh, int64_t Pn, const float *mask, int64_t B,
                      int64_t P, int nleaves, const int64_t *F, float *const *out, void *stream);
int hrl_hidden_update_backward(const float *const *dout, const float *mask, int64_t B, int64_t P, int64_t Pn,
                               int nleaves, const int64_t *F, float *const *dH, float *const *dnh, void *stream);
int hrl_hidden_gather_backward_add(const float *const *dout, const float *mask, int64_t B, int64_t P, int nleaves,
                                   const int64_t *F, int sum, const float *const *addend,
                                   const int64_t *addend_strides, float *const *dH, void *stream);
int hrl_hidden_update_backward_add(const float *const *dout, const float *mask, int64_t B, int64_t P, int64_t Pn,
                                   int nleaves, const int64_t *F, const float *const *addend,
                                   const int64_t *addend_strides, float *const *dH, float *const *dnh,
                                   void *stream);
int hrl_hidden_update_gather(const float *const *H, const float *const *nh, int64_t Pn, const float *mask,
                             const float *mask_next, int64_t B, int64_t P, int nleaves, const int64_t *F, int sum,
                             float *const *out, float *const *gathered, void *stream);
int hrl_hidden_update_gather_backward(const float *const *dgathered, const float *mask, const float *mask_next,
                                      int64_t B, int64_t P, int64_t Pn, int nleaves, const int64_t *F, int sum,
                                      const float *const *dstate, const int64_t *dstate_strides,
                                      const float *const *dout_add, const int64_t *dout_add_strides,
                                      float *const *dH, float *const *dnh, void *stream);

int64_t hrl_torus_workspace_bytes(int64_t N);
int hrl_torus_set_split(int on);
int hrl_torus_set_form(int form);
int64_t hrl_torus_stats_blocks(int64_t N);
int hrl_torus_conv_forward(const float *x, int64_t N, int64_t Cin, int64_t Cout, int64_t H, int64_t W,
                           const float *weight, const float *bias, int flip, float *y, double *part,
                           const float *add, const float *add_mask, void *workspace, int64_t workspace_bytes,
                           void *stream);
int hrl_torus_conv_wgrad(const float *x, const float *dy, int64_t N, int64_t Cin, int64_t Cout, int64_t H, int64_t W,
                         float *dweight, float *dbias, void *workspace, int64_t workspace_bytes, void *stream);
int hrl_torus_conv_wgrad_bn(const float *x, int64_t N, int64_t Cin, int64_t H, int64_t W, const float *y,
                            const float *g, const float *alpha, const float *beta, int residual, const float *gamma,
                            const float *save_mean, const float *save_invstd, const float *kcoef, const float *gmean,
                            float *dy, float *dweight, float *dbias, void *workspace, int64_t workspace_bytes,
                            void *stream);

int hrl_torus_unit_forward(const float *y_prev, const float *res, const float *alpha, const float *beta, float *h,
                           int64_t N, int64_t H, int64_t W, const float *weight, const float *bias, float *y,
                           double *part, void *workspace, int64_t workspace_bytes, void *stream);
int64_t hrl_board_conv_workspace_bytes(int64_t Cout);
int hrl_board_conv_forward(const float *x, int64_t N, int64_t Cin, int64_t H, int64_t W, const float *weight,
                           int64_t w_cin_total, int64_t w_ci0, int64_t Cout, const float *bias, float *y,
                           void *workspace, int64_t workspace_bytes, void *stream);
int hrl_board_conv_pack(const float *weight, int64_t w_cin_total, int64_t w_ci0, int64_t Cout, void *packed,
                        int64_t packed_bytes, void *stream);
int hrl_board_conv_forward_packed(const float *x, int64_t N, int64_t Cin, int64_t H, int64_t W, const void *packed,
                                  int64_t Cout, const float *bias, float *y, void *stream);

int64_t hrl_gboard_pack_bytes(int64_t Cout, int64_t Cin_g);
int hrl_gboard_pack(const float *weight, int64_t Cout, int64_t Cin_g, int64_t w_cin_total, int64_t w_ci0,
                    void *packed, int64_t packed_bytes, void *stream);
int hrl_gboard_pack_adjoint(const float *weight, int64_t Cout_fwd, int64_t w_cin_total, int64_t w_ci0,
                            int64_t Cin_slice, void *packed, int64_t packed_bytes, void *stream);
int64_t hrl_gboard_wgrad_workspace_bytes(int64_t Cout, int64_t Cin, int64_t total_games);
int hrl_gboard_wgrad(const float *const *xs, const int64_t *x_strides, const float *const *dys,
                     const int64_t *dy_strides, const int64_t *ns, int nseg, int64_t Cout, int64_t Cin,
                     float *dweight, int64_t w_cin_total, int64_t w_ci0, float *dbias, void *workspace,
                     int64_t workspace_bytes, void *stream);
int hrl_gboard_set_whole_ring(int on);
int hrl_gboard_set_nctw(int nctw);
int hrl_gboard_launch_stats(int64_t *counts, int n, int reset);
int64_t hrl_gboard_pointwise_wgrad_workspace_bytes(int64_t C, int64_t O, int64_t N);
int hrl_gboard_pointwise_wgrad(const float *x, int64_t x_stride, const float *dy, int64_t dy_stride, int64_t N,
                               int64_t C, int64_t O, float *dweight, void *workspace, int64_t workspace_bytes,
                               void *stream);
int hrl_gboard_forward_groups(const float *const *xs, const int64_t *x_strides, int64_t N, int64_t Cin_g,
                              int64_t groups, const void *packed, int64_t packed_bytes, int64_t Cout, float *y,
                              int64_t y_stride, void *stream);
int hrl_gboard_forward(const float *x, int64_t x_stride, const float *x2, int64_t x2_stride, int64_t N, int64_t Cin_g,
                       int64_t groups, const void *packed, int64_t packed_bytes, int64_t Cout, const float *bias,
                       const float *alpha, const float *beta, int relu, float *y, int64_t y_stride, void *stream);

int hrl_gboard_pointwise(const float *x1, int64_t x1_stride, int64_t C1, const float *x2, int64_t x2_stride,
                          int64_t C2, int64_t N, const float *weight, int64_t O, const float *alpha, const float *beta,
                          int relu, float *y, int64_t y_stride, void *stream);

int hrl_torus_head_pool(const float *h, const float *x, int64_t N, int64_t H, int64_t W, int64_t x_stride,
                        float *head, float *avg, void *stream);
int hrl_torus_head_unpool(const float *dhead, const float *davg, const float *x, int64_t N, int64_t H, int64_t W,
                          int64_t x_stride, float *g, void *stream);
int hrl_torus_unit_input_grad(const float *dy, int64_t N, int64_t H, int64_t W, const float *weight, const float *g,
                              const float *out, float *dh, const float *h_mask, const float *y_prev,
                              const float *mean_prev, double *part, void *workspace, int64_t workspace_bytes,
                              void *stream);

int64_t hrl_heads_workspace_bytes(int64_t N);
int64_t hrl_heads_bn_parts(int64_t N);
int hrl_heads_forward(const float *h, int64_t N, const float *w1p, const float *b1p, const float *w1v,
                      const float *b1v, const float *wp, const float *wv, const float *bn_alpha, const float *bn_beta,
                      float *a_p, float *a_v, float *p_out, float *v_out, int tanh_v, void *stream);
int hrl_heads_set_bwd_form(int form);
int hrl_heads_backward(const float *h, int64_t N, const float *w1p, const float *w1v, const float *wp,
                       const float *wv, const float *bn_alpha, const float *bn_beta, const float *bn_mean,
                       double *bn_part, const float *a_p, const float *a_v, const float *dp, const float *dv,
                       const float *v_tanh, float *dh, float *dw1p, float *db1p, float *dw1v, float *db1v, float *dwp, float *dwv,
                       void *workspace, int64_t workspace_bytes, void *stream);
int hrl_heads_backward_dz(const float *h, int64_t N, const float *w1p, const float *w1v, const float *wp,
                          const float *wv, const float *bn_alpha, const float *bn_beta, const float *bn_mean,
                          double *bn_part, const float *a_p, const float *a_v, const float *dp, const float *dv,
                          const float *v_tanh, float *dz, float *dw1p, float *db1p, float *dw1v, float *db1v,
                          float *dwp, float *dwv, void *workspace, int64_t workspace_bytes, void *stream);

int64_t hrl_stem_workspace_bytes(int64_t N);
int hrl_stem_forward(const float *x, int64_t N, int64_t Cin, const float *weight, const float *bias, float *y,
                     void *stream);
int hrl_stem_wgrad(const float *x, const float *dy, int64_t N, int64_t Cin, float *dweight, float *dbias,
                   void *workspace, int64_t workspace_bytes, void *stream);
int64_t hrl_stem_wgrad_partials(int64_t N, int64_t *row_floats);
int hrl_stem_set_wgrad_form(int form);
int hrl_stem_set_fwd_form(int form);

int64_t hrl_grad_fold_norm_blocks(int64_t n);
int hrl_grad_fold_norm(float *grads, int64_t n, const float *const *parts, const int64_t *strides,
                       const int64_t *col0, const int64_t *nparts, const int64_t *dst, const int64_t *count,
                       const int *modes, int nfolds, float *step, int64_t *const *counters,
                       const int64_t *increments, int ncounters, double *norm_part, int64_t norm_part_bytes,
                       void *stream);
int hrl_grad_fold_norm_ex(float *grads, int64_t n, const float *const *parts, const int64_t *strides,
                          const int64_t *col0, const int64_t *nparts, const int64_t *dst, const int64_t *count,
                          const int *modes, int nfolds, float *step, int64_t *const *counters,
                          const int64_t *increments, int ncounters, double *norm_part, int64_t norm_part_bytes,
                          const double *loss_part, int64_t loss_nparts, double ent_coef, float *losses,
                          void *stream);
int hrl_adam_clip(float *grads, int64_t n, const double *norm_part, double max_norm, float *total_norm,
                  float *const *params, const int64_t *offsets, const int *live, int ntensors, float *exp_avg,
                  float *exp_avg_sq, const float *lr, const float *step, double beta1, double beta2, double eps,
                  double weight_decay, const float *const *acc_src, int nacc, float *acc_dst, void *stream);

int hrl_clip_grad_norm(float *grads, int64_t n, double max_norm, float *total_norm, void *stream);
int64_t hrl_clip_workspace_bytes(int64_t n);
int hrl_clip_grad_norm_ws(float *grads, int64_t n, double max_norm, float *total_norm, void *workspace,
                          int64_t workspace_bytes, void *stream);

#ifdef __cplusplus
// ... 5 lines not shown
```

Before: 134.4 million env-steps/s.

## Fuse stem 3x3 conv into first residual-chain block forward and backward

Removes the separate stem convolution by recomputing its output inside the first chain block's forward and backward kernels. The kernels read the small observation tile and the stem weights into LDS and rebuild the 32-channel activations on the fly. This avoids writing and re-reading the stem activation tensor and saves separate kernel launches. The cost is extra recompute per tile and more LDS per block, plus a more complex FX fusion path with fallbacks.

```diff
diff --git a/handyrl_amd/_native.py b/handyrl_amd/_native.py
--- a/handyrl_amd/_native.py
+++ b/handyrl_amd/_native.py
@@ -109,6 +109,11 @@
                                                      _f32p, _f32p, _f32p, _f32p, _f32p, _f32p, _f32p, _f32p,
                                                      ctypes.c_int, _f32p, _f32p, _f32p, ctypes.c_void_p,
                                                      ctypes.c_void_p, _i64, ctypes.c_void_p]),
+    'hrl_conv3x3_forward_stem': (ctypes.c_int, [_f32p, _i64, _i64, _f32p, _f32p, _f32p, _f32p, ctypes.c_void_p,
+                                                ctypes.c_void_p, _i64, ctypes.c_void_p]),
+    'hrl_conv3x3_block_backward_stem': (ctypes.c_int, [_f32p, _f32p, _i64, _f32p, _f32p, _f32p, _f32p, _f32p, _f32p,
+                                                       _f32p, _i64, _f32p, _f32p, _f32p, _f32p, _f32p,
+                                                       ctypes.c_void_p, _i64, ctypes.c_void_p]),
     'hrl_conv3x3_wgrad_ex': (ctypes.c_int, [_f32p, _f32p, _f32p, _f32p, _i64, _f32p, ctypes.c_void_p, _i64,
                                             ctypes.c_void_p]),
     'hrl_hidden_gather': (ctypes.c_int, [ctypes.c_void_p, _f32p, _i64, _i64, ctypes.c_int, ctypes.c_void_p,
diff --git a/handyrl_amd/csrc/hrl_conv.hip b/handyrl_amd/csrc/hrl_conv.hip
--- a/handyrl_amd/csrc/hrl_conv.hip
+++ b/handyrl_amd/csrc/hrl_conv.hip
@@ -562,6 +562,8 @@
     float *wpart;
     int64_t M;
     const float *w1p = nullptr, *w1v = nullptr;
+    const float *obs = nullptr, *stem_w = nullptr, *stem_b = nullptr;
+    int cin = 0;
 };
 
 typedef unsigned int u32x3 __attribute__((ext_vector_type(3)));
@@ -828,6 +830,77 @@
     HRL_STAMP_WALL(15);
 }
 
+namespace stemx {
+
+constexpr int kKMax = 27;
+constexpr int kObBytes = kKMax * kTile * 4;
+constexpr int kWtBytes = (kKMax + 1) * kC * 4;
+constexpr int kBytes = 2 * kObBytes + kWtBytes;
+static_assert(kKMax * kTile <= 7 * 64, "a dword per lane of waves 0..6");
+
+typedef float f32x2 __attribute__((ext_vector_type(2)));
+
+__device__ __forceinline__ void fill_table(float *wt, const float *w, const float *b, int cin, int tid) {
+    const int K = cin * kCells;
+    for (int i = tid; i < (kKMax + 1) * kC; i += 512) {
+        const int k = i / kC, c = i - k * kC;
+        float v = 0.f;
+        if (k < K) v = w[c * K + k];
+        else if (k == kKMax && b) v = b[c];
+        wt[i] = v;
+    }
+}
+
+__device__ __forceinline__ int slot_off(int d, int cin) {
+    const int K = cin * kCells;
+    const int row = d / K, k = d - row * K;
+    return d < kTile * K ? k * kTile + row : -1;
+}
+
+template <int W> struct Map {
+    static constexpr int kC0 = W < 4 ? 0 : 5, kNc = W < 4 ? 5 : 4;
+    static __device__ __forceinline__ int rho0(int ch, int hh) { return 2 * ((2 * (W & 3) + hh + (ch >> 2)) & 7); }
+};
+
+template <int C0, int NC>
+__device__ __forceinline__ void taps(const float (&w)[kTaps], const f32x2 (&x)[kCells], f32x2 (&acc)[5]) {
+#pragma unroll
+    for (int i = 0; i < NC; ++i)
+#pragma unroll
+        for (int p = 0; p < kCells; ++p) {
+            const int t = tap_of(p, C0 + i);
+            if (t < 0) continue;
+            acc[i] = __builtin_elementwise_fma((f32x2){w[t], w[t]}, x[p], acc[i]);
+        }
+}
+
+template <int C0, int NC>
+__device__ __forceinline__ void rebuild(const float *wt, const float *ob, int cin, int ch, int rho0, int rows,
+                                        float (&X)[2][5]) {
+    const float b = wt[kKMax * kC + ch];
+    f32x2 acc[5];
+#pragma unroll
+    for (int i = 0; i < 5; ++i) acc[i] = (f32x2){b, b};
+#pragma unroll 1
+    for (int ci = 0; ci < cin; ++ci) {
+        float w[kTaps];
+        f32x2 x[kCells];
+#pragma unroll
+        for (int t = 0; t < kTaps; ++t) w[t] = wt[(ci * kTaps + t) * kC + ch];
+#pragma unroll
+        for (int p = 0; p < kCells; ++p) x[p] = *reinterpret_cast<const f32x2 *>(ob + (ci * kCells + p) * kTile + rho0);
+        taps<C0, NC>(w, x, acc);
+    }
+    const bool v0 = rho0 < rows, v1 = rho0 + 1 < rows;
+#pragma unroll
+    for (int i = 0; i < NC; ++i) {
+        X[0][i] = v0 ? acc[i].x : 0.f;
+        X[1][i] = v1 ? acc[i].y : 0.f;
+    }
+}
+
+}
+
 namespace bb2 {
 
 constexpr int kWaves = 8;
@@ -847,6 +920,10 @@
 constexpr int kLdsBytesDz = kDz0 + 2 * kDzBytes;
 static_assert(kLdsBytesDz <= 160 * 1024, "LDS");
 static_assert(kDzBytes / 4 <= 7 * 64, "a dword per lane of waves 0..6");
+constexpr int kOb0 = kLdsBytes;
+constexpr int kWt0 = kOb0 + 2 * stemx::kObBytes;
+constexpr int kLdsBytesStem = kLdsBytes + stemx::kBytes;
+static_assert(kLdsBytesStem <= 160 * 1024, "LDS");
 
 typedef short v4s __attribute__((ext_vector_type(4)));
 typedef __attribute__((address_space(3))) v4s lds_v4s;
@@ -915,9 +992,10 @@
 #define BB2_STAMP(it, k) do { } while (0)
 #endif
 
-template <bool PRO, int EPI, int W, bool DZ = false>
+template <bool PRO, int EPI, int W, bool DZ = false, bool STEM = false>
 __device__ __forceinline__ void run(const BlockBwdArgs &a, unsigned char *smem, int lane) {
     static_assert(!DZ || EPI == 2, "the dz form is the last chain block's");
+    static_assert(!STEM || (EPI == 3 && PRO && !DZ), "the stem form is block 0's, behind the stem's ReLU");
     using R = Role<W>;
     constexpr bool kIg = R::kIg;
     constexpr int kNq = R::kNq > 0 ? R::kNq : 1;
@@ -934,7 +1012,7 @@
         be = (a.bn_b ? a.bn_b[ch] : 0.0f) - mu * al;
     }
     float pa = 1.f, pb = 0.f;
-    if constexpr (PRO) {
+    if constexpr (PRO && !STEM) {
         pa = a.in_alpha[ch];
         pb = a.in_beta[ch];
     }
@@ -1003,7 +1081,7 @@
         for (int r = 0; r < 2; ++r) {
             const int off = ldoff + r * kRow * 4;
 #pragma unroll
-            for (int k = kFwd ? 2 : (DZ ? 1 : 0); k < 3; ++k) {
+            for (int k = kFwd ? 2 : (DZ ? 1 : 0); k < (STEM ? 2 : 3); ++k) {
                 const __amdgpu_buffer_rsrc_t rs = k == 0 ? rg : (k == 1 ? ry : rx);
                 float(&d)[5] = k == 0 ? G[r] : (k == 1 ? Y[r] : X[r]);
                 const u32x3 v = __builtin_amdgcn_raw_buffer_load_b96(rs, off, 0, 0);
@@ -1033,9 +1111,53 @@
             reinterpret_cast<float *>(smem + kDz0 + (it & 1) * kDzBytes)[W * 64 + lane] = v;
     };
     float DZv = 0.f;
+    const int ob_off = STEM && W < 7 ? stemx::slot_off(W * 64 + lane, a.cin) : -1;
+    auto load_ob = [&](int it) __attribute__((always_inline)) {
+        float v = 0.f;
+        if constexpr (STEM && W < 7) {
+            const int K = a.cin * kCells;
+            const int64_t t = t0 + (int64_t)it * step;
+            const bool ok = it < n_iter;
+            const int rows = ok ? (int)min<int64_t>(kTile, a.M - t * kTile) : 0;
+            const __amdgpu_buffer_rsrc_t ro = wave_rsrc(a.obs + (ok ? t * kTile * K : 0), (uint32_t)(rows * K * 4));
+            v = __uint_as_float(__builtin_amdgcn_raw_buffer_load_b32(ro, (W * 64 + lane) * 4, 0, 0));
+        }
+        return v;
+    };
+    auto put_ob = [&](int it, float v) __attribute__((always_inline)) {
+        if constexpr (STEM && W < 7)
+            if (ob_off >= 0) reinterpret_cast<float *>(smem + kOb0 + (it & 1) * stemx::kObBytes)[ob_off] = v;
+    };
+    float OBv = 0.f;
     auto stage = [&](int it) __attribute__((always_inline)) {
         const int64_t t = t0 + (int64_t)it * step;
         const int rows = (int)max<int64_t>(0, min<int64_t>(kTile, a.M - t * kTile));
+        if constexpr (STEM) {
+            using SM = stemx::Map<W>;
+            const int rx0 = SM::rho0(ch, hh);
+            float XS[2][5];
+            stemx::rebuild<SM::kC0, SM::kNc>(reinterpret_cast<const float *>(smem + kWt0),
+                                             reinterpret_cast<const float *>(smem + kOb0 + (it & 1) * stemx::kObBytes),
+                                             a.cin, ch, rx0, rows, XS);
+            float *xr = reinterpret_cast<float *>(smem + kXr0 + (it & 1) * kXrBytes);
+            unsigned char *xi = smem + kX0 + (it & 1) * kImgBytes;
+            const int halfx = rx0 >> 3, subx = 2 * (rx0 & 7);
+#pragma unroll
+            for (int i = 0; i < SM::kNc; ++i) {
+                float xv2[2];
+                uint32_t xs[3];
+#pragma unroll
+                for (int r = 0; r < 2; ++r) {
+                    const float u = XS[r][i] * pa + pb;
+                    xv2[r] = u < 0.f ? 0.f : u;
+                    xr[(rx0 + r) * kXrStride + ch * kCells + SM::kC0 + i] = XS[r][i];
+                }
+                hrl_split::split_pair(xv2[0], xv2[1], xs[0], xs[1], xs[2]);
+                const int o = img_off(SM::kC0 + i, ch, halfx) + subx;
+#pragma unroll
+                for (int part = 0; part < 3; ++part) *reinterpret_cast<uint32_t *>(xi + part * kPartBytes + o) = xs[part];
+            }
+        }
         unsigned char *dyi = smem + kDy0 + (it & 1) * kImgBytes;
         unsigned char *xi = smem + kX0 + (it & 1) * kImgBytes;
         const float *dzl = reinterpret_cast<const float *>(smem + kDz0 + (it & 1) * kDzBytes);
@@ -1060,8 +1182,8 @@
                 const float tt = (yv - mu) * kk;
                 float d = (((gv - gmn) - tt) * is) * ww;
                 d = valid ? d : 0.f;
-                float xv = X[r][i];
-                if constexpr (PRO) {
+                float xv = STEM ? 0.f : X[r][i];
+                if constexpr (PRO && !STEM) {
                     const float u = xv * pa + pb;
                     xv = u < 0.f ? 0.f : u;
                 }
@@ -1070,7 +1192,7 @@
                 xv2[r] = xv;
             }
             hrl_split::split_pair(dv[0], dv[1], dp[0][i], dp[1][i], dp[2][i]);
-            if constexpr (!kFwd) hrl_split::split_pair(xv2[0], xv2[1], xp[0][i], xp[1][i], xp[2][i]);
+            if constexpr (!kFwd && !STEM) hrl_split::split_pair(xv2[0], xv2[1], xp[0][i], xp[1][i], xp[2][i]);
         }
         const int half = rho0 >> 3, sub = 2 * (rho0 & 7);
 #pragma unroll
@@ -1079,10 +1201,11 @@
 #pragma unroll
             for (int part = 0; part < 3; ++part) {
                 *reinterpret_cast<uint32_t *>(dyi + part * kPartBytes + o) = dp[part][i];
-                if constexpr (!kFwd) *reinterpret_cast<uint32_t *>(xi + part * kPartBytes + o) = xp[part][i];
-            }
-        }
-        if constexpr (EPI == 2 || EPI == 3) {
+                if constexpr (!kFwd && !STEM)
+                    *reinterpret_cast<uint32_t *>(xi + part * kPartBytes + o) = xp[part][i];
+            }
+        }
+        if constexpr ((EPI == 2 || EPI == 3) && !STEM) {
             float *xr = reinterpret_cast<float *>(smem + kXr0 + (it & 1) * kXrBytes);
 #pragma unroll
             for (int r = 0; r < 2; ++r)
@@ -1246,6 +1369,20 @@
             stage(0);
             issue(1);
         }
+    } else if constexpr (STEM) {
+        stemx::fill_table(reinterpret_cast<float *>(smem + kWt0), a.stem_w, a.stem_b, a.cin, W * 64 + lane);
+        if (n_iter > 0) {
+            const float o0 = load_ob(0), o1 = load_ob(1);
+            issue(0);
+            put_ob(0, o0);
+            put_ob(1, o1);
+            OBv = load_ob(2);
+        }
+        bar_lds();
+        if (n_iter > 0) {
+            stage(0);
+            issue(1);
+        }
     } else if (n_iter > 0) {
         issue(0);
         stage(0);
@@ -1263,6 +1400,10 @@
                 put_dz(it + 2, DZv);
                 DZv = load_dz(it + 3);
             }
+            if constexpr (STEM) {
+                put_ob(it + 2, OBv);
+                OBv = load_ob(it + 3);
+            }
             issue(it + 2);
             BB2_STAMP(it, 2);
         } else {
@@ -1270,6 +1411,10 @@
             if constexpr (DZ) {
                 put_dz(it + 2, DZv);
                 DZv = load_dz(it + 3);
+            }
+            if constexpr (STEM) {
+                put_ob(it + 2, OBv);
+                OBv = load_ob(it + 3);
             }
             issue(it + 2);
             BB2_STAMP(it, 1);
@@ -1322,6 +1467,9 @@
 constexpr int kLdsBytes = kRaw0 + kSlots * kRawBytes;
 static_assert(kLdsBytes <= 160 * 1024, "LDS");
 static_assert(kRawBytes % 1024 == 0, "whole LDS-DMA pieces per tile");
+constexpr int kOb0 = kRaw0;
+constexpr int kWt0 = kOb0 + 2 * stemx::kObBytes;
+constexpr int kLdsBytesStem = kRaw0 + stemx::kBytes;
 
 template <int N> __device__ __forceinline__ void vm_wait() { asm volatile("s_waitcnt vmcnt(%0)" ::"n"(N) : "memory"); }
 
@@ -1378,8 +1526,9 @@
     static_assert(kSlots == 5, "the early-iteration counts above are written for kSlots = 5");
 }
 
-template <bool PRO, int W>
+template <bool PRO, int W, bool STEM = false>
 __device__ __forceinline__ void run(const BlockBwdArgs &a, unsigned char *smem, int lane) {
+    static_assert(!STEM || PRO, "the stem form is behind the stem's ReLU");
     constexpr int kCt = W & 1, G = W >> 1;
     using C = Cells<G>;
     constexpr int kNq = C::kN;
@@ -1415,7 +1564,7 @@
         }
     }
     float pa = 1.f, pb = 0.f;
-    if constexpr (PRO) {
+    if constexpr (PRO && !STEM) {
         pa = a.in_alpha[ch];
         pb = a.in_beta[ch];
     }
@@ -1433,19 +1582,29 @@
             dma16(desc, p * 1024 + lane * 16, raw + p * 1024);
         }
     };
-    const int c0 = hh ? 4 : 0;
-    const int rho0 = 2 * ((W + (ch >> 2)) & 7);
+    constexpr int kNc = STEM ? stemx::Map<W>::kNc : 5;
+    const int c0 = STEM ? stemx::Map<W>::kC0 : (hh ? 4 : 0);
+    const int rho0 = STEM ? stemx::Map<W>::rho0(ch, hh) : 2 * ((W + (ch >> 2)) & 7);
     auto stage = [&](int it, int slot) __attribute__((always_inline)) {
         const float *raw = reinterpret_cast<const float *>(smem + kRaw0 + slot * kRawBytes);
         unsigned char *xi = smem + kImg0 + (it & 1) * bb2::kImgBytes;
         uint32_t xp[3][5];
         float xv[2][5];
+        if constexpr (STEM) {
+            const int64_t t = t0 + (int64_t)it * step;
+            const int rows = (int)max<int64_t>(0, min<int64_t>(kTile, a.M - t * kTile));
+            stemx::rebuild<stemx::Map<W>::kC0, kNc>(
+                reinterpret_cast<const float *>(smem + kWt0),
+                reinterpret_cast<const float *>(smem + kOb0 + slot * stemx::kObBytes), a.cin, ch, rho0, rows, xv);
+        }
 #pragma unroll
         for (int r = 0; r < 2; ++r) {
             const float *src = raw + (rho0 + r) * kRow + ch * kCells + c0;
 #pragma unroll
-            for (int i = 0; i < 5; ++i) {
-                float v = src[i];
+            for (int i = 0; i < kNc; ++i) {
+                float v;
+                if constexpr (STEM) v = xv[r][i];
+                else v = src[i];
                 if constexpr (PRO) {
                     const float u = v * pa + pb;
                     v = u < 0.f ? 0.f : u;
@@ -1454,10 +1613,10 @@
             }
         }
 #pragma unroll
-        for (int i = 0; i < 5; ++i) hrl_split::split_pair(xv[0][i], xv[1][i], xp[0][i], xp[1][i], xp[2][i]);
+        for (int i = 0; i < kNc; ++i) hrl_split::split_pair(xv[0][i], xv[1][i], xp[0][i], xp[1][i], xp[2][i]);
         const int half = rho0 >> 3, sub = 2 * (rho0 & 7);
 #pragma unroll
-        for (int i = 0; i < 5; ++i) {
+        for (int i = 0; i < kNc; ++i) {
             const int o = bb2::img_off(c0 + i, ch, half) + sub;
 #pragma unroll
             for (int part = 0; part < 3; ++part)
@@ -1468,19 +1627,52 @@
     const int g = lane >> 4, i16 = lane & 15, qq = i16 >> 2, pp = i16 & 3;
     const int tr_sub = 8 * (pp & 1);
     double s1 = 0.0, s2 = 0.0;
-#pragma unroll
-    for (int j = 0; j < kSlots; ++j) dma(j, j);
-    vm_wait<(kSlots - 1) * NP>();
-    bb2::bar_lds();
-    stage(0, 0);
-    vm_wait<(kSlots - 2) * NP>();
-    bb2::bar_lds();
+    const int ob_off = STEM && W < 7 ? stemx::slot_off(W * 64 + lane, a.cin) : -1;
+    auto load_ob = [&](int it) __attribute__((always_inline)) {
+        float v = 0.f;
+        if constexpr (STEM && W < 7) {
+            const int K = a.cin * kCells;
+            const int64_t t = t0 + (int64_t)it * step;
+            const bool ok = it < n_iter;
+            const int rows = ok ? (int)min<int64_t>(kTile, a.M - t * kTile) : 0;
+            const __amdgpu_buffer_rsrc_t ro = wave_rsrc(a.obs + (ok ? t * kTile * K : 0), (uint32_t)(rows * K * 4));
+            v = __uint_as_float(__builtin_amdgcn_raw_buffer_load_b32(ro, (W * 64 + lane) * 4, 0, 0));
+        }
+        return v;
+    };
+    auto put_ob = [&](int it, float v) __attribute__((always_inline)) {
+        if constexpr (STEM && W < 7)
+            if (ob_off >= 0) reinterpret_cast<float *>(smem + kOb0 + (it & 1) * stemx::kObBytes)[ob_off] = v;
+    };
+    float OBv = 0.f;
+    if constexpr (STEM) {
+        stemx::fill_table(reinterpret_cast<float *>(smem + kWt0), a.stem_w, a.stem_b, a.cin, W * 64 + lane);
+        const float o0 = load_ob(0), o1 = load_ob(1);
+        put_ob(0, o0);
+        put_ob(1, o1);
+        OBv = load_ob(2);
+        bb2::bar_lds();
+        stage(0, 0);
+        bb2::bar_lds();
+    } else {
+#pragma unroll
+        for (int j = 0; j < kSlots; ++j) dma(j, j);
+        vm_wait<(kSlots - 1) * NP>();
+        bb2::bar_lds();
+        stage(0, 0);
+        vm_wait<(kSlots - 2) * NP>();
+        bb2::bar_lds();
+    }
     int slot = 0;
     for (int it = 0; it < n_iter; ++it) {
         BB2_STAMP(it, 0);
-        dma(it + kSlots, slot);
-        const int next = slot + 1 == kSlots ? 0 : slot + 1;
+        if constexpr (!STEM) dma(it + kSlots, slot);
+        const int next = STEM ? (slot ^ 1) : (slot + 1 == kSlots ? 0 : slot + 1);
         stage(it + 1, next);
+        if constexpr (STEM) {
+            put_ob(it + 2, OBv);
+            OBv = load_ob(it + 3);
+        }
         BB2_STAMP(it, 1);
         const unsigned char *img = smem + kImg0 + (it & 1) * bb2::kImgBytes;
         f32x4 acc[kNq];
@@ -1553,7 +1745,7 @@
                 __builtin_amdgcn_raw_buffer_store_b64(v, od, off, 0, 0);
             }
         }
-        wait_tile_after<NP, NS>(it);
+        if constexpr (!STEM) wait_tile_after<NP, NS>(it);
         BB2_STAMP(it, 3);
         bb2::bar_lds();
         slot = next;
@@ -1575,37 +1767,38 @@
 
 }
 
-template <bool PRO>
+template <bool PRO, bool STEM = false>
 __global__ __launch_bounds__(bb2::kThreads) void conv3x3_fwd_dma_kernel(BlockBwdArgs a) {
-    __shared__ __attribute__((aligned(16))) unsigned char smem[fw3::kLdsBytes];
+    __shared__ __attribute__((aligned(16))) unsigned char smem[STEM ? fw3::kLdsBytesStem : fw3::kLdsBytes];
     const int lane = threadIdx.x & 63;
     const int wave = __builtin_amdgcn_readfirstlane(threadIdx.x >> 6);
     switch (wave) {
-    case 0: fw3::run<PRO, 0>(a, smem, lane); break;
-    case 1: fw3::run<PRO, 1>(a, smem, lane); break;
-    case 2: fw3::run<PRO, 2>(a, smem, lane); break;
-    case 3: fw3::run<PRO, 3>(a, smem, lane); break;
-    case 4: fw3::run<PRO, 4>(a, smem, lane); break;
-    case 5: fw3::run<PRO, 5>(a, smem, lane); break;
-    case 6: fw3::run<PRO, 6>(a, smem, lane); break;
-    default: fw3::run<PRO, 7>(a, smem, lane); break;
-    }
-}
-
-template <bool PRO, int EPI, bool DZ = false>
+    case 0: fw3::run<PRO, 0, STEM>(a, smem, lane); break;
+    case 1: fw3::run<PRO, 1, STEM>(a, smem, lane); break;
+    case 2: fw3::run<PRO, 2, STEM>(a, smem, lane); break;
+    case 3: fw3::run<PRO, 3, STEM>(a, smem, lane); break;
+    case 4: fw3::run<PRO, 4, STEM>(a, smem, lane); break;
+    case 5: fw3::run<PRO, 5, STEM>(a, smem, lane); break;
+    case 6: fw3::run<PRO, 6, STEM>(a, smem, lane); break;
+    default: fw3::run<PRO, 7, STEM>(a, smem, lane); break;
+    }
+}
+
+template <bool PRO, int EPI, bool DZ = false, bool STEM = false>
 __global__ __launch_bounds__(bb2::kThreads) void conv3x3_block_bwd2_kernel(BlockBwdArgs a) {
-    __shared__ __attribute__((aligned(16))) unsigned char smem[DZ ? bb2::kLdsBytesDz : bb2::kLdsBytes];
+    __shared__ __attribute__((aligned(16)))
+    unsigned char smem[DZ ? bb2::kLdsBytesDz : (STEM ? bb2::kLdsBytesStem : bb2::kLdsBytes)];
     const int lane = threadIdx.x & 63;
     const int wave = __builtin_amdgcn_readfirstlane(threadIdx.x >> 6);
     switch (wave) {
-    case 0: bb2::run<PRO, EPI, 0, DZ>(a, smem, lane); break;
-    case 1: bb2::run<PRO, EPI, 1, DZ>(a, smem, lane); break;
-    case 2: bb2::run<PRO, EPI, 2, DZ>(a, smem, lane); break;
-    case 3: bb2::run<PRO, EPI, 3, DZ>(a, smem, lane); break;
-    case 4: bb2::run<PRO, EPI, 4, DZ>(a, smem, lane); break;
-    case 5: bb2::run<PRO, EPI, 5, DZ>(a, smem, lane); break;
-    case 6: bb2::run<PRO, EPI, 6, DZ>(a, smem, lane); break;
-    default: bb2::run<PRO, EPI, 7, DZ>(a, smem, lane); break;
+    case 0: bb2::run<PRO, EPI, 0, DZ, STEM>(a, smem, lane); break;
+    case 1: bb2::run<PRO, EPI, 1, DZ, STEM>(a, smem, lane); break;
+    case 2: bb2::run<PRO, EPI, 2, DZ, STEM>(a, smem, lane); break;
+    case 3: bb2::run<PRO, EPI, 3, DZ, STEM>(a, smem, lane); break;
+    case 4: bb2::run<PRO, EPI, 4, DZ, STEM>(a, smem, lane); break;
+    case 5: bb2::run<PRO, EPI, 5, DZ, STEM>(a, smem, lane); break;
+    case 6: bb2::run<PRO, EPI, 6, DZ, STEM>(a, smem, lane); break;
+    default: bb2::run<PRO, EPI, 7, DZ, STEM>(a, smem, lane); break;
     }
 }
 
@@ -1938,6 +2131,47 @@
     return status();
 }
 
+int hrl_conv3x3_forward_stem(const float *obs, int64_t M, int64_t Cin, const float *stem_w, const float *stem_b,
+                             const float *packed_w, float *y, double *part, void *workspace,
+                             int64_t workspace_bytes, void *stream) {
+    if (M < 1 || Cin < 1 || Cin > 3 || !obs || !stem_w || !packed_w || !y || !part || !workspace) return HRL_EINVAL;
+    if (!aligned16(y) || (reinterpret_cast<uintptr_t>(obs) & 3) != 0) return HRL_EINVAL;
+    if (workspace_bytes < hrl_conv3x3_workspace_bytes(M) || M * kRow * 4 > 0xffffffffLL) return HRL_EINVAL;
+    if (g_fwd_form != 2 || !g_split) return HRL_EINVAL;
+    BlockBwdArgs a{};
+    a.obs = obs; a.stem_w = stem_w; a.stem_b = stem_b; a.cin = (int)Cin;
+    a.wpk = packed_w; a.gin = y; a.part = part; a.M = M;
+    hipLaunchKernelGGL((conv3x3_fwd_dma_kernel<true, true>), dim3(grid_for(M)), dim3(bb2::kThreads), 0,
+                       static_cast<hipStream_t>(stream), a);
+    return status();
+}
+
+int hrl_conv3x3_block_backward_stem(const float *g, const float *y, int64_t M, const float *bn_weight,
+                                    const float *bn_bias, const float *save_mean, const float *save_invstd,
+                                    const float *kcoef, const float *gmean, const float *obs, int64_t Cin,
+                                    const float *stem_w, const float *stem_b, const float *packed_flip,
+                                    float *dweight, float *gin, void *workspace, int64_t workspace_bytes,
+                                    void *stream) {
+    if (M < 1 || Cin < 1 || Cin > 3 || !g || !y || !save_mean || !save_invstd || !kcoef || !gmean || !obs ||
+        !stem_w || !packed_flip || !gin || !workspace)
+        return HRL_EINVAL;
+    if ((reinterpret_cast<uintptr_t>(obs) & 3) != 0) return HRL_EINVAL;
+    if (workspace_bytes < hrl_conv3x3_workspace_bytes(M) || M * kRow * 4 > 0xffffffffLL) return HRL_EINVAL;
+    if (g_block_form != 1) return HRL_EINVAL;
+    hipStream_t s = static_cast<hipStream_t>(stream);
+    const int grid = grid_for(M);
+    float *wpart = static_cast<float *>(workspace) + kTaps * 2 * kC * 16 * 2;
+    BlockBwdArgs a{g, y, bn_weight, bn_bias, save_mean, save_invstd, kcoef, gmean, nullptr, nullptr, nullptr,
+                   packed_flip, nullptr, nullptr, nullptr, gin, nullptr, wpart, M};
+    a.obs = obs; a.stem_w = stem_w; a.stem_b = stem_b; a.cin = (int)Cin;
+    hipLaunchKernelGGL((conv3x3_block_bwd2_kernel<true, 3, false, true>), dim3(grid), dim3(bb2::kThreads), 0, s, a);
+    int rc = status();
+    if (rc || !dweight) return rc;
+    hipLaunchKernelGGL(conv3x3_wgrad_reduce_kernel, dim3(kTaps * kC * kC / 64), dim3(256), 0, s, wpart, grid,
+                       dweight);
+    return status();
+}
+
 int64_t hrl_conv3x3_wgrad_partials(int64_t M, int64_t *offset_bytes) {
     if (M < 1) return -1;
     if (offset_bytes) *offset_bytes = (int64_t)kTaps * 2 * kC * 16 * 2 * 4;
diff --git a/handyrl_amd/nn.py b/handyrl_amd/nn.py
--- a/handyrl_amd/nn.py
+++ b/handyrl_amd/nn.py
@@ -1332,6 +1332,8 @@
         b = bias.contiguous() if bias is not None else None
         _native.check(lib.hrl_stem_forward(_native.ptr(x), N, Cin, _native.ptr(w), _native.ptr(b), _native.ptr(y),
                                            _native.stream_of(x.device)), 'hrl_stem_forward')
+        STEM_STATS['materialised'] += 1
+        STEM_STATS['last'] = ('materialised', N)
         ctx.save_for_backward(x, w)
         ctx.params = (weight, bias)
         return y
@@ -1340,27 +1342,31 @@
     def backward(ctx, dy):
         x, w = ctx.saved_tensors
         weight, bias = ctx.params
-        N, Cin = x.shape[0], x.shape[1]
-        lib = _native.load()
-        ws_bytes = lib.hrl_stem_workspace_bytes(N)
-        ws = torch.empty(ws_bytes, dtype=torch.uint8, device=x.device)
-        bw = _grad_buffer(weight)
-        bb = _grad_buffer(bias) if bias is not None else (None, False)
-        df = _defer_folds([bw, bb]) if lib.hrl_stem_set_wgrad_form(0) == 2 else None
-        dwp, dbp = (None, None) if df is not None else (bw[0], bb[0])
-        _native.check(lib.hrl_stem_wgrad(_native.ptr(x), _native.ptr(dy.contiguous()), N, Cin, _native.ptr(dwp),
-                                         _native.ptr(dbp), _native.ptr(ws), ws_bytes,
-                                         _native.stream_of(x.device)), 'hrl_stem_wgrad')
-        if df is not None:
-            row = ctypes.c_int64(0)
-            nparts = lib.hrl_stem_wgrad_partials(N, ctypes.byref(row))
-            part = ws.view(torch.float32)
-            nw = 32 * Cin * 9
-            df.add(part, row.value, 0, nparts, bw[0], nw)
-            if bb[0] is not None:
-                df.add(part, row.value, nw, nparts, bb[0], 32)
-            df.keep.append(ws)
-        return None, _ret(bw), _ret(bb)
+        return (None, *_stem_wgrad(x, dy, weight, bias))
+
+
+def _stem_wgrad(x, dy, weight, bias):
+    N, Cin = x.shape[0], x.shape[1]
+    lib = _native.load()
+    ws_bytes = lib.hrl_stem_workspace_bytes(N)
+    ws = torch.empty(ws_bytes, dtype=torch.uint8, device=x.device)
+    bw = _grad_buffer(weight)
+    bb = _grad_buffer(bias) if bias is not None else (None, False)
+    df = _defer_folds([bw, bb]) if lib.hrl_stem_set_wgrad_form(0) == 2 else None
+    dwp, dbp = (None, None) if df is not None else (bw[0], bb[0])
+    _native.check(lib.hrl_stem_wgrad(_native.ptr(x), _native.ptr(dy.contiguous()), N, Cin, _native.ptr(dwp),
+                                     _native.ptr(dbp), _native.ptr(ws), ws_bytes,
+                                     _native.stream_of(x.device)), 'hrl_stem_wgrad')
+    if df is not None:
+        row = ctypes.c_int64(0)
+        nparts = lib.hrl_stem_wgrad_partials(N, ctypes.byref(row))
+        part = ws.view(torch.float32)
+        nw = 32 * Cin * 9
+        df.add(part, row.value, 0, nparts, bw[0], nw)
+        if bb[0] is not None:
+            df.add(part, row.value, nw, nparts, bb[0], 32)
+        df.keep.append(ws)
+    return _ret(bw), _ret(bb)
 
 
 class _BoardWeight(torch.autograd.Function):
@@ -1733,7 +1739,7 @@
     return u
 
 
-def _chain_forward(h0, meta, relu_in, params, apply_out=True):
+def _chain_forward(h0, meta, relu_in, params, apply_out=True, stem=None):
     lib = _native.load()
     M = h0.shape[0]
     dev = h0.device
@@ -1760,10 +1766,15 @@
                                              P(packed[k]), stream), 'hrl_conv3x3_pack_n')
     for i, (rm, rv, momentum, eps) in enumerate(meta):
         w, gamma, beta = params[3 * i:3 * i + 3]
-        y = torch.empty_like(h0)
-        _native.check(lib.hrl_conv3x3_forward_ex(P(x), M, P(a_prev), P(b_prev), P(packed[i, 0]), None, 2, P(y),
-                                                 1, None, None, None, None, P(part), P(ws), ws_bytes, stream),
-                      'hrl_conv3x3_forward_ex')
+        y = torch.empty(M, 32, 3, 3, dtype=torch.float32, device=dev)
+        if i == 0 and stem is not None:
+            _native.check(lib.hrl_conv3x3_forward_stem(P(h0), M, h0.shape[1], P(stem[0]), P(stem[1]), P(packed[0, 0]),
+                                                       P(y), P(part), P(ws), ws_bytes, stream),
+                          'hrl_conv3x3_forward_stem')
+        else:
+            _native.check(lib.hrl_conv3x3_forward_ex(P(x), M, P(a_prev), P(b_prev), P(packed[i, 0]), None, 2, P(y),
+                                                     1, None, None, None, None, P(part), P(ws), ws_bytes, stream),
+                          'hrl_conv3x3_forward_ex')
         coef = torch.empty(4, 32, dtype=torch.float32, device=dev)
         _native.check(lib.hrl_bn_finalize_stats(P(part), nblk, 32, M * 9, P(gamma), P(beta), P(rm), P(rv),
                                                 float(momentum), float(eps), P(coef[0]), P(coef[1]),
@@ -1773,7 +1784,7 @@
         x, a_prev, b_prev = y, coef[2], coef[3]
     out = None
     if apply_out:
-        out = torch.empty_like(h0)
+        out = torch.empty_like(ys[-1])
         _native.check(lib.hrl_bn_apply(P(x), M, 32, 9, P(a_prev), P(b_prev), 1, P(out), stream), 'hrl_bn_apply')
     return out, ys, coefs, unit, packed
 
@@ -1791,8 +1802,24 @@
     return form
 
 
+STEM_FUSED = True
+STEM_STATS = {'fused_forward': 0, 'fused_backward': 0, 'materialised': 0, 'last': None}
+
+
+def _form_of(setter):
+    form = setter(0)
+    setter(form)
+    return form
+
+
+def _stem_fused_ok(lib, n, heads):
+    return (STEM_FUSED and (heads or n >= 2) and _form_of(lib.hrl_stem_set_fwd_form) == 2
+            and _form_of(lib.hrl_conv3x3_set_fwd_form) == 2 and _form_of(lib.hrl_conv3x3_set_split) == 1
+            and _block_form(lib) == 1)
+
+
 def _chain_backward(h0, ys, coefs, unit, params, relu_in, g, need_input_grad, packed, part_in=None, nblk_in=0,
-                    heads_dz=None):
+                    heads_dz=None, stem=None):
     lib = _native.load()
     n = len(ys)
     M = h0.shape[0]
@@ -1826,9 +1853,9 @@
                           'hrl_bn_finalize_backward')
             gin, epi, ep = None, 0, (None, None, None)
             if i > 0:
-                gin, epi, ep = torch.empty_like(h0), 2, (coefs[i - 1][0], coefs[i - 1][2], coefs[i - 1][3])
-            elif need_input_grad:
-                gin, epi = torch.empty_like(h0), (3 if relu_in else 0)
+                gin, epi, ep = torch.empty_like(ys[0]), 2, (coefs[i - 1][0], coefs[i - 1][2], coefs[i - 1][3])
+            elif need_input_grad or stem is not None:
+                gin, epi = torch.empty_like(ys[0]), (3 if relu_in else 0)
             df = _defer_folds([bw])
             wsb = ws if df is None else torch.empty(ws_bytes, dtype=torch.uint8, device=dev)
             ev = _block_timing_start()
@@ -1838,6 +1865,11 @@
                     P(kg[0]), P(kg[1]), P(x), P(a), P(b), P(packed[i, 1]), None if df is not None else P(dw), P(gin),
                     epi, P(ep[0]), P(ep[1]), P(ep[2]), P(part), P(wsb), ws_bytes, stream),
                     'hrl_conv3x3_block_backward_dz')
+            elif stem is not None and i == 0:
+                _native.check(lib.hrl_conv3x3_block_backward_stem(
+                    P(g), P(ys[0]), M, P(gamma), P(beta), P(mean), P(invstd), P(kg[0]), P(kg[1]), P(h0), h0.shape[1],
+                    P(stem[0]), P(stem[1]), P(packed[0, 1]), None if df is not None else P(dw), P(gin), P(wsb),
+                    ws_bytes, stream), 'hrl_conv3x3_block_backward_stem')
             else:
                 _native.check(lib.hrl_conv3x3_block_backward(
                     P(g), P(ys[i]), M, P(gamma), P(beta), P(mean), P(invstd), P(kg[0]), P(kg[1]), P(x), P(a), P(b),
@@ -1880,12 +1912,32 @@
     return g, grads
 
 
+def _stem_enter(ctx, stem_w, stem_b, rows):
+    ctx.stem = ctx.stem_params = None
+    if stem_w is None:
+        return None
+    ctx.stem_params = (stem_w, stem_b)
+    ctx.stem = (stem_w.contiguous(), stem_b.contiguous() if stem_b is not None else None)
+    STEM_STATS['fused_forward'] += 1
+    STEM_STATS['last'] = ('fused', rows)
+    return ctx.stem
+
+
+def _stem_leave(ctx, obs, g_in):
+    if ctx.stem is None:
+        return g_in, None, None
+    STEM_STATS['fused_backward'] += 1
+    dsw, dsb = _stem_wgrad(obs, g_in, *ctx.stem_params)
+    return None, dsw, dsb
+
+
 class _BoardChain(torch.autograd.Function):
 
     @staticmethod
-    def forward(ctx, h0, meta, relu_in, *params):
+    def forward(ctx, h0, stem_w, stem_b, meta, relu_in, *params):
         h0 = h0.contiguous()
-        out, ys, coefs, unit, packed = _chain_forward(h0, meta, relu_in, params)
+        stem = _stem_enter(ctx, stem_w, stem_b, h0.shape[0])
+        out, ys, coefs, unit, packed = _chain_forward(h0, meta, relu_in, params, stem=stem)
         ctx.save_for_backward(h0, *ys, *coefs, packed, *params)
         ctx.n = len(meta)
         ctx.relu_in = relu_in
@@ -1897,16 +1949,19 @@
         t = ctx.saved_tensors
         h0, ys, coefs, packed, params = t[0], list(t[1:1 + n]), list(t[1 + n:1 + 2 * n]), t[1 + 2 * n], t[2 + 2 * n:]
         unit = _unit_coefs(h0.device) if ctx.relu_in else None
-        g_in, grads = _chain_backward(h0, ys, coefs, unit, params, ctx.relu_in, g, ctx.needs_input_grad[0], packed)
-        return (g_in, None, None, *grads)
+        g_in, grads = _chain_backward(h0, ys, coefs, unit, params, ctx.relu_in, g, ctx.needs_input_grad[0], packed,
+                                      stem=ctx.stem)
+        g_in, dsw, dsb = _stem_leave(ctx, h0, g_in)
+        return (g_in, dsw, dsb, None, None, *grads)
 
 
 class _ChainHeadsFn(torch.autograd.Function):
 
     @staticmethod
-    def forward(ctx, h0, meta, relu_in, tanh_v, w1p, b1p, w1v, b1v, wp, wv, *params):
+    def forward(ctx, h0, stem_w, stem_b, meta, relu_in, tanh_v, w1p, b1p, w1v, b1v, wp, wv, *params):
         h0 = h0.contiguous()
-        _, ys, coefs, unit, packed = _chain_forward(h0, meta, relu_in, params, apply_out=False)
+        stem = _stem_enter(ctx, stem_w, stem_b, h0.shape[0])
+        _, ys, coefs, unit, packed = _chain_forward(h0, meta, relu_in, params, apply_out=False, stem=stem)
         y, coef = ys[-1], coefs[-1]
         N = h0.shape[0]
         dev = h0.device
@@ -1942,7 +1997,7 @@
         y, coef = ys[-1], coefs[-1]
         dp, dv = dp.contiguous(), dv.contiguous()
         use_dz = _heads_dz_ok(lib, n)
-        dh = torch.empty(N, 28, device=dev, dtype=h0.dtype) if use_dz else torch.empty_like(h0)
+        dh = torch.empty(N, 28, device=dev, dtype=h0.dtype) if use_dz else torch.empty_like(y)
         heads_backward = lib.hrl_heads_backward_dz if use_dz else lib.hrl_heads_backward
         hbufs = [_grad_buffer(x) for x in (w1p, b1p, w1v, b1v, wp, wv)]
         ws_bytes = lib.hrl_heads_workspace_bytes(N)
@@ -1961,8 +2016,10 @@
             call(*(b[0] for b in hbufs))
         unit = _unit_coefs(dev) if ctx.relu_in else None
         g_in, grads = _chain_backward(h0, ys, coefs, unit, params, ctx.relu_in, dh, ctx.needs_input_grad[0], packed,
-                                      part_in=bn_part, nblk_in=nparts, heads_dz=(w1p, w1v) if use_dz else None)
-        return (g_in, None, None, None, *(_ret(b) for b in hbufs), *grads)
+                                      part_in=bn_part, nblk_in=nparts, heads_dz=(w1p, w1v) if use_dz else None,
+                                      stem=ctx.stem)
+        g_in, dsw, dsb = _stem_leave(ctx, h0, g_in)
+        return (g_in, dsw, dsb, None, None, None, *(_ret(b) for b in hbufs), *grads)
 
 
 class _ConvBNChain(nn.Module):
@@ -1971,6 +2028,7 @@
         super().__init__()
         object.__setattr__(self, 'convs', list(convs))
         object.__setattr__(self, 'bns', list(bns))
+        object.__setattr__(self, 'stem', None)
         self.relu_in = relu_in
 
     @staticmethod
@@ -1981,19 +2039,39 @@
                 and b.num_features == 32 for b in bns)
 
     def forward(self, x):
+        return self.run(*self.enter(x, heads=False))
+
+    def enter(self, x, heads):
+        if self.stem is None or (x.dim() == 4 and x.shape[1] == 32):
+            return x, None
+        stem_args = self.stem_args(x, heads)
+        return (x, stem_args) if stem_args is not None else (self.stem(x), None)
+
+    def run(self, x, stem_args=None):
         convs, bns = self.convs, self.bns
-        if not self.fused_ok(x):
+        if not self.fused_ok(x, stem_args is not None):
             if self.relu_in:
                 x = torch.relu(x)
             for c, b in zip(convs, bns):
                 x = b(c(x))
             return x
         meta, params = self.meta_params()
-        return _BoardChain.apply(x, meta, self.relu_in, *params)
-
-    def fused_ok(self, x):
-        return (x.is_cuda and x.dtype == torch.float32 and x.dim() == 4 and tuple(x.shape[1:]) == (32, 3, 3)
-                and x.shape[0] > 0 and all(b.training and b.fused_relu for b in self.bns)
+        return _BoardChain.apply(x, *(stem_args or (None, None)), meta, self.relu_in, *params)
+
+    def stem_args(self, x, heads):
+        stem = self.stem
+        if stem is None or not (x.is_cuda and x.dtype == torch.float32 and x.dim() == 4 and x.shape[0] > 0
+                                and tuple(x.shape[1:]) == (stem.in_channels, 3, 3) and not x.requires_grad
+                                and stem.weight.requires_grad and (stem.bias is None or stem.bias.requires_grad)
+                                and stem.weight.dtype == torch.float32 and self.fused_ok(x, True)):
+            return None
+        if not _stem_fused_ok(_native.load(), len(self.convs), heads):
+            return None
+        return stem.weight, stem.bias
+
+    def fused_ok(self, x, stem_input=False):
+        return (x.is_cuda and x.dtype == torch.float32 and x.dim() == 4
+                and (stem_input or tuple(x.shape[1:]) == (32, 3, 3)) and x.shape[0] > 0 and all(b.training and b.fused_relu for b in self.bns)
                 and torch.is_grad_enabled())
 
     def meta_params(self):
@@ -2016,13 +2094,14 @@
         self.tanh_v = False
 
     def forward(self, x):
-        if not self.chain.fused_ok(x):
-            p, v = self.heads(self.chain(x))
+        x, stem_args = self.chain.enter(x, heads=True)
+        if not self.chain.fused_ok(x, stem_args is not None):
+            p, v = self.heads(self.chain.run(x))
             return p, (torch.tanh(v) if self.tanh_v else v)
         (cp, fp), (cv, fv) = _board_head_spec(self.heads.head_p), _board_head_spec(self.heads.head_v)
         meta, params = self.chain.meta_params()
-        return _ChainHeadsFn.apply(x, meta, self.chain.relu_in, self.tanh_v, cp.weight, cp.bias, cv.weight, cv.bias,
-                                   fp.weight, fv.weight, *params)
+        return _ChainHeadsFn.apply(x, *(stem_args or (None, None)), meta, self.chain.relu_in, self.tanh_v, cp.weight,
+                                   cp.bias, cv.weight, cv.bias, fp.weight, fv.weight, *params)
 
 
 def _fuse_chain_heads(gm):
@@ -2050,6 +2129,30 @@
                     fused.tanh_v = True
         return 1
     return 0
+
+
+def _fuse_stem(gm):
+    count = 0
+    for node in list(gm.graph.nodes):
+        if node.op != 'call_module' or node.kwargs or len(node.args) != 1:
+            continue
+        mod = gm.get_submodule(node.target)
+        chain = mod.chain if isinstance(mod, _ChainHeads) else mod
+        if not isinstance(chain, _ConvBNChain) or not chain.relu_in or chain.stem is not None:
+            continue
+        src = node.args[0]
+        if not (isinstance(src, torch.fx.Node) and src.op == 'call_module' and len(src.users) == 1
+                and len(src.args) == 1 and not src.kwargs):
+            continue
+        stem = gm.get_submodule(src.target)
+        if not (type(stem) is BoardConv2d and tuple(stem.weight.shape[2:]) == (3, 3) and stem.out_channels == 32
+                and stem.in_channels <= 3 and _board_conv_ok(stem)):
+            continue
+        object.__setattr__(chain, 'stem', stem)
+        node.args = src.args
+        gm.graph.erase_node(src)
+        count += 1
+    return count
 
 
 class _LeafTracer(torch.fx.Tracer):
@@ -2122,6 +2225,8 @@
     fused_heads = _fuse_heads(gm, heads) if heads else 0
     if fused_heads:
         fused_heads += _fuse_chain_heads(gm)
+    if chains:
+        _fuse_stem(gm)
     if not pairs and not merged and not fused_heads:
         return 0
     gm.graph.lint()
diff --git a/handyrl_amd/trainer.py b/handyrl_amd/trainer.py
--- a/handyrl_amd/trainer.py
+++ b/handyrl_amd/trainer.py
@@ -445,7 +445,11 @@
         return None
 
     def _grab_cut(self, _module, args):
-        cut = args[0].view_as(args[0])
+        x = args[0]
+        stem = getattr(getattr(_module, 'chain', _module), 'stem', None)
+        if stem is not None and x.shape[1] != 32:
+            x = stem(x)
+        cut = x.view_as(x)
         self._cut = cut
         return (cut,) + tuple(args[1:])
 
diff --git a/include/hrl_nn.h b/include/hrl_nn.h
--- a/include/hrl_nn.h
+++ b/include/hrl_nn.h
@@ -104,6 +104,15 @@
                                   float *dweight, float *gin, int epilogue, const float *ep_mean,
                                   const float *ep_alpha, const float *ep_beta, double *part, void *workspace,
                                   int64_t workspace_bytes, void *stream);
+int hrl_conv3x3_forward_stem(const float *obs, int64_t M, int64_t Cin, const float *stem_w, const float *stem_b,
+                             const float *packed_w, float *y, double *part, void *workspace,
+                             int64_t workspace_bytes, void *stream);
+int hrl_conv3x3_block_backward_stem(const float *g, const float *y, int64_t M, const float *bn_weight,
+                                    const float *bn_bias, const float *save_mean, const float *save_invstd,
+                                    const float *kcoef, const float *gmean, const float *obs, int64_t Cin,
+                                    const float *stem_w, const float *stem_b, const float *packed_flip,
+                                    float *dweight, float *gin, void *workspace, int64_t workspace_bytes,
+                                    void *stream);
 
 int hrl_lstm_gates_forward(const float *zx, int64_t zx_stride, const float *zh, const float *c, int64_t N, int64_t H,
                            int64_t HW, const float *bias, int64_t bias_rows, float *h_out, float *c_out, float *gates,
```

Result: no change. 135.4 million env-steps/s (median of 6 runs) (+0.8%).
